# hamaadshah/gan_deeplearning4j

Hardware: NVIDIA H100
Metric: images/sec (full G+D step) (higher is better)
Workload: dtype bf16

## Files before the change

gan_deeplearning4j_b200/__init__.py:

```python
from ._lib import B200GanError, LIB_PATH, PROTOTYPES, load
from .engine import BF16, FP32, EPI_ACTBWD, EPI_BNBWD, EPI_PLAIN, EPI_STATS, Context, Gan, Net, comm_unique_id, test_bn, test_conv, test_conv_ex, test_dropout, test_ew
from . import data, models, parallel, serializer
```

gan_deeplearning4j_b200/_lib.py:

```python
from __future__ import annotations

import ctypes as C
import os

_HERE = os.path.dirname(os.path.abspath(__file__))
LIB_PATH = os.path.join(_HERE, "lib", "libb200gan.so")
NAME_LEN = 64


class B200GanError(RuntimeError):
    def __init__(self, code, msg):
        super().__init__(f"libb200gan error {code}: {msg}")
        self.code = code


class LayerDesc(C.Structure):
    _fields_ = [("type", C.c_int32), ("name", C.c_char * NAME_LEN), ("n_in", C.c_int32), ("n_out", C.c_int32),
                ("k_h", C.c_int32), ("k_w", C.c_int32), ("s_h", C.c_int32), ("s_w", C.c_int32), ("p_h", C.c_int32), ("p_w", C.c_int32),
                ("has_bias", C.c_int32), ("act", C.c_int32), ("act_alpha", C.c_float), ("updater", C.c_int32),
                ("lr", C.c_float), ("beta1", C.c_float), ("beta2", C.c_float), ("eps", C.c_float), ("l2", C.c_float),
                ("bn_decay", C.c_float), ("bn_eps", C.c_float), ("pre_h", C.c_int32), ("pre_w", C.c_int32), ("pre_c", C.c_int32),
                ("loss", C.c_int32), ("frozen", C.c_int32)]


class NetConfig(C.Structure):
    _fields_ = [("in_h", C.c_int32), ("in_w", C.c_int32), ("in_c", C.c_int32), ("max_batch", C.c_int32), ("precision", C.c_int32),
                ("grad_clip", C.c_float), ("xent_clip_eps", C.c_float), ("bn_groups", C.c_int32), ("seed", C.c_uint64)]


class GanConfig(C.Structure):
    _fields_ = [("fake_bn_train", C.c_int32), ("use_cuda_graph", C.c_int32)]


class LrSchedule(C.Structure):
    _fields_ = [("kind", C.c_int32), ("type", C.c_int32), ("initial", C.c_double), ("gamma", C.c_double), ("power", C.c_double),
                ("step", C.c_double), ("decay_rate", C.c_double), ("n_map", C.c_int32), ("map_keys", C.POINTER(C.c_int32)),
                ("map_values", C.POINTER(C.c_double))]


class ConvGeom(C.Structure):
    _fields_ = [(k, C.c_int32) for k in ("n", "h", "w", "c", "oh", "ow", "o", "kh", "kw", "sh", "sw", "ph", "pw")]


class TestConvOpts(C.Structure):
    _fields_ = [("epi", C.c_int32), ("act", C.c_int32), ("alpha", C.c_float), ("bias", C.POINTER(C.c_float)), ("scale", C.POINTER(C.c_float)),
                ("groups", C.c_int32), ("aux", C.POINTER(C.c_float)), ("aux2", C.POINTER(C.c_float)), ("stats", C.POINTER(C.c_double)), ("kernel", C.c_char * 64),
                ("bn", C.c_int32), ("max_ctas", C.c_int32), ("poison", C.c_int32), ("w_mn", C.c_int32), ("per_tap", C.c_int32), ("slab", C.c_int32),
                ("defer", C.c_int32), ("db", C.POINTER(C.c_float)), ("param_offset", C.c_int32), ("splits", C.c_int32)]


class EwReduceJob(C.Structure):
    _fields_ = [("n", C.c_int64), ("stride", C.c_int64), ("src_off", C.c_int64), ("dst_off", C.c_int64), ("splits", C.c_int32), ("wide", C.c_int32)]


class TestEwOpts(C.Structure):
    _fields_ = [("op", C.c_int32), ("n", C.c_int64), ("rows", C.c_int32), ("cols", C.c_int32), ("groups", C.c_int32), ("splits", C.c_int32),
                ("stride", C.c_int64)] + [(k, C.c_int32) for k in ("N", "H", "W", "C", "KH", "KW", "SH", "SW", "act")] + [
                ("alpha", C.c_float), ("clip_eps", C.c_float), ("offset", C.c_int32), ("in_place", C.c_int32), ("accumulate", C.c_int32),
                ("poison", C.c_int32), ("n_jobs", C.c_int32), ("jobs", C.POINTER(EwReduceJob)), ("n_seg", C.c_int32),
                ("seg_off", C.POINTER(C.c_int64)), ("seg_len", C.POINTER(C.c_int64)), ("seg_coef", C.POINTER(C.c_float)), ("sumsq", C.c_double),
                ("kernel", C.c_char * 64), ("loss", C.c_int32)]


_vp, _i32, _i64, _fp = C.c_void_p, C.c_int32, C.c_int64, C.POINTER(C.c_float)
_pvp = C.POINTER(C.c_void_p)

PROTOTYPES = {
    "b2g_version": (_i32, []),
    "b2g_ctx_create": (_i32, [_i32, _pvp]),
    "b2g_ctx_destroy": (_i32, [_vp]),
    "b2g_last_error": (C.c_char_p, []),
    "b2g_sync": (_i32, [_vp]),
    "b2g_launch_count": (_i32, [_vp, C.POINTER(C.c_uint64)]),
    "b2g_timer_start": (_i32, [_vp]),
    "b2g_timer_stop_ms": (_i32, [_vp, _fp]),
    "b2g_flush_l2": (_i32, [_vp]),
    "b2g_device_info": (_i32, [_vp, C.POINTER(_i32), C.POINTER(_i32), C.POINTER(_i32), C.POINTER(C.c_uint64)]),
    "b2g_net_create": (_i32, [_vp, C.POINTER(NetConfig), C.POINTER(LayerDesc), _i32, _pvp]),
    "b2g_net_destroy": (_i32, [_vp]),
    "b2g_net_num_params": (_i32, [_vp, C.POINTER(_i64)]),
    "b2g_net_output_size": (_i32, [_vp, C.POINTER(_i64)]),
    "b2g_net_layer_output_size": (_i32, [_vp, _i32, C.POINTER(_i64)]),
    "b2g_net_set_param": (_i32, [_vp, C.c_char_p, C.c_char_p, _fp, _i64]),
    "b2g_net_get_param": (_i32, [_vp, C.c_char_p, C.c_char_p, _fp, _i64]),
    "b2g_net_get_params": (_i32, [_vp, _fp, _i64]),
    "b2g_net_set_params": (_i32, [_vp, _fp, _i64]),
    "b2g_net_get_gradients": (_i32, [_vp, _fp, _i64]),
    "b2g_net_updater_state_size": (_i32, [_vp, C.POINTER(_i64)]),
    "b2g_net_get_updater_state": (_i32, [_vp, _fp, _i64]),
    "b2g_net_set_updater_state": (_i32, [_vp, _fp, _i64]),
    "b2g_net_output": (_i32, [_vp, _fp, _i32, _i32, _fp]),
    "b2g_net_get_activation": (_i32, [_vp, _i32, _i32, _fp]),
    "b2g_net_compute_gradient_and_score": (_i32, [_vp, _fp, _fp, _i32, _fp]),
    "b2g_net_get_input_gradient": (_i32, [_vp, _i32, _fp]),
    "b2g_net_fit": (_i32, [_vp, _fp, _fp, _i32, _fp]),
    "b2g_net_get_iteration": (_i32, [_vp, C.POINTER(_i64)]),
    "b2g_net_set_iteration": (_i32, [_vp, _i64]),
    "b2g_net_get_dropout_pass": (_i32, [_vp, C.POINTER(_i64)]),
    "b2g_net_set_dropout_pass": (_i32, [_vp, _i64]),
    "b2g_net_set_gradient_normalization": (_i32, [_vp, _i32, C.c_float]),
    "b2g_net_set_lr_schedule": (_i32, [_vp, C.c_char_p, C.POINTER(LrSchedule)]),
    "b2g_net_get_learning_rate": (_i32, [_vp, C.c_char_p, _fp]),
    "b2g_net_get_epoch": (_i32, [_vp, C.POINTER(_i64)]),
    "b2g_net_set_epoch": (_i32, [_vp, _i64]),
    "b2g_net_simt_gemm_calls": (_i32, [_vp, C.POINTER(C.c_uint64)]),
    "b2g_gan_create": (_i32, [_vp, _vp, C.POINTER(GanConfig), _pvp]),
    "b2g_gan_destroy": (_i32, [_vp]),
    "b2g_gan_step": (_i32, [_vp, _fp, _fp, _fp, _fp, _fp, _fp, _i32, _fp]),
    "b2g_gan_upload": (_i32, [_vp, _fp, _fp, _fp, _fp, _fp, _fp, _i32]),
    "b2g_gan_step_resident": (_i32, [_vp, _i32]),
    "b2g_gan_read_losses": (_i32, [_vp, _fp]),
    "b2g_gan_last_step_ms": (_i32, [_vp, _fp]),
    "b2g_comm_unique_id": (_i32, [_vp]),
    "b2g_ctx_comm_init": (_i32, [_vp, _i32, _i32, _vp]),
    "b2g_ctx_comm_destroy": (_i32, [_vp]),
    "b2g_net_set_grad_allreduce": (_i32, [_vp, _i32]),
    "b2g_net_average_parameters": (_i32, [_vp]),
    "b2g_net_set_sync_bn": (_i32, [_vp, _i32]),
    "b2g_net_set_grad_payload_bf16": (_i32, [_vp, _i32]),
    "b2g_net_enable_p2p_allreduce": (_i32, [_vp, C.POINTER(C.c_int32)]),
    "b2g_ctx_allreduce_test": (_i32, [_vp, _fp, _i64]),
    "b2g_test_conv": (_i32, [_vp, _i32, _i32, _i32, C.POINTER(ConvGeom), _fp, _fp, _fp, _i32, _fp]),
    "b2g_test_hbm_kernels": (_i32, [_vp, _i32, _i32, _i32, _fp]),
    "b2g_test_conv_ex": (_i32, [_vp, _i32, _i32, _i32, C.POINTER(ConvGeom), _fp, _fp, _fp, _i32, _fp, C.POINTER(TestConvOpts)]),
    "b2g_test_bn": (_i32, [_vp, _i32, _i32, _i32, _i32, _i32, _fp, _fp, _fp, _fp, _fp, _fp, _i32, C.c_float, C.c_float, C.c_float,
                           _i32, _fp, _fp, _fp, _fp, _fp, _fp, _fp, _fp]),
    "b2g_test_net_shadow": (_i32, [_vp, _i32, _i32, _fp, _i64]),
    "b2g_test_dropout": (_i32, [_vp, _i32, C.c_uint64, _i32, _i32, _i64, _i32, _i32, _i32, _i32, C.c_float, _fp, _fp, _fp, _fp]),
    "b2g_test_ew": (_i32, [_vp, _i32, C.POINTER(TestEwOpts), _fp, _fp, _fp, _fp, _fp]),
}

_lib = None


def load():
    global _lib
    if _lib is not None:
        return _lib
    if not os.path.exists(LIB_PATH):
        raise B200GanError(-7, f"{LIB_PATH} is missing: build it with `make` (nvcc, sm_90a). There is no CPU fallback.")
    lib = C.CDLL(LIB_PATH, mode=C.RTLD_GLOBAL)
    for name, (res, args) in PROTOTYPES.items():
        fn = getattr(lib, name)
        fn.restype, fn.argtypes = res, args
    _lib = lib
    return lib


def check(code):
    if code != 0:
        raise B200GanError(code, load().b2g_last_error().decode(errors="replace"))
```

gan_deeplearning4j_b200/csrc/common.cuh:

```cuda
#pragma once
#include <cuda_runtime.h>
#include <cuda_bf16.h>
#include <math.h>
#include <stdlib.h>
#include <stdint.h>
#include "kernels.h"

namespace b2g {

#define LAUNCHED() do { ++::b2g::g_launch_count; } while (0)

__device__ __forceinline__ void pdl_wait() { asm volatile("griddepcontrol.wait;" ::: "memory"); }
__device__ __forceinline__ void pdl_trigger() { asm volatile("griddepcontrol.launch_dependents;" ::: "memory"); }
__device__ __forceinline__ void pdl_enter() { pdl_trigger(); pdl_wait(); }
template <typename... KArgs, typename... Args>
inline cudaError_t launch_pdl(void (*kernel)(KArgs...), dim3 grid, dim3 block, size_t smem, cudaStream_t stream, Args&&... args) {
  cudaLaunchConfig_t cfg{}; cfg.gridDim = grid; cfg.blockDim = block; cfg.dynamicSmemBytes = smem; cfg.stream = stream;
  cudaLaunchAttribute at[1]; at[0].id = cudaLaunchAttributeProgrammaticStreamSerialization; at[0].val.programmaticStreamSerializationAllowed = 1;
  cfg.attrs = at; cfg.numAttrs = 1;
  return cudaLaunchKernelEx(&cfg, kernel, static_cast<KArgs>(args)...);
}

__device__ __forceinline__ void sacc_add(unsigned long long* hi_lo, size_t stride, size_t idx, double d) {
  const long long hi = __double2ll_rn(d * 1024.0);
  const double r = d - (double)hi * (1.0 / 1024.0);
  const long long lo = __double2ll_rn(r * 1152921504606846976.0);
  atomicAdd(hi_lo + idx, (unsigned long long)hi);
  atomicAdd(hi_lo + stride + idx, (unsigned long long)lo);
}
__device__ __forceinline__ double sacc_read(const unsigned long long* hi_lo, size_t stride, size_t idx) {
  return (double)(long long)hi_lo[idx] * (1.0 / 1024.0) + (double)(long long)hi_lo[stride + idx] * (1.0 / 1152921504606846976.0);
}

__device__ __forceinline__ double block_sum(double v, double* red) {
#pragma unroll
  for (int o = 16; o > 0; o >>= 1) v += __shfl_xor_sync(0xffffffffu, v, o);
  if ((threadIdx.x & 31) == 0) red[threadIdx.x >> 5] = v;
  __syncthreads();
  double t = 0.0;
  if (threadIdx.x == 0) for (int w = 0; w < (int)(blockDim.x >> 5); ++w) t += red[w];
  return t;
}

struct Philox4 { uint32_t x[4]; };
__device__ __forceinline__ Philox4 philox4x32_10(uint32_t c0, uint32_t c1, uint32_t c2, uint32_t c3, uint32_t k0, uint32_t k1) {
#pragma unroll
  for (int r = 0; r < 10; ++r) {
    if (r) { k0 += 0x9E3779B9u; k1 += 0xBB67AE85u; }
    const uint32_t lo0 = 0xD2511F53u * c0, hi0 = __umulhi(0xD2511F53u, c0);
    const uint32_t lo1 = 0xCD9E8D57u * c2, hi1 = __umulhi(0xCD9E8D57u, c2);
    c0 = hi1 ^ c1 ^ k0; c1 = lo1; c2 = hi0 ^ c3 ^ k1; c3 = lo0;
  }
  return Philox4{{c0, c1, c2, c3}};
}

#define DISPATCH_PREC(prec, T, ...)                                   \
  do {                                                                \
    if ((prec) == ::b2g::PREC_F32) { using T = float; __VA_ARGS__; }  \
    else { using T = __nv_bfloat16; __VA_ARGS__; }                    \
  } while (0)

__device__ __forceinline__ float ldf(const float* p, size_t i) { return p[i]; }
__device__ __forceinline__ float ldf(const __nv_bfloat16* p, size_t i) { return __bfloat162float(p[i]); }
__device__ __forceinline__ void stf(float* p, size_t i, float v) { p[i] = v; }
__device__ __forceinline__ void stf(__nv_bfloat16* p, size_t i, float v) { p[i] = __float2bfloat16_rn(v); }

__device__ __forceinline__ float act_fwd(int act, float z, float alpha) {
  switch (act) {
    case ACT_TANH: return tanhf(z);
    case ACT_SIGMOID: return 1.0f / (1.0f + expf(-z));
    case ACT_RELU: return fmaxf(z, 0.f);
    case ACT_LRELU: return z > 0.f ? z : alpha * z;
    default: return z;
  }
}
__device__ __forceinline__ float act_grad_from_pre(int act, float z, float alpha) {
  switch (act) {
    case ACT_TANH: { float t = tanhf(z); return 1.0f - t * t; }
    case ACT_SIGMOID: { float s = 1.0f / (1.0f + expf(-z)); return s * (1.0f - s); }
    case ACT_RELU: return z > 0.f ? 1.0f : 0.f;
    case ACT_LRELU: return z > 0.f ? 1.0f : alpha;
    default: return 1.0f;
  }
}
__device__ __forceinline__ float act_grad_from_out(int act, float a, float alpha) {
  switch (act) {
    case ACT_TANH: return 1.0f - a * a;
    case ACT_SIGMOID: return a * (1.0f - a);
    case ACT_RELU: return a > 0.f ? 1.0f : 0.f;
    case ACT_LRELU: return a > 0.f ? 1.0f : alpha;
    default: return 1.0f;
  }
}

}
```

gan_deeplearning4j_b200/csrc/engine.cu:

```cuda
#include <cuda_runtime.h>
#include <dlfcn.h>
#include <math.h>
#include <stdarg.h>
#include <stdio.h>
#include <stdlib.h>
#include <string.h>

#include <algorithm>
#include <string>
#include <vector>

#include "../../include/b200gan.h"
#include "kernels.h"

using namespace b2g;

static thread_local char g_err[1024] = "";
static int32_t fail(int32_t code, const char* fmt, ...) {
  va_list ap; va_start(ap, fmt); vsnprintf(g_err, sizeof(g_err), fmt, ap); va_end(ap); return code;
}
#define CU(call) do { cudaError_t e_ = (call); if (e_ != cudaSuccess) return fail(B2G_ERR_CUDA, "%s:%d %s -> %s", __FILE__, __LINE__, #call, cudaGetErrorString(e_)); } while (0)
#define B2(call) do { int32_t r_ = (call); if (r_ != 0) return r_; } while (0)
#define CHECK_KERNELS() CU(cudaGetLastError())

// ... 1065 lines not shown
      g->graph_launches = g_launch_count - before; g_launch_count = before;
      g->graph_simt_g = g->G->simt_gemm_calls - sg0; g->graph_simt_d = g->D->simt_gemm_calls - sd0; g->G->simt_gemm_calls = sg0; g->D->simt_gemm_calls = sd0;
      if (r) return r; if (e != cudaSuccess) return fail(B2G_ERR_CUDA, "graph capture: %s", cudaGetErrorString(e));
      CU(cudaGraphInstantiate(&g->exec1, g->graph1, 0)); CU(cudaGraphInstantiate(&g->exec, g->graph, 0)); g->graph_batch = batch;
      g->graph_settings_g = g->G->settings_gen; g->graph_settings_d = g->D->settings_gen;
    }
    CU(cudaGraphLaunch(g->exec1, s));
    CU(cudaStreamWaitEvent(s, g->ev_x, 0));
    CU(cudaGraphLaunch(g->exec, s)); g_launch_count += g->graph_launches; g->G->simt_gemm_calls += g->graph_simt_g; g->D->simt_gemm_calls += g->graph_simt_d;
  }
  CU(cudaEventRecord(g->ev1, s)); g->ev1_valid = true;
  return 0;
}
extern "C" int32_t b2g_gan_read_losses(b2g_gan* g, float* losses) {
  if (!g || !losses) return fail(B2G_ERR_ARG, "null"); cudaStream_t s = g->G->ctx->stream; CU(cudaSetDevice(g->G->ctx->device));
  float h[4]; CU(cudaMemcpyAsync(h, g->loss_dev, sizeof(h), cudaMemcpyDeviceToHost, s)); CU(cudaStreamSynchronize(s));
  int N = g->last_batch;
  losses[0] = h[0] / N; losses[1] = h[1] / N; losses[2] = h[2] / N; return 0;
}
extern "C" int32_t b2g_gan_last_step_ms(b2g_gan* g, float* ms) {
  if (!g || !ms) return fail(B2G_ERR_ARG, "null"); CU(cudaEventSynchronize(g->ev1)); CU(cudaEventElapsedTime(ms, g->ev0, g->ev1)); return 0;
}
extern "C" int32_t b2g_gan_step(b2g_gan* g, const float* x_real, const float* z_d, const float* z_g, const float* y_real, const float* y_fake, const float* y_gen, int32_t batch, float* losses) {
  B2(b2g_gan_upload(g, x_real, z_d, z_g, y_real, y_fake, y_gen, batch));
  B2(b2g_gan_step_resident(g, batch));
  if (losses) return b2g_gan_read_losses(g, losses);
  return 0;
}

extern "C" int32_t b2g_net_get_iteration(b2g_net* n, int64_t* out) {
  if (!n || !out) return fail(B2G_ERR_ARG, "null"); CU(cudaSetDevice(n->ctx->device));
  int v = 0; CU(cudaMemcpyAsync(&v, n->step_dev, sizeof(int), cudaMemcpyDeviceToHost, n->ctx->stream)); CU(cudaStreamSynchronize(n->ctx->stream)); *out = v; return 0;
}
extern "C" int32_t b2g_net_set_iteration(b2g_net* n, int64_t it) {
  if (!n || it < 0 || it > 0x7fffffff) return fail(B2G_ERR_ARG, "bad iteration"); CU(cudaSetDevice(n->ctx->device));
  int v = (int)it; CU(cudaMemcpyAsync(n->step_dev, &v, sizeof(int), cudaMemcpyHostToDevice, n->ctx->stream)); CU(cudaStreamSynchronize(n->ctx->stream)); return 0;
}
extern "C" int32_t b2g_net_get_dropout_pass(b2g_net* n, int64_t* out) {
  if (!n || !out) return fail(B2G_ERR_ARG, "null"); CU(cudaSetDevice(n->ctx->device));
  unsigned long long v = 0; CU(cudaMemcpyAsync(&v, n->drop_pass, sizeof(v), cudaMemcpyDeviceToHost, n->ctx->stream)); CU(cudaStreamSynchronize(n->ctx->stream)); *out = (int64_t)v; return 0;
}
extern "C" int32_t b2g_net_set_dropout_pass(b2g_net* n, int64_t pass) {
  if (!n || pass < 0) return fail(B2G_ERR_ARG, "bad dropout pass"); CU(cudaSetDevice(n->ctx->device));
  unsigned long long v = (unsigned long long)pass; CU(cudaMemcpyAsync(n->drop_pass, &v, sizeof(v), cudaMemcpyHostToDevice, n->ctx->stream)); CU(cudaStreamSynchronize(n->ctx->stream)); return 0;
}
extern "C" int32_t b2g_net_set_gradient_normalization(b2g_net* n, int32_t mode, float threshold) {
  if (!n) return fail(B2G_ERR_ARG, "null");
  if (mode == B2G_GN_CLIP_ELEMENTWISE) return fail(B2G_ERR_ARG, "ClipElementWiseAbsoluteValue is b2g_net_config.grad_clip, set when the net is created");
  if (mode != B2G_GN_NONE && mode != B2G_GN_RENORM_L2_LAYER && mode != B2G_GN_RENORM_L2_PARAM && mode != B2G_GN_CLIP_L2_LAYER && mode != B2G_GN_CLIP_L2_PARAM)
    return fail(B2G_ERR_ARG, "unknown gradient normalization %d", mode);
  if (mode != B2G_GN_NONE && n->cfg.grad_clip > 0.f)
    return fail(B2G_ERR_ARG, "the net was created with grad_clip %g (ClipElementWiseAbsoluteValue): one gradient normalization per layer", (double)n->cfg.grad_clip);
  const bool clip = mode == B2G_GN_CLIP_L2_LAYER || mode == B2G_GN_CLIP_L2_PARAM;
  if (clip && !(threshold > 0.f && isfinite(threshold))) return fail(B2G_ERR_ARG, "gradient normalization threshold %g: the clip modes need a finite threshold > 0", (double)threshold);
  if (!clip) threshold = 1.0f;
  if (mode != n->gn_mode || threshold != n->gn_threshold) { n->gn_mode = mode; n->gn_threshold = threshold; ++n->settings_gen; }
  return 0;
}

static int lr_segment(const b2g_net* n, int li) {
  for (size_t i = 0; i < n->segs.size(); ++i) if (n->seg_layer[i] == li && n->segs[i].kind != 3 && n->segs[i].kind != 9) return (int)i;
  return -1;
}
static bool layer_has_lr(const b2g_net* n, int li) { return lr_segment(n, li) >= 0; }
static int32_t find_lr_layer(const b2g_net* n, const char* layer, int* li) {
  for (size_t i = 0; i < n->L.size(); ++i) if (!strncmp(n->L[i].d.name, layer, B2G_NAME_LEN)) {
    if (!layer_has_lr(n, (int)i)) return fail(B2G_ERR_ARG, "layer %s has no learning rate (frozen, no parameters, NoOp or AdaDelta)", layer);
    *li = (int)i; return 0;
  }
  return fail(B2G_ERR_ARG, "no layer named %s", layer);
}
static int32_t net_upload_schedules(b2g_net* n) {
  cudaStream_t s = n->ctx->stream;
  size_t nv = 0; for (auto& ls : n->layer_sched) nv += ls.vals.size();
  const size_t bytes = nv * (sizeof(double) + sizeof(int32_t));
  CU(cudaStreamSynchronize(s));
  if (bytes > n->sched_map_bytes) {
    if (n->sched_map) { cudaFree(n->sched_map); n->sched_map = nullptr; n->sched_map_bytes = 0; }
    cudaError_t e = cudaMalloc(&n->sched_map, bytes);
    if (e != cudaSuccess) { n->sched_map = nullptr; return fail(B2G_ERR_OOM, "cudaMalloc(%zu) failed: %s", bytes, cudaGetErrorString(e)); }
    n->sched_map_bytes = bytes;
  }
  std::vector<char> host(bytes); double* dv = (double*)n->sched_map; int32_t* dk = (int32_t*)((char*)n->sched_map + nv * sizeof(double));
  std::vector<UpdSched> per_layer(n->L.size()); size_t at = 0;
  for (size_t li = 0; li < n->L.size(); ++li) {
    const auto& ls = n->layer_sched[li]; per_layer[li] = ls.sc;
    if (ls.sc.kind == B2G_SCHED_MAP) {
      memcpy(host.data() + at * sizeof(double), ls.vals.data(), ls.vals.size() * sizeof(double));
      memcpy(host.data() + nv * sizeof(double) + at * sizeof(int32_t), ls.keys.data(), ls.keys.size() * sizeof(int32_t));
      per_layer[li].vals = dv + at; per_layer[li].keys = dk + at; at += ls.vals.size();
    }
  }
  std::vector<UpdSched> seg(n->segs.size()); bool on = false;
  for (size_t i = 0; i < n->segs.size(); ++i) { seg[i] = per_layer[n->seg_layer[i]]; on = on || seg[i].kind != B2G_SCHED_NONE; }
  if (bytes) CU(cudaMemcpyAsync(n->sched_map, host.data(), bytes, cudaMemcpyHostToDevice, s));
  if (!seg.empty()) CU(cudaMemcpyAsync(n->sched_dev, seg.data(), sizeof(UpdSched) * seg.size(), cudaMemcpyHostToDevice, s));
  CU(cudaStreamSynchronize(s));
  n->sched_on = on; ++n->settings_gen;
  return 0;
}
extern "C" int32_t b2g_net_set_lr_schedule(b2g_net* n, const char* layer, const b2g_lr_schedule* s) {
  if (!n) return fail(B2G_ERR_ARG, "null"); CU(cudaSetDevice(n->ctx->device));
  b2g_net::LayerSched ls;
  if (s && s->kind != B2G_SCHED_NONE) {
    if (s->kind < B2G_SCHED_EXPONENTIAL || s->kind > B2G_SCHED_MAP) return fail(B2G_ERR_ARG, "unknown schedule kind %d (PolySchedule is not supported)", s->kind);
    if (s->type != B2G_SCHED_ITERATION && s->type != B2G_SCHED_EPOCH) return fail(B2G_ERR_ARG, "unknown schedule type %d", s->type);
    if (!std::isfinite(s->initial) || !std::isfinite(s->gamma) || !std::isfinite(s->power) || !std::isfinite(s->step) || !std::isfinite(s->decay_rate))
      return fail(B2G_ERR_ARG, "schedule parameters must be finite");
    if (s->kind == B2G_SCHED_STEP && !(s->step > 0.0)) return fail(B2G_ERR_ARG, "StepSchedule step %g: must be > 0", s->step);
    if (s->kind == B2G_SCHED_INVERSE && s->gamma < 0.0) return fail(B2G_ERR_ARG, "InverseSchedule gamma %g: must be >= 0", s->gamma);
    UpdSched& sc = ls.sc; sc.kind = s->kind; sc.type = s->type;
    sc.initial = s->initial; sc.gamma = s->gamma; sc.power = s->power; sc.step = s->step; sc.decay = s->decay_rate;
    if (s->kind == B2G_SCHED_MAP) {
      if (s->n_map < 1 || !s->map_keys || !s->map_values) return fail(B2G_ERR_ARG, "MapSchedule needs at least one entry");
      bool has0 = false;
      for (int j = 0; j < s->n_map; ++j) {
        if (j > 0 && s->map_keys[j] <= s->map_keys[j - 1]) return fail(B2G_ERR_ARG, "MapSchedule keys must strictly increase");
        if (!std::isfinite(s->map_values[j])) return fail(B2G_ERR_ARG, "MapSchedule values must be finite");
        has0 = has0 || s->map_keys[j] == 0;
      }
      if (!has0) return fail(B2G_ERR_ARG, "MapSchedule has no value for key 0");
      ls.keys.assign(s->map_keys, s->map_keys + s->n_map); ls.vals.assign(s->map_values, s->map_values + s->n_map); sc.n_map = s->n_map;
    }
  }
  if (layer) { int li = 0; B2(find_lr_layer(n, layer, &li)); n->layer_sched[li] = ls; }
  else for (size_t li = 0; li < n->L.size(); ++li) if (layer_has_lr(n, (int)li)) n->layer_sched[li] = ls;
  return net_upload_schedules(n);
}
extern "C" int32_t b2g_net_get_learning_rate(b2g_net* n, const char* layer, float* out) {
  if (!n || !layer || !out) return fail(B2G_ERR_ARG, "null"); CU(cudaSetDevice(n->ctx->device));
  int li = 0; B2(find_lr_layer(n, layer, &li));
  const int seg = lr_segment(n, li);
  k_sched_lr(n->segs_dev, n->sched_dev, seg, n->step_dev, n->epoch_dev, n->lr_out, n->ctx->stream); CHECK_KERNELS();
  CU(cudaMemcpyAsync(out, n->lr_out, sizeof(float), cudaMemcpyDeviceToHost, n->ctx->stream)); CU(cudaStreamSynchronize(n->ctx->stream));
  return 0;
}
extern "C" int32_t b2g_net_get_epoch(b2g_net* n, int64_t* out) {
  if (!n || !out) return fail(B2G_ERR_ARG, "null"); CU(cudaSetDevice(n->ctx->device));
  int64_t v = 0; CU(cudaMemcpyAsync(&v, n->epoch_dev, sizeof(v), cudaMemcpyDeviceToHost, n->ctx->stream)); CU(cudaStreamSynchronize(n->ctx->stream)); *out = v; return 0;
}
extern "C" int32_t b2g_net_set_epoch(b2g_net* n, int64_t epoch) {
  if (!n || epoch < 0) return fail(B2G_ERR_ARG, "bad epoch"); CU(cudaSetDevice(n->ctx->device));
  CU(cudaMemcpyAsync(n->epoch_dev, &epoch, sizeof(epoch), cudaMemcpyHostToDevice, n->ctx->stream)); CU(cudaStreamSynchronize(n->ctx->stream)); return 0;
}
extern "C" int32_t b2g_net_simt_gemm_calls(b2g_net* n, uint64_t* out) { if (!n || !out) return fail(B2G_ERR_ARG, "null"); *out = n->simt_gemm_calls; return 0; }

extern "C" int32_t b2g_comm_unique_id(void* id128) { if (!id128) return fail(B2G_ERR_ARG, "null"); B2(nccl_load()); NcclId id; NC(g_nccl.uid(&id)); memcpy(id128, &id, sizeof(id)); return 0; }
extern "C" int32_t b2g_ctx_comm_init(b2g_ctx* c, int32_t world, int32_t rank, const void* id128) {
  if (!c || !id128 || world < 1 || rank < 0 || rank >= world) return fail(B2G_ERR_ARG, "bad communicator arguments");
  B2(nccl_load()); CU(cudaSetDevice(c->device));
  NcclId id; memcpy(&id, id128, sizeof(id));
  NC(g_nccl.init(&c->comm, world, id, rank)); c->world = world; c->rank = rank; return 0;
}
extern "C" int32_t b2g_ctx_comm_destroy(b2g_ctx* c) { if (c && c->comm) { g_nccl.destroy(c->comm); c->comm = nullptr; c->world = 1; c->rank = 0; } return 0; }
extern "C" int32_t b2g_net_set_grad_allreduce(b2g_net* n, int32_t enabled) { if (!n) return fail(B2G_ERR_ARG, "null"); n->grad_allreduce = enabled != 0; return 0; }
extern "C" int32_t b2g_net_set_sync_bn(b2g_net* n, int32_t enabled) { if (!n) return fail(B2G_ERR_ARG, "null"); if (enabled && n->prec != PREC_BF16) return fail(B2G_ERR_UNSUPPORTED, "sync_bn rides on the fused BatchNorm path (BF16 nets)"); n->sync_bn = enabled != 0; return 0; }
extern "C" int32_t b2g_net_set_grad_payload_bf16(b2g_net* n, int32_t enabled) {
  if (!n) return fail(B2G_ERR_ARG, "null"); CU(cudaSetDevice(n->ctx->device));
  if (enabled && !n->ar_buf) B2(dalloc(n, &n->ar_buf, sizeof(__nv_bfloat16) * (size_t)n->n_params));
  n->ar_bf16 = enabled != 0; return 0;
}
extern "C" int32_t b2g_net_enable_p2p_allreduce(b2g_net* n, int32_t* enabled) {
  if (!n) return fail(B2G_ERR_ARG, "null"); b2g_ctx* c = n->ctx; CU(cudaSetDevice(c->device)); if (enabled) *enabled = 0;
  if (!c->comm || c->world < 2) return 0;
  if (c->world > 8 || !g_nccl.ag) return 0;
  cudaStream_t s = c->stream;
  if (!c->p2p_flags) { CU(cudaMalloc(&c->p2p_flags, 16 * sizeof(unsigned))); CU(cudaMalloc(&c->p2p_state, 2 * sizeof(unsigned)));
                       CU(cudaMemsetAsync(c->p2p_flags, 0, 16 * sizeof(unsigned), s)); CU(cudaMemsetAsync(c->p2p_state, 0, 2 * sizeof(unsigned), s)); CU(cudaStreamSynchronize(s)); }
  struct Pair { cudaIpcMemHandle_t flags, grads; };
  Pair mine; memset(&mine, 0, sizeof(mine)); float ok = 1.f;
  if (cudaIpcGetMemHandle(&mine.flags, c->p2p_flags) != cudaSuccess || cudaIpcGetMemHandle(&mine.grads, n->grads) != cudaSuccess) { cudaGetLastError(); ok = 0.f; }
  std::vector<Pair> all(c->world);
  char *d_send = nullptr, *d_recv = nullptr; float* d_ok = nullptr;
  CU(cudaMalloc(&d_send, sizeof(Pair))); CU(cudaMalloc(&d_recv, sizeof(Pair) * c->world)); CU(cudaMalloc(&d_ok, sizeof(float)));
  CU(cudaMemcpyAsync(d_send, &mine, sizeof(Pair), cudaMemcpyHostToDevice, s));
  NC(g_nccl.ag(d_send, d_recv, sizeof(Pair),  0, c->comm, s));
  CU(cudaMemcpyAsync(all.data(), d_recv, sizeof(Pair) * c->world, cudaMemcpyDeviceToHost, s)); CU(cudaStreamSynchronize(s));
  float* pg[8] = {}; unsigned* pf[8] = {};
  for (int r = 0; r < c->world && ok > 0.f; ++r) {
    if (r == c->rank) { pg[r] = n->grads; pf[r] = c->p2p_flags; continue; }
    void* q = nullptr;
    if (cudaIpcOpenMemHandle(&q, all[r].grads, cudaIpcMemLazyEnablePeerAccess) != cudaSuccess) { cudaGetLastError(); ok = 0.f; break; }
    pg[r] = (float*)q;
    if (c->p2p_flags_mapped) pf[r] = c->p2p_peer_flags[r];
    else { if (cudaIpcOpenMemHandle(&q, all[r].flags, cudaIpcMemLazyEnablePeerAccess) != cudaSuccess) { cudaGetLastError(); ok = 0.f; break; } pf[r] = (unsigned*)q; }
  }
  CU(cudaMemcpyAsync(d_ok, &ok, sizeof(float), cudaMemcpyHostToDevice, s)); NC(g_nccl.ar(d_ok, d_ok, 1, 7, 0, c->comm, s));
  float sum = 0.f; CU(cudaMemcpyAsync(&sum, d_ok, sizeof(float), cudaMemcpyDeviceToHost, s)); CU(cudaStreamSynchronize(s));
  cudaFree(d_send); cudaFree(d_recv); cudaFree(d_ok);
  if (sum < (float)c->world - 0.5f) {
    for (int r = 0; r < c->world; ++r) { if (r == c->rank) continue; if (pg[r]) cudaIpcCloseMemHandle(pg[r]); if (!c->p2p_flags_mapped && pf[r]) cudaIpcCloseMemHandle(pf[r]); }
    return 0;
  }
  for (int r = 0; r < c->world; ++r) { n->p2p_peer_grads[r] = pg[r]; c->p2p_peer_flags[r] = pf[r]; }
  c->p2p_flags_mapped = true; n->p2p = true; if (enabled) *enabled = 1;
  return 0;
}
extern "C" int32_t b2g_net_average_parameters(b2g_net* n) {
  if (!n) return fail(B2G_ERR_ARG, "null"); b2g_ctx* c = n->ctx; CU(cudaSetDevice(c->device));
  if (!c->comm || c->world == 1) return 0;
  const float inv = 1.0f / (float)c->world; cudaStream_t s = c->stream;
  float* bufs[4] = {n->params, n->st0, n->st1, n->st2};
  for (float* b : bufs) { if (!b) continue; NC(g_nccl.ar(b, b, (size_t)n->n_params, 7, 0, c->comm, s)); k_scale_f32(b, inv, (size_t)n->n_params, s); }
  net_refresh_shadow(n);
  CU(cudaStreamSynchronize(s)); return 0;
}
extern "C" int32_t b2g_ctx_allreduce_test(b2g_ctx* c, float* host, int64_t n) {
  if (!c || !host || n < 1) return fail(B2G_ERR_ARG, "null"); if (!c->comm) return fail(B2G_ERR_NCCL, "no communicator"); CU(cudaSetDevice(c->device));
  float* d = nullptr; CU(cudaMalloc(&d, sizeof(float) * n));
  CU(cudaMemcpyAsync(d, host, sizeof(float) * n, cudaMemcpyHostToDevice, c->stream));
  NC(g_nccl.ar(d, d, (size_t)n, 7, 0, c->comm, c->stream));
  CU(cudaMemcpyAsync(host, d, sizeof(float) * n, cudaMemcpyDeviceToHost, c->stream)); CU(cudaStreamSynchronize(c->stream)); cudaFree(d); return 0;
}

struct TcTestSchedule {
  TcTestSchedule(int bn, int max_ctas, int per_tap) { g_tc_test_bn = bn; g_tc_test_max_ctas = max_ctas; g_tc_test_per_tap = per_tap; }
  ~TcTestSchedule() { reset(); }
  void reset() { g_tc_test_bn = 0; g_tc_test_max_ctas = 0; g_tc_test_per_tap = 0; }
};
extern "C" int32_t b2g_test_conv_ex(b2g_ctx* c, int32_t kind, int32_t impl, int32_t precision, const b2g_conv_geom* gg, const float* a_host, const float* b_host, float* out, int32_t iters, float* ms_per_iter,
                                    b2g_test_conv_opts* opt) {
  if (!c || !gg || !a_host || !b_host || !out) return fail(B2G_ERR_ARG, "null"); CU(cudaSetDevice(c->device));
  cudaStream_t s = c->stream; int prec = precision == B2G_PREC_BF16 ? PREC_BF16 : PREC_F32; size_t ts = prec_size(prec);
  ConvGeom g{gg->n, gg->h, gg->w, gg->c, gg->oh, gg->ow, gg->o, gg->kh, gg->kw, gg->sh, gg->sw, gg->ph, gg->pw};
  size_t nx = (size_t)g.N * g.H * g.W * g.C, ny = (size_t)g.N * g.OH * g.OW * g.O, nw = (size_t)g.O * g.KH * g.KW * g.C;
  size_t na = kind == 1 ? ny : nx, nb = kind == 2 ? ny : nw, no = kind == 0 ? ny : kind == 1 ? nx : nw;
  const int oc = kind == 0 ? g.O : g.C;
  if (impl == 1) {
    if (prec != PREC_BF16 || !c->tc_ok) return fail(B2G_ERR_UNSUPPORTED, "tensor-core kernels need BF16 precision and a working tensor-map encoder");
    bool ok = kind == 0 ? tc_fprop_supported(g) : kind == 1 ? tc_dgrad_supported(g) : tc_wgrad_supported(g);
    if (!ok) return fail(B2G_ERR_UNSUPPORTED, "no tensor-core kernel for this shape");
  }
  const bool tc_conv = impl == 1 && kind != 2, ps = impl == 3 && kind == 1;
  const bool gemm = impl == 0 || impl == 2 || impl == 4;
  const bool gemm_epi = gemm && kind != 2 && !(impl == 4 && kind == 1 && !dense_small_k_supported(g));
  if (opt && gemm) {
    if (opt->epi || (!gemm_epi && (opt->bias || opt->scale || opt->act)))
      return fail(B2G_ERR_UNSUPPORTED, "impl %d kind %d: no epilogue (bias / activation: impl 0 / 2 kind 0 / 1, impl 4 kind 0 and the short-reduction kind 1; no fused BatchNorm epilogue)", impl, kind);
    if (opt->scale && impl != 0) return fail(B2G_ERR_UNSUPPORTED, "scale applies to the SIMT fprop / dgrad (impl 0) and the tensor-core kernels");
  }
  else if (opt && !tc_conv && !ps && (opt->epi || opt->bias || opt->scale || opt->act))
    return fail(B2G_ERR_UNSUPPORTED, "epilogue options apply to the tensor-core fprop / dgrad kernels (impl 1, kind 0 / 1), the pixel-shuffle deconv (impl 3, kind 1) and the SIMT / skinny-layer / dense kernels (impl 0 / 2 / 4)");
  const int poff = opt ? opt->param_offset : 0;
  if (poff < 0 || (poff && !gemm)) return fail(B2G_ERR_UNSUPPORTED, "param_offset %d: applies to the SIMT / skinny-layer / dense kernels (impl 0 / 2 / 4)", poff);
  if (opt && ps && (opt->scale || (opt->epi != EPI_PLAIN && opt->epi != EPI_ACTBWD)))
    return fail(B2G_ERR_UNSUPPORTED, "the pixel-shuffle deconv has bias, activation and the activation-backward epilogue only");
  const int force_bn = opt ? opt->bn : 0, max_ctas = opt ? opt->max_ctas : 0;
  const bool poison = opt && opt->poison, w_mn = opt && opt->w_mn, per_tap = opt && opt->per_tap;
  if (per_tap && !tc_conv) return fail(B2G_ERR_UNSUPPORTED, "per_tap applies to the tensor-core fprop / dgrad kernels (impl 1, kind 0 / 1)");
  if (force_bn && (!tc_conv || (force_bn != 64 && force_bn != 128) || oc % force_bn))
    return fail(B2G_ERR_UNSUPPORTED, "bn %d: the tensor-core fprop / dgrad tile is 64 or 128 columns and must divide the %d output channels", force_bn, oc);
  if (max_ctas < 0 || (max_ctas && !tc_conv && !ps)) return fail(B2G_ERR_UNSUPPORTED, "max_ctas %d: a grid cap applies to tc_conv_kernel launches only", max_ctas);
  if (poison && kind == 2 && !gemm) return fail(B2G_ERR_UNSUPPORTED, "poison applies to the outputs of kinds 0 / 1, and to the weight gradients of impl 0 / 2 / 4");
  if (w_mn && (impl != 1 || kind != 0 || g.KH != 1 || g.KW != 1)) return fail(B2G_ERR_UNSUPPORTED, "w_mn: the [C][O] weight operand exists for the 1x1 tensor-core fprop only");
  const bool defer = opt && opt->defer; float* db_host = opt ? opt->db : nullptr;
  if (defer && !(kind == 2 && (impl == 1 || impl == 3))) return fail(B2G_ERR_UNSUPPORTED, "defer applies to the tensor-core weight gradients (kind 2, impl 1 / 3)");
  if (db_host && !(kind == 2 && impl == 3)) return fail(B2G_ERR_UNSUPPORTED, "db is the edge tensor-core weight gradient's bias column (kind 2, impl 3)");
  if (impl == 2 || impl == 3) {
    bool ok = kind == 0 ? edge_conv_small_cin_supported(g) : kind == 1 ? edge_deconv_small_c_supported(g) : edge_wgrad_small_cin_supported(g);
    if (impl == 3) ok = ok && prec == PREC_BF16 && c->tc_ok && (kind == 0 ? tc_edge_conv_supported(g) : kind == 1 ? tc_deconv_ps_supported(g) : tc_edge_wgrad_supported(g));
    if (ps) ok = prec == PREC_BF16 && c->tc_ok && tc_deconv_ps_supported(g);
    if (!ok) return fail(B2G_ERR_UNSUPPORTED, "no skinny-layer kernel (impl %d) for this shape", impl);
  }
  if (impl == 4 && !(dense_small_o_supported(g) || (dense_small_k_supported(g) && kind != 0))) return fail(B2G_ERR_UNSUPPORTED, "no dense kernel for this shape");
  float *fa = nullptr, *fb = nullptr, *fo = nullptr, *scratch = nullptr; void *ta = nullptr, *tb = nullptr, *to = nullptr; __nv_bfloat16* wps = nullptr;
  float *d_bias = nullptr, *d_scale = nullptr, *d_coef = nullptr, *d_auxf = nullptr; __nv_bfloat16 *d_aux = nullptr, *d_aux2 = nullptr; unsigned long long* d_acc = nullptr;
  size_t sc = std::max(std::max(std::max(k_simt_wgrad_scratch_floats(g), k_tc_wgrad_scratch_floats(g)), std::max(k_edge_wgrad_scratch_floats(g), k_tc_edge_wgrad_scratch_floats(g))), k_dense_small_o_wgrad_scratch_floats(g)) + 16;
  const size_t woff = (prec == PREC_F32 && kind != 2) ? (size_t)poff : 0, dwoff = kind == 2 ? (size_t)poff : 0;
  CU(cudaMalloc(&fa, 4 * na)); CU(cudaMalloc(&fb, 4 * nb)); CU(cudaMalloc(&fo, 4 * (no + dwoff))); CU(cudaMalloc(&scratch, 4 * sc));
  CU(cudaMalloc(&ta, ts * na)); CU(cudaMalloc(&tb, ts * nb + 4 * woff)); CU(cudaMalloc(&to, ts * no));
  float* const fres = fo + dwoff;
  void* const tbase = tb; tb = (float*)tb + woff;
  CU(cudaMemcpyAsync(fa, a_host, 4 * na, cudaMemcpyHostToDevice, s)); CU(cudaMemcpyAsync(fb, b_host, 4 * nb, cudaMemcpyHostToDevice, s));
  if (prec == PREC_BF16) { k_cast_f32_to_bf16(fa, (__nv_bfloat16*)ta, na, s); k_cast_f32_to_bf16(fb, (__nv_bfloat16*)tb, nb, s); }
  else { CU(cudaMemcpyAsync(ta, fa, 4 * na, cudaMemcpyDeviceToDevice, s)); CU(cudaMemcpyAsync(tb, fb, 4 * nb, cudaMemcpyDeviceToDevice, s)); }
  if (impl == 3 && kind == 1) { CU(cudaMalloc(&wps, 2 * k_tc_deconv_ps_weight_elems(g))); k_pack_deconv_ps(fb, wps, g.O, g.C, s); }
  float* d_db = nullptr; int db_written = 0;
  if (db_host) CU(cudaMalloc(&d_db, 4 * (size_t)g.O));
  ReduceList rl{}; ReduceList* prl = defer ? &rl : nullptr;
  TcEpi epi{}; const TcEpi* pe = nullptr; const float* bias = nullptr; int act = 0; float alpha = 0.f; int groups = 1;
  if (opt && (tc_conv || ps)) {
    groups = opt->groups > 0 ? opt->groups : 1; act = opt->act; alpha = opt->alpha;
    if (opt->bias) { CU(cudaMalloc(&d_bias, 4 * oc)); CU(cudaMemcpyAsync(d_bias, opt->bias, 4 * oc, cudaMemcpyHostToDevice, s)); bias = d_bias; }
    if (opt->scale) { CU(cudaMalloc(&d_scale, 4 * oc)); CU(cudaMemcpyAsync(d_scale, opt->scale, 4 * oc, cudaMemcpyHostToDevice, s)); }
    epi.mode = opt->epi; epi.scale = d_scale; epi.imgs_per_group = g.N / groups; epi.act = opt->act; epi.alpha = opt->alpha;
    if (opt->epi == EPI_STATS || opt->epi == EPI_BNBWD) { CU(cudaMalloc(&d_acc, 8 * k_bn_acc_elems(oc, groups))); epi.acc = d_acc; }
    if (opt->epi == EPI_BNBWD || opt->epi == EPI_ACTBWD) {
      if (!opt->aux) return fail(B2G_ERR_ARG, "epilogue %d needs aux", opt->epi);
      CU(cudaMalloc(&d_auxf, 4 * no)); CU(cudaMalloc(&d_aux, 2 * no)); CU(cudaMemcpyAsync(d_auxf, opt->aux, 4 * no, cudaMemcpyHostToDevice, s)); k_cast_f32_to_bf16(d_auxf, d_aux, no, s); epi.aux = d_aux;
    }
    if (opt->epi == EPI_BNBWD) {
      if (!opt->aux2) return fail(B2G_ERR_ARG, "epilogue 2 needs aux2 (the BatchNorm input z)");
      CU(cudaMalloc(&d_coef, 4 * no)); CU(cudaMalloc(&d_aux2, 2 * no)); CU(cudaMemcpyAsync(d_coef, opt->aux2, 4 * no, cudaMemcpyHostToDevice, s)); k_cast_f32_to_bf16(d_coef, d_aux2, no, s); epi.aux2 = d_aux2;
    }
    if (opt->epi || opt->scale) pe = &epi;
  }
  if (opt && gemm_epi) {
    act = opt->act; alpha = opt->alpha;
    if (opt->bias) { CU(cudaMalloc(&d_bias, 4 * oc)); CU(cudaMemcpyAsync(d_bias, opt->bias, 4 * oc, cudaMemcpyHostToDevice, s)); bias = d_bias; }
    if (opt->scale) { CU(cudaMalloc(&d_scale, 4 * oc)); CU(cudaMemcpyAsync(d_scale, opt->scale, 4 * oc, cudaMemcpyHostToDevice, s)); }
  }
  cudaEvent_t e0, e1; CU(cudaEventCreate(&e0)); CU(cudaEventCreate(&e1));
  int reps = iters < 1 ? 1 : iters; int rc = 0;
  g_tc_last_kernel = ""; g_tc_last_slab = false; g_gemm_last_kernel = ""; g_gemm_last_splits = 0;
  TcTestSchedule schedule(force_bn, max_ctas, per_tap);
  for (int it = -1; it < reps; ++it) {
    if (it == 0) CU(cudaEventRecord(e0, s));
    if (d_acc) CU(cudaMemsetAsync(d_acc, 0, 8 * k_bn_acc_elems(oc, groups), s));
    if (poison) CU(cudaMemsetAsync(to, 0xFF, ts * no, s));
    if (poison && kind == 2) { CU(cudaMemsetAsync(fres, 0xFF, 4 * no, s)); CU(cudaMemsetAsync(scratch, 0xFF, 4 * sc, s)); }
    if (impl == 4) {
      const bool so = dense_small_o_supported(g);
      if (kind == 0) k_dense_small_o_fwd(prec, prec, g, ta, tb, bias, to, act, alpha, s);
      else if (kind == 1) { if (so && !bias && !act) k_dense_small_o_dgrad(prec, prec, g, ta, tb, to, s); else k_dense_small_k_dgrad(prec, prec, g, ta, tb, bias, to, act, alpha, s); }
      else { if (so) k_dense_small_o_wgrad(prec, g, ta, tb, fres, scratch, 0, s); else k_dense_small_k_wgrad(prec, g, ta, tb, fres, s); }
    }
    else if (impl >= 2) {
      if (kind == 0) { if (impl == 3) rc = k_tc_edge_conv(g, (const __nv_bfloat16*)ta, (const __nv_bfloat16*)tb, nullptr, (__nv_bfloat16*)to, 0, 0.f, s); else k_edge_conv_small_cin(prec, prec, g, ta, tb, bias, to, act, alpha, s); }
      else if (kind == 1) { if (impl == 3) rc = k_tc_deconv_ps(g, (const __nv_bfloat16*)ta, wps, bias, (__nv_bfloat16*)to, act, alpha, s, pe); else k_edge_deconv_small_c(prec, prec, g, ta, tb, bias, to, act, alpha, s); }
      else {
        if (impl == 3) { rc = k_tc_edge_wgrad(g, (const __nv_bfloat16*)ta, (const __nv_bfloat16*)tb, fres, d_db, scratch, sc, 0, s, prl); if (rc >= 0) { db_written = rc; rc = 0; } }
        else k_edge_wgrad_small_cin(prec, g, ta, tb, fres, scratch, 0, s);
      }
    }
    else if (kind == 0) { if (impl) rc = k_tc_fprop(g, (const __nv_bfloat16*)ta, (const __nv_bfloat16*)tb, bias, (__nv_bfloat16*)to, act, alpha, s, pe, w_mn ? 1 : 0); else k_simt_fprop(prec, prec, g, ta, tb, bias, to, act, alpha, s, d_scale); }
    else if (kind == 1) { if (impl) rc = k_tc_dgrad(g, (const __nv_bfloat16*)ta, (const __nv_bfloat16*)tb, bias, (__nv_bfloat16*)to, act, alpha, s, pe); else k_simt_dgrad(prec, prec, g, ta, tb, bias, to, act, alpha, s, d_scale); }
    else { if (impl) rc = k_tc_wgrad(g, (const __nv_bfloat16*)ta, (const __nv_bfloat16*)tb, fres, scratch, sc, 0, s, prl); else k_simt_wgrad(prec, g, ta, tb, fres, scratch, sc, 0, s); }
    if (rc) break;
    if (defer) {
      if (!rl.count) { rc = -4; break; }
      k_reduce_multi(rl, s); rl.count = 0;
    }
  }
  schedule.reset();
  CU(cudaEventRecord(e1, s));
  if (rc == -4) return fail(B2G_ERR_CUDA, "defer: the weight gradient queued no reduction");
  if (rc) return fail(B2G_ERR_CUDA, "tensor-core kernel launch failed (%d)", rc);
  if (opt) {
    strncpy(opt->kernel, gemm ? g_gemm_last_kernel : g_tc_last_kernel, sizeof(opt->kernel) - 1); opt->kernel[sizeof(opt->kernel) - 1] = 0; opt->slab = g_tc_last_slab;
    opt->splits = gemm ? g_gemm_last_splits : 0;
  }
  if (d_db) {
    if (!db_written) { cudaFree(d_db); return fail(B2G_ERR_UNSUPPORTED, "the edge weight gradient produces no bias column for C = %d", g.C); }
    CU(cudaMemcpyAsync(db_host, d_db, 4 * (size_t)g.O, cudaMemcpyDeviceToHost, s));
  }
  if (kind != 2) { if (prec == PREC_BF16) {  k_nhwc_to_nchw_f32(prec, to, fo, 1, 1, (int)no, s); } else CU(cudaMemcpyAsync(fo, to, 4 * no, cudaMemcpyDeviceToDevice, s)); }
  CU(cudaMemcpyAsync(out, fres, 4 * no, cudaMemcpyDeviceToHost, s));
  CU(cudaStreamSynchronize(s)); CHECK_KERNELS();
  if (d_acc && opt && opt->stats) {
    std::vector<long long> h(k_bn_acc_elems(oc, groups)); CU(cudaMemcpy(h.data(), d_acc, 8 * h.size(), cudaMemcpyDeviceToHost));
    for (int gi = 0; gi < groups; ++gi) for (int st = 0; st < 2; ++st) for (int ch = 0; ch < oc; ++ch)
      opt->stats[((size_t)gi * 2 + st) * oc + ch] = (double)h[((size_t)(gi * 2 + st) * 2 + 0) * oc + ch] / 1024.0 + (double)h[((size_t)(gi * 2 + st) * 2 + 1) * oc + ch] / 1152921504606846976.0;
  }
  float ms = 0.f; CU(cudaEventElapsedTime(&ms, e0, e1)); if (ms_per_iter) *ms_per_iter = ms / reps;
  cudaEventDestroy(e0); cudaEventDestroy(e1);
  cudaFree(fa); cudaFree(fb); cudaFree(fo); cudaFree(scratch); cudaFree(ta); cudaFree(tbase); cudaFree(to); if (wps) cudaFree(wps); if (d_db) cudaFree(d_db);
  if (d_bias) cudaFree(d_bias); if (d_scale) cudaFree(d_scale); if (d_coef) cudaFree(d_coef); if (d_auxf) cudaFree(d_auxf); if (d_aux) cudaFree(d_aux); if (d_aux2) cudaFree(d_aux2); if (d_acc) cudaFree(d_acc);
  return 0;
}
extern "C" int32_t b2g_test_conv(b2g_ctx* c, int32_t kind, int32_t impl, int32_t precision, const b2g_conv_geom* gg, const float* a_host, const float* b_host, float* out, int32_t iters, float* ms_per_iter) {
  return b2g_test_conv_ex(c, kind, impl, precision, gg, a_host, b_host, out, iters, ms_per_iter, nullptr);
}

extern "C" int32_t b2g_test_bn(b2g_ctx* c, int32_t precision, int32_t path, int32_t groups, int32_t rows, int32_t C, const float* x, const float* eps_out,
                               const float* gamma, const float* beta, const float* run_mean, const float* run_var, int32_t act, float alpha, float eps, float decay,
                               int32_t want_param_grads, float* y, float* eps_in, float* g_gamma, float* g_beta, float* g_mean, float* g_var, float* mean, float* invstd) {
  if (!c || !x || !eps_out || !gamma || !beta || !run_mean || !run_var || !y || !eps_in || !g_gamma || !g_beta || !g_mean || !g_var || !mean || !invstd) return fail(B2G_ERR_ARG, "null");
  if (groups < 1 || rows < 1 || C < 1 || path < 0 || path > 2) return fail(B2G_ERR_ARG, "bad BatchNorm test arguments");
  const int prec = precision == B2G_PREC_BF16 ? PREC_BF16 : PREC_F32;
  if (path != 0 && !k_bn_vec_ok(prec, C)) return fail(B2G_ERR_UNSUPPORTED, "the accumulator BatchNorm kernels need bf16 and C %% 8 == 0 with 256 %% (C/8) == 0 (C = %d)", C);
  CU(cudaSetDevice(c->device)); cudaStream_t s = c->stream;
  const size_t n = (size_t)groups * rows * C, gc = (size_t)groups * C, ts = prec_size(prec);
  std::vector<void*> mem;
  auto alloc = [&](void** p, size_t bytes) -> int32_t { *p = nullptr; CU(cudaMalloc(p, bytes)); mem.push_back(*p); return 0; };
  auto release = [&]() { for (void* p : mem) cudaFree(p); mem.clear(); };
  float *fx, *fe, *fo, *d_par, *d_grad, *d_stat, *scratch, *coef, *unit; void *tx, *te, *ty, *tei; unsigned long long* acc;
  int32_t r = 0;
  if ((r = alloc((void**)&fx, 4 * n)) || (r = alloc((void**)&fe, 4 * n)) || (r = alloc((void**)&fo, 4 * n)) || (r = alloc(&tx, ts * n)) || (r = alloc(&te, ts * n)) ||
      (r = alloc(&ty, ts * n)) || (r = alloc(&tei, ts * n)) || (r = alloc((void**)&d_par, 4 * 4 * (size_t)C)) || (r = alloc((void**)&d_grad, 4 * 4 * (size_t)C)) ||
      (r = alloc((void**)&d_stat, 4 * 2 * gc)) || (r = alloc((void**)&scratch, 4 * k_bn_scratch_floats(C, groups))) || (r = alloc((void**)&coef, 4 * 4 * gc)) ||
      (r = alloc((void**)&unit, 4 * 4 * gc)) || (r = alloc((void**)&acc, 8 * 2 * k_bn_acc_elems(C, groups)))) { release(); return r; }
  float *d_gamma = d_par, *d_beta = d_par + C, *d_rm = d_par + 2 * C, *d_rv = d_par + 3 * C;
  float *d_gg = d_grad, *d_gb = d_grad + C, *d_gm = d_grad + 2 * C, *d_gv = d_grad + 3 * C, *d_mean = d_stat, *d_is = d_stat + gc;
  unsigned long long *acc_f = acc, *acc_b = acc + k_bn_acc_elems(C, groups);
  auto up = [&](float* d, const float* h, size_t k) { return cudaMemcpyAsync(d, h, 4 * k, cudaMemcpyHostToDevice, s); };
  if (up(fx, x, n) || up(fe, eps_out, n) || up(d_gamma, gamma, C) || up(d_beta, beta, C) || up(d_rm, run_mean, C) || up(d_rv, run_var, C) ||
      up(d_gg, g_gamma, C) || up(d_gb, g_beta, C) || cudaMemsetAsync(acc, 0, 8 * 2 * k_bn_acc_elems(C, groups), s)) { release(); return fail(B2G_ERR_CUDA, "BatchNorm test upload failed"); }
  if (prec == PREC_BF16) { k_cast_f32_to_bf16(fx, (__nv_bfloat16*)tx, n, s); k_cast_f32_to_bf16(fe, (__nv_bfloat16*)te, n, s); }
  else { cudaMemcpyAsync(tx, fx, 4 * n, cudaMemcpyDeviceToDevice, s); cudaMemcpyAsync(te, fe, 4 * n, cudaMemcpyDeviceToDevice, s); }
  const int want = want_param_grads ? 1 : 0;
  if (path == 0) {
    k_bn_stats(prec, tx, rows, C, groups, scratch, d_mean, d_is, eps, d_rm, d_rv, d_gm, d_gv, decay, s);
    k_bn_apply(prec, tx, ty, rows, C, groups, d_mean, d_is, d_gamma, d_beta, act, alpha, s);
    k_bn_bwd(prec, tx, te, tei, rows, C, groups, d_mean, d_is, d_gamma, d_beta, act, alpha, scratch, d_gg, d_gb, want, s);
  } else {
    k_bn_stats_acc(tx, rows, C, groups, acc_f, s);
    k_bn_apply_acc(tx, ty, rows, C, groups, acc_f, d_gamma, d_beta, act, alpha, eps, coef, d_rm, d_rv, d_gm, d_gv, decay, s, 1);
    if (path == 1) k_bn_bwd_stats_acc(tx, te, rows, C, groups, coef, act, alpha, acc_b, s);
    else {
      for (int g = 0; g < groups; ++g) for (int k = 0; k < 4; ++k) k_fill_f32(unit + (size_t)(g * 4 + k) * C, (k == 0 || k == 3) ? 1.f : 0.f, C, s);
      k_bn_bwd_stats_acc(tx, te, rows, C, groups, unit, ACT_IDENTITY, 0.f, acc_b, s);
    }
    k_bn_bwd_apply_acc(tx, te, tei, rows, C, groups, coef, act, alpha, path == 2 ? 1 : 0, acc_b, d_gg, d_gb, want, s, 1);
    for (int g = 0; g < groups; ++g) {
      cudaMemcpyAsync(d_mean + (size_t)g * C, coef + (size_t)(g * 4 + 2) * C, 4 * C, cudaMemcpyDeviceToDevice, s);
      cudaMemcpyAsync(d_is + (size_t)g * C, coef + (size_t)(g * 4 + 3) * C, 4 * C, cudaMemcpyDeviceToDevice, s);
    }
  }
  auto down = [&](float* h, const void* t) -> int32_t {
    k_nhwc_to_nchw_f32(prec, t, fo, 1, 1, (int)n, s); CU(cudaMemcpyAsync(h, fo, 4 * n, cudaMemcpyDeviceToHost, s)); CU(cudaStreamSynchronize(s)); return 0;
  };
  if ((r = down(y, ty)) || (r = down(eps_in, tei))) { release(); return r; }
  cudaError_t e = cudaSuccess;
  float* hs[6] = {g_gamma, g_beta, g_mean, g_var, mean, invstd}; const float* ds[6] = {d_gg, d_gb, d_gm, d_gv, d_mean, d_is}; const size_t ks[6] = {(size_t)C, (size_t)C, (size_t)C, (size_t)C, gc, gc};
  for (int k = 0; k < 6 && e == cudaSuccess; ++k) e = cudaMemcpyAsync(hs[k], ds[k], 4 * ks[k], cudaMemcpyDeviceToHost, s);
  if (e == cudaSuccess) e = cudaStreamSynchronize(s);
  if (e == cudaSuccess) e = cudaGetLastError();
  release();
  if (e != cudaSuccess) return fail(B2G_ERR_CUDA, "BatchNorm test: %s", cudaGetErrorString(e));
  return 0;
}

extern "C" int32_t b2g_test_dropout(b2g_ctx* c, int32_t precision, uint64_t seed, int32_t layer, int32_t rank, int64_t pass, int32_t rows, int32_t h, int32_t w, int32_t ch,
                                    float p, const float* x, const float* dy, float* y, float* dx) {
  if (!c || !x || !dy || !y || !dx) return fail(B2G_ERR_ARG, "null");
  if (!(p > 0.f && p <= 1.f)) return fail(B2G_ERR_ARG, "dropout retain probability %g outside (0, 1]", (double)p);
  if (rows < 1 || h < 1 || w < 1 || ch < 1 || layer < 0 || layer > 0xffff || rank < 0 || rank > 0xffff || pass < 0) return fail(B2G_ERR_ARG, "bad dropout test arguments");
  const size_t n = (size_t)rows * h * w * ch;
  if (n > 0x7fffffff) return fail(B2G_ERR_UNSUPPORTED, "the dropout test hook takes at most 2^31 - 1 elements (%zu)", n);
  const int prec = precision == B2G_PREC_BF16 ? PREC_BF16 : PREC_F32; const size_t ts = prec_size(prec);
  CU(cudaSetDevice(c->device)); cudaStream_t s = c->stream;
  std::vector<void*> mem;
  auto alloc = [&](void** q, size_t bytes) -> int32_t { *q = nullptr; CU(cudaMalloc(q, bytes)); mem.push_back(*q); return 0; };
  auto release = [&]() { for (void* q : mem) cudaFree(q); mem.clear(); };
  float *fx, *fe; void *tx, *te, *ty; uint32_t* mask; unsigned long long* dpass; unsigned* ticket; int32_t r = 0;
  if ((r = alloc((void**)&fx, 4 * n)) || (r = alloc((void**)&fe, 4 * n)) || (r = alloc(&tx, ts * n)) || (r = alloc(&te, ts * n)) || (r = alloc(&ty, ts * n)) ||
      (r = alloc((void**)&mask, 4 * ((n + 31) / 32))) || (r = alloc((void**)&dpass, sizeof(unsigned long long))) || (r = alloc((void**)&ticket, sizeof(unsigned)))) { release(); return r; }
  const unsigned long long p0 = (unsigned long long)pass;
  cudaError_t e = cudaMemcpyAsync(fx, x, 4 * n, cudaMemcpyHostToDevice, s);
  if (e == cudaSuccess) e = cudaMemcpyAsync(fe, dy, 4 * n, cudaMemcpyHostToDevice, s);
  if (e == cudaSuccess) e = cudaMemcpyAsync(dpass, &p0, sizeof(p0), cudaMemcpyHostToDevice, s);
  if (e == cudaSuccess) e = cudaMemsetAsync(ticket, 0, sizeof(unsigned), s);
  if (e != cudaSuccess) { release(); return fail(B2G_ERR_CUDA, "dropout test upload: %s", cudaGetErrorString(e)); }
  if (prec == PREC_BF16) { k_cast_f32_to_bf16(fx, (__nv_bfloat16*)tx, n, s); k_cast_f32_to_bf16(fe, (__nv_bfloat16*)te, n, s); }
  else { cudaMemcpyAsync(tx, fx, 4 * n, cudaMemcpyDeviceToDevice, s); cudaMemcpyAsync(te, fe, 4 * n, cudaMemcpyDeviceToDevice, s); }
  const DropoutArgs a = make_dropout_args(seed, layer, rank, p);
  k_dropout_fwd(prec, tx, ty, mask, n, a, dpass, ticket, 1, s);
  k_dropout_bwd(prec, te, te, mask, n, a.scale, s);
  unsigned long long p1 = 0;
  k_nhwc_to_nchw_f32(prec, ty, fx, 1, 1, (int)n, s);
  k_nhwc_to_nchw_f32(prec, te, fe, 1, 1, (int)n, s);
  e = cudaMemcpyAsync(y, fx, 4 * n, cudaMemcpyDeviceToHost, s);
  if (e == cudaSuccess) e = cudaMemcpyAsync(dx, fe, 4 * n, cudaMemcpyDeviceToHost, s);
  if (e == cudaSuccess) e = cudaMemcpyAsync(&p1, dpass, sizeof(p1), cudaMemcpyDeviceToHost, s);
  if (e == cudaSuccess) e = cudaStreamSynchronize(s);
  if (e == cudaSuccess) e = cudaGetLastError();
  release();
  if (e != cudaSuccess) return fail(B2G_ERR_CUDA, "dropout test: %s", cudaGetErrorString(e));
  if (p1 != p0 + 1) return fail(B2G_ERR_CUDA, "dropout test: the forward left the pass counter at %llu, expected %llu", p1, p0 + 1);
  return 0;
}

namespace {
struct EwMem {
  std::vector<void*> v;
  ~EwMem() { for (void* p : v) cudaFree(p); }
};
}
extern "C" int32_t b2g_test_ew(b2g_ctx* c, int32_t precision, b2g_test_ew_opts* o, const float* in0, const float* in1, float* out0, float* out1, float* out2) {
  if (!c || !o) return fail(B2G_ERR_ARG, "null");
  const int prec = precision == B2G_PREC_BF16 ? PREC_BF16 : PREC_F32; const size_t ts = prec_size(prec);
  const int off = o->offset;
  if (off < 0 || off > 64) return fail(B2G_ERR_ARG, "offset %d outside [0, 64]", off);
  if (o->poison && o->accumulate) return fail(B2G_ERR_ARG, "poison would overwrite the initial destination accumulate adds to");
  CU(cudaSetDevice(c->device)); cudaStream_t s = c->stream;
  EwMem mem;
  auto dev = [&](size_t count, size_t es, void** p) -> int32_t { void* b = nullptr; CU(cudaMalloc(&b, es * (count + off) + 16)); mem.v.push_back(b); *p = (char*)b + es * off; return 0; };
  auto upF = [&](const float* h, size_t count, float** p) -> int32_t {
    B2(dev(count, 4, (void**)p)); if (h) CU(cudaMemcpyAsync(*p, h, 4 * count, cudaMemcpyHostToDevice, s)); return 0; };
  auto upT = [&](const float* h, size_t count, void** p) -> int32_t {
    B2(dev(count, ts, p)); if (!h) return 0;
    if (prec == PREC_F32) { CU(cudaMemcpyAsync(*p, h, 4 * count, cudaMemcpyHostToDevice, s)); return 0; }
    float* f = nullptr; CU(cudaMalloc(&f, 4 * count)); mem.v.push_back(f);
    CU(cudaMemcpyAsync(f, h, 4 * count, cudaMemcpyHostToDevice, s)); k_cast_f32_to_bf16(f, (__nv_bfloat16*)*p, count, s); return 0; };
  auto downF = [&](float* h, const float* d, size_t count) -> int32_t { if (h) CU(cudaMemcpyAsync(h, d, 4 * count, cudaMemcpyDeviceToHost, s)); return 0; };
  auto downT = [&](float* h, const void* d, size_t count) -> int32_t {
    if (!h) return 0;
    float* f = nullptr; CU(cudaMalloc(&f, 4 * count)); mem.v.push_back(f);
    k_nhwc_to_nchw_f32(prec, d, f, 1, 1, (int)count, s); CU(cudaMemcpyAsync(h, f, 4 * count, cudaMemcpyDeviceToHost, s)); return 0; };
  auto poison = [&](void* d, size_t bytes) -> int32_t { if (o->poison) CU(cudaMemsetAsync(d, 0xFF, bytes, s)); return 0; };
  std::string names;
  auto ran = [&]() { if (!names.empty()) names += ","; names += g_ew_last_kernel; g_ew_last_kernel = ""; };
  const int64_t lim = 0x7fffffff;
  g_ew_last_kernel = "";
  switch (o->op) {
    case B2G_EW_REDUCE_SPLITS: {
      if (!in0 || o->n < 1 || o->n > lim || o->splits < 1 || o->stride < o->n || (o->accumulate && !in1)) return fail(B2G_ERR_ARG, "bad REDUCE_SPLITS arguments");
      float *src = nullptr, *dst = nullptr; B2(upF(in0, (size_t)o->splits * o->stride, &src)); B2(upF(in1, (size_t)o->n, &dst)); B2(poison(dst, 4 * o->n));
      k_reduce_splits(src, dst, (size_t)o->n, o->splits, (size_t)o->stride, o->accumulate ? 1 : 0, s); ran();
      B2(downF(out0, dst, (size_t)o->n));
      break;
    }
    case B2G_EW_REDUCE_MULTI: {
      if (!in0 || o->n < 1 || o->n > lim || o->n_jobs < 1 || o->n_jobs > ReduceList::MAX_JOBS || !o->jobs) return fail(B2G_ERR_ARG, "bad REDUCE_MULTI arguments");
      const b2g_ew_reduce_job* J = o->jobs;
      auto src_end = [&](int i) { return J[i].src_off + (int64_t)(J[i].splits - 1) * J[i].stride + J[i].n; };
      for (int i = 0; i < o->n_jobs; ++i) {
        if (J[i].n < 1 || J[i].splits < 1 || J[i].stride < J[i].n || J[i].src_off < 0 || J[i].dst_off < 0 || src_end(i) > o->n || J[i].dst_off + J[i].n > o->n)
          return fail(B2G_ERR_ARG, "reduce job %d outside the buffer", i);
        for (int k = 0; k < o->n_jobs; ++k) {
          const bool src_hit = J[i].dst_off < src_end(k) && J[k].src_off < J[i].dst_off + J[i].n;
          const bool dst_hit = k != i && J[i].dst_off < J[k].dst_off + J[k].n && J[k].dst_off < J[i].dst_off + J[i].n;
          if (src_hit || dst_hit) return fail(B2G_ERR_ARG, "reduce job %d's destination overlaps job %d", i, k);
        }
      }
      float* buf = nullptr; B2(upF(in0, (size_t)o->n, &buf));
      ReduceList rl{};
      for (int i = 0; i < o->n_jobs; ++i) {
        reduce_list_push(&rl, buf + J[i].src_off, buf + J[i].dst_off, J[i].n, J[i].splits, J[i].stride);
        o->jobs[i].wide = rl.jobs[i].blocks < 0 ? 1 : 0;
        B2(poison(buf + J[i].dst_off, 4 * (size_t)J[i].n));
      }
      if (rl.count != o->n_jobs) return fail(B2G_ERR_ARG, "the reduce list took %d of %d jobs", rl.count, o->n_jobs);
      k_reduce_multi(rl, s); ran();
      B2(downF(out0, buf, (size_t)o->n));
      break;
    }
    case B2G_EW_COLSUM: {
      if (!in0 || o->rows < 1 || o->cols < 1 || (int64_t)o->rows * o->cols > lim || (o->accumulate && !in1)) return fail(B2G_ERR_ARG, "bad COLSUM arguments");
      void* x = nullptr; float *out = nullptr, *scratch = nullptr; B2(upT(in0, (size_t)o->rows * o->cols, &x)); B2(upF(in1, (size_t)o->cols, &out)); B2(poison(out, 4 * (size_t)o->cols));
      CU(cudaMalloc(&scratch, 4 * k_colsum_scratch_floats(o->cols))); mem.v.push_back(scratch);
      k_colsum(prec, x, o->rows, o->cols, scratch, out, o->accumulate ? 1 : 0, s); ran();
      B2(downF(out0, out, (size_t)o->cols));
      break;
    }
    case B2G_EW_XENT: {
      const size_t n = (size_t)o->rows * o->groups;
      if (!in0 || !in1 || o->rows < 1 || o->groups < 1 || (int64_t)n > lim) return fail(B2G_ERR_ARG, "bad XENT arguments");
      void *z = nullptr, *dz = nullptr; float *y = nullptr, *loss = nullptr; B2(upT(in0, n, &z)); B2(upF(in1, n, &y)); B2(dev(n, ts, &dz)); B2(upF(nullptr, (size_t)o->groups, &loss));
      B2(poison(dz, ts * n)); B2(poison(loss, 4 * (size_t)o->groups));
      k_xent(prec, z, y, dz, loss, o->rows, o->groups, o->clip_eps, s); ran();
      B2(downT(out0, dz, n)); B2(downF(out1, loss, (size_t)o->groups));
      break;
    }
    case B2G_EW_SOFTMAX_XENT: {
      const size_t n = (size_t)o->rows * o->cols;
      if (!in0 || o->rows < 1 || o->cols < 1 || (int64_t)n > lim) return fail(B2G_ERR_ARG, "bad SOFTMAX_XENT arguments");
      void *z = nullptr, *dz = nullptr, *p = nullptr; float *y = nullptr, *loss = nullptr; B2(upT(in0, n, &z)); if (in1) B2(upF(in1, n, &y));
      B2(dev(n, ts, &dz)); B2(dev(n, ts, &p)); B2(upF(nullptr, 1, &loss));
      B2(poison(dz, ts * n)); B2(poison(p, ts * n)); B2(poison(loss, 4));
      k_softmax_xent(prec, z, y, y ? dz : nullptr, p, y ? loss : nullptr, o->rows, o->cols, s); ran();
      B2(downT(out0, dz, n)); B2(downF(out1, loss, 1)); B2(downT(out2, p, n));
      break;
    }
    case B2G_EW_LOSS: {
      const size_t per = (size_t)o->rows * o->cols, n = per * o->groups;
      if (!in0 || !in1 || o->rows < 1 || o->cols < 1 || o->groups < 1 || (int64_t)n > lim || o->loss < B2G_LOSS_MSE || o->loss > B2G_LOSS_WASSERSTEIN ||
          o->act < B2G_ACT_IDENTITY || o->act > B2G_ACT_LRELU) return fail(B2G_ERR_ARG, "bad LOSS arguments");
      void *z = nullptr, *dz = nullptr; float *y = nullptr, *loss = nullptr; double* partial = nullptr; unsigned* ticket = nullptr;
      B2(upT(in0, n, &z)); B2(upF(in1, n, &y)); B2(dev(n, ts, &dz)); B2(upF(nullptr, (size_t)o->groups, &loss));
      B2(dev((size_t)o->groups * k_loss_blocks(per, o->groups), 8, (void**)&partial)); B2(dev(1, 4, (void**)&ticket)); CU(cudaMemsetAsync(ticket, 0, 4, s));
      B2(poison(dz, ts * n)); B2(poison(loss, 4 * (size_t)o->groups));
      k_loss(prec, o->loss, o->act, o->alpha, z, y, dz, loss, o->rows, o->cols, o->groups, partial, ticket, s); ran();
      B2(downT(out0, dz, n)); B2(downF(out1, loss, (size_t)o->groups));
      break;
    }
    case B2G_EW_ACT_FWD: case B2G_EW_ACT_BWD: {
      const size_t n = (size_t)o->n; const bool bwd = o->op == B2G_EW_ACT_BWD;
      if (!in0 || (bwd && !in1) || o->n < 1 || o->n > lim || o->act < B2G_ACT_IDENTITY || o->act > B2G_ACT_LRELU) return fail(B2G_ERR_ARG, "bad activation arguments");
      void *a = nullptr, *e = nullptr, *r = nullptr; B2(upT(in0, n, &a));
      if (bwd) B2(upT(in1, n, &e));
      if (bwd && o->in_place) r = e;
      else { B2(dev(n, ts, &r)); B2(poison(r, ts * n)); }
      if (bwd) k_act_bwd_from_output(prec, a, e, r, n, o->act, o->alpha, s);
      else k_act_fwd(prec, a, r, n, o->act, o->alpha, s);
      ran();
      B2(downT(out0, r, n));
      break;
    }
    case B2G_EW_MAXPOOL: {
      if (!in0 || !in1 || o->N < 1 || o->C < 1 || o->KH < 1 || o->KW < 1 || o->SH < 1 || o->SW < 1 || o->H < o->KH || o->W < o->KW || o->KH * o->KW > 255)
        return fail(B2G_ERR_ARG, "bad MAXPOOL arguments");
      const int OH = (o->H - o->KH) / o->SH + 1, OW = (o->W - o->KW) / o->SW + 1;
      const size_t ni = (size_t)o->N * o->H * o->W * o->C, no = (size_t)o->N * OH * OW * o->C;
      if (ni > (size_t)lim) return fail(B2G_ERR_ARG, "MAXPOOL input too large");
      void *x = nullptr, *eo = nullptr, *y = nullptr, *ei = nullptr; uint8_t* arg = nullptr;
      B2(upT(in0, ni, &x)); B2(upT(in1, no, &eo)); B2(dev(no, ts, &y)); B2(dev(ni, ts, &ei)); B2(dev(no, 1, (void**)&arg));
      B2(poison(y, ts * no)); B2(poison(ei, ts * ni)); B2(poison(arg, no));
      k_maxpool_fwd(prec, x, y, arg, o->N, o->H, o->W, o->C, OH, OW, o->KH, o->KW, o->SH, o->SW, s); ran();
      k_maxpool_bwd(prec, eo, arg, ei, o->N, o->H, o->W, o->C, OH, OW, o->KH, o->KW, o->SH, o->SW, s); ran();
      B2(downT(out0, y, no)); B2(downT(out1, ei, ni));
      if (out2) {
        std::vector<uint8_t> h(no); CU(cudaMemcpyAsync(h.data(), arg, no, cudaMemcpyDeviceToHost, s)); CU(cudaStreamSynchronize(s));
        for (size_t i = 0; i < no; ++i) out2[i] = (float)h[i];
      }
      break;
    }
    case B2G_EW_UPSAMPLE: {
      const int f = o->KH;
      if (!in0 || !in1 || o->N < 1 || o->H < 1 || o->W < 1 || o->C < 1 || f < 1) return fail(B2G_ERR_ARG, "bad UPSAMPLE arguments");
      const size_t ni = (size_t)o->N * o->H * o->W * o->C, no = ni * f * f;
      if (no > (size_t)lim) return fail(B2G_ERR_ARG, "UPSAMPLE output too large");
      void *x = nullptr, *eo = nullptr, *y = nullptr, *ei = nullptr;
      B2(upT(in0, ni, &x)); B2(upT(in1, no, &eo)); B2(dev(no, ts, &y)); B2(dev(ni, ts, &ei)); B2(poison(y, ts * no)); B2(poison(ei, ts * ni));
      k_upsample_fwd(prec, x, y, o->N, o->H, o->W, o->C, f, s); ran();
      k_upsample_bwd(prec, eo, ei, o->N, o->H, o->W, o->C, f, s); ran();
      B2(downT(out0, y, no)); B2(downT(out1, ei, ni));
      break;
    }
    case B2G_EW_SUMSQ: {
      if (!in0 || o->n < 1 || o->n_seg < 1 || !o->seg_off || !o->seg_len || !o->seg_coef) return fail(B2G_ERR_ARG, "bad SUMSQ arguments");
      for (int i = 0; i < o->n_seg; ++i)
        if (o->seg_off[i] < 0 || o->seg_len[i] < 0 || o->seg_off[i] + o->seg_len[i] > o->n) return fail(B2G_ERR_ARG, "segment %d outside the tensor", i);
      float *p = nullptr, *coef = nullptr; int64_t *so = nullptr, *sl = nullptr; double* res = nullptr;
      B2(upF(in0, (size_t)o->n, &p)); B2(upF(o->seg_coef, (size_t)o->n_seg, &coef)); B2(dev((size_t)o->n_seg, 8, (void**)&so)); B2(dev((size_t)o->n_seg, 8, (void**)&sl)); B2(dev(1, 8, (void**)&res));
      CU(cudaMemcpyAsync(so, o->seg_off, 8 * (size_t)o->n_seg, cudaMemcpyHostToDevice, s)); CU(cudaMemcpyAsync(sl, o->seg_len, 8 * (size_t)o->n_seg, cudaMemcpyHostToDevice, s));
      B2(poison(res, 8));
      k_sumsq_segments(p, so, sl, coef, o->n_seg, res, s); ran();
      CU(cudaMemcpyAsync(&o->sumsq, res, 8, cudaMemcpyDeviceToHost, s));
      break;
    }
    default: return fail(B2G_ERR_ARG, "unknown op %d", o->op);
  }
  CU(cudaStreamSynchronize(s)); CHECK_KERNELS();
  strncpy(o->kernel, names.c_str(), sizeof(o->kernel) - 1); o->kernel[sizeof(o->kernel) - 1] = 0;
  return 0;
}

extern "C" int32_t b2g_test_net_shadow(b2g_net* n, int32_t layer, int32_t which, float* out, int64_t count) {
  if (!n || !out) return fail(B2G_ERR_ARG, "null");
  if (layer < 0 || layer >= (int)n->L.size()) return fail(B2G_ERR_ARG, "layer %d out of range", layer);
  if (n->prec != PREC_BF16) return fail(B2G_ERR_UNSUPPORTED, "FP32 nets keep no bf16 weight copies");
  const LayerRT& l = n->L[layer];
  int64_t off = -1, len = 0;
  if (which == 0) { off = l.off_W_bf; len = l.n_W; }
  else if (which == 1) { off = l.off_Wps_bf; len = (int64_t)k_tc_deconv_ps_weight_elems(l.geom); }
  else return fail(B2G_ERR_ARG, "which = %d (0 straight copy, 1 pixel-shuffle operand)", which);
  if (off < 0) return fail(B2G_ERR_UNSUPPORTED, "layer %d has no %s", layer, which ? "pixel-shuffle operand" : "bf16 weight copy");
  if (count != len) return fail(B2G_ERR_SHAPE, "layer %d operand has %lld elements, %lld requested", layer, (long long)len, (long long)count);
  CU(cudaSetDevice(n->ctx->device)); cudaStream_t s = n->ctx->stream;
  if ((size_t)len > n->stage_floats) return fail(B2G_ERR_SHAPE, "operand larger than the staging buffer");
  k_nhwc_to_nchw_f32(PREC_BF16, n->shadow + off, n->stage_f32, 1, 1, (int)len, s);
  CU(cudaMemcpyAsync(out, n->stage_f32, sizeof(float) * len, cudaMemcpyDeviceToHost, s)); CU(cudaStreamSynchronize(s)); CHECK_KERNELS();
  return 0;
}

extern "C" int32_t b2g_test_hbm_kernels(b2g_net* n, int32_t rows, int32_t channels, int32_t iters, float* ms3) {
  if (!n || !ms3 || rows < 8 || iters < 1) return fail(B2G_ERR_ARG, "bad arguments"); b2g_ctx* c = n->ctx; CU(cudaSetDevice(c->device)); cudaStream_t s = c->stream;
  if (!k_bn_vec_ok(PREC_BF16, channels)) return fail(B2G_ERR_UNSUPPORTED, "channels %d not supported by the vector BatchNorm kernels", channels);
  const size_t ne = (size_t)rows * channels; __nv_bfloat16 *x = nullptr, *e = nullptr, *y = nullptr; float *coef = nullptr, *gb = nullptr; unsigned long long* acc = nullptr;
  CU(cudaMalloc(&x, 2 * ne)); CU(cudaMalloc(&e, 2 * ne)); CU(cudaMalloc(&y, 2 * ne)); CU(cudaMalloc(&coef, 4 * 4 * channels)); CU(cudaMalloc(&gb, 4 * 4 * channels)); CU(cudaMalloc(&acc, 8 * k_bn_acc_elems(channels, 1)));
  CU(cudaMemsetAsync(x, 0x3c, 2 * ne, s)); CU(cudaMemsetAsync(e, 0x3c, 2 * ne, s)); CU(cudaMemsetAsync(acc, 0, 8 * k_bn_acc_elems(channels, 1), s)); k_fill_f32(coef, 1.0f, 4 * channels, s); k_fill_f32(gb, 1.0f, 4 * channels, s);
  cudaEvent_t e0, e1; CU(cudaEventCreate(&e0)); CU(cudaEventCreate(&e1));
  ms3[0] = ms3[1] = ms3[2] = 0.f;
  for (int which = 0; which < 3; ++which) for (int it = -1; it < iters; ++it) {
    B2(b2g_flush_l2(c));
    CU(cudaEventRecord(e0, s));
    if (which == 0) k_updater(n->params, n->grads, n->st0, n->st1, n->st2, n->segs_dev, n->chunk_seg_dev, n->chunk_off_dev, n->nchunks, 1.0f, 1.0f, n->step_dev, n->upd_ticket,
                              n->shadow, nullptr, nullptr, nullptr, n->upd_ext, s);
    else if (which == 1) k_bn_apply_acc(x, y, rows, channels, 1, acc, gb, gb + channels, ACT_LRELU, 0.2f, 1e-5f, coef, gb + 2 * channels, gb + 3 * channels, nullptr, nullptr, 0.9f, s);
    else k_bn_bwd_apply_acc(x, e, y, rows, channels, 1, coef, ACT_LRELU, 0.2f, 1, acc, gb, gb + channels, 0, s);
    CU(cudaEventRecord(e1, s)); CU(cudaEventSynchronize(e1));
    float ms = 0.f; CU(cudaEventElapsedTime(&ms, e0, e1)); if (it >= 0) ms3[which] += ms / iters;
  }
  CHECK_KERNELS();
// ... 4 lines not shown
```

gan_deeplearning4j_b200/csrc/kernels.h:

```cpp
#pragma once
#include <cuda_runtime.h>
#include <cuda_bf16.h>
#include <stdint.h>

namespace b2g {

enum Prec { PREC_F32 = 0, PREC_BF16 = 1 };
enum Act { ACT_IDENTITY = 0, ACT_TANH = 1, ACT_SIGMOID = 2, ACT_RELU = 3, ACT_LRELU = 4 };
enum Loss { LOSS_MSE = 2, LOSS_L1 = 3, LOSS_L2 = 4, LOSS_MAE = 5, LOSS_HINGE = 6, LOSS_SQUARED_HINGE = 7, LOSS_WASSERSTEIN = 8 };

inline size_t prec_size(int prec) { return prec == PREC_F32 ? 4 : 2; }

struct ConvGeom {
  int N, H, W, C;
  int OH, OW, O;
  int KH, KW, SH, SW, PH, PW;
};

extern uint64_t g_launch_count;
extern const char* g_ew_last_kernel;
int device_sm_count();

void k_nchw_f32_to_nhwc(int prec, const float* src, void* dst, int N, int C, int HW, cudaStream_t s);
void k_nhwc_to_nchw_f32(int prec, const void* src, float* dst, int N, int C, int HW, cudaStream_t s);
void k_permute(int prec, const void* src, void* dst, int N, int C, int HW, int to_nhwc, cudaStream_t s);
void k_cast_f32_to_bf16(const float* src, __nv_bfloat16* dst, size_t n, cudaStream_t s);

void k_bn_stats(int prec, const void* x, int rows_per_group, int C, int groups, float* scratch,
                float* mean, float* invstd, float eps,
                const float* run_mean, const float* run_var, float* g_mean, float* g_var, float decay, cudaStream_t s);
size_t k_bn_scratch_floats(int C, int groups);
void k_bn_fold(const float* run_mean, const float* run_var, const float* gamma, const float* beta, const float* conv_bias, int C, float eps, float* scale, float* shift, cudaStream_t s);
void k_bn_prep_infer(const float* run_mean, const float* run_var, int C, int groups, float eps, float* mean, float* invstd, cudaStream_t s);
void k_bn_apply(int prec, const void* x, void* y, int rows_per_group, int C, int groups, const float* mean, const float* invstd,
                const float* gamma, const float* beta, int act, float alpha, cudaStream_t s);
void k_bn_bwd(int prec, const void* x, const void* eps_out, void* eps_in, int rows_per_group, int C, int groups,
              const float* mean, const float* invstd, const float* gamma, const float* beta, int act, float alpha,
              float* scratch, float* g_gamma, float* g_beta, int want_param_grads, cudaStream_t s);

bool k_bn_vec_ok(int prec, int C);
size_t k_bn_acc_elems(int C, int groups);
void k_bn_stats_acc(const void* x, int rows_per_group, int C, int groups, unsigned long long* acc, cudaStream_t s);
void k_bn_apply_acc(const void* x, void* y, int rows_per_group, int C, int groups, const unsigned long long* acc, const float* gamma, const float* beta,
                    int act, float alpha, float eps, float* coef, const float* run_mean, const float* run_var, float* g_mean, float* g_var, float decay, cudaStream_t s, int replicas = 1);
void k_bn_bwd_stats_acc(const void* x, const void* eps_out, int rows_per_group, int C, int groups, const float* coef, int act, float alpha, unsigned long long* acc, cudaStream_t s);
void k_bn_bwd_apply_acc(const void* x, const void* eps_out, void* eps_in, int rows_per_group, int C, int groups, const float* coef, int act, float alpha, int premul,
                        const unsigned long long* acc, float* g_gamma, float* g_beta, int want_param_grads, cudaStream_t s, int replicas = 1);

void k_act_fwd(int prec, const void* x, void* y, size_t n, int act, float alpha, cudaStream_t s);
void k_act_bwd_from_output(int prec, const void* a, const void* eps_out, void* eps_in, size_t n, int act, float alpha, cudaStream_t s);
void k_maxpool_fwd(int prec, const void* x, void* y, uint8_t* argmax, int N, int H, int W, int C, int OH, int OW, int KH, int KW, int SH, int SW, cudaStream_t s);
void k_maxpool_bwd(int prec, const void* eps_out, const uint8_t* argmax, void* eps_in, int N, int H, int W, int C, int OH, int OW, int KH, int KW, int SH, int SW, cudaStream_t s);
void k_upsample_fwd(int prec, const void* x, void* y, int N, int H, int W, int C, int f, cudaStream_t s);
void k_upsample_bwd(int prec, const void* eps_out, void* eps_in, int N, int H, int W, int C, int f, cudaStream_t s);

struct DropoutArgs { uint64_t seed; uint32_t tag; uint32_t threshold; float scale; int keep_all; };
void k_dropout_fwd(int prec, const void* x, void* y, uint32_t* mask, size_t n, const DropoutArgs& a, unsigned long long* pass, unsigned* ticket, int bump_pass, cudaStream_t s);
void k_dropout_bwd(int prec, const void* eps_out, void* eps_in, const uint32_t* mask, size_t n, float scale, cudaStream_t s);

void k_xent(int prec, const void* z, const float* y, void* dz, float* loss_sums, int rows_per_group, int groups, float clip_eps, cudaStream_t s);
void k_sigmoid_out(int prec, const void* z, void* p, size_t n, cudaStream_t s);
void k_softmax_xent(int prec, const void* z, const float* y, void* dz, void* p_out, float* loss_sums, int rows, int K, cudaStream_t s);
int k_loss_blocks(size_t n_per_group, int groups);
void k_loss(int prec, int loss, int act, float alpha, const void* z, const float* y, void* dz, float* loss_sums, int rows_per_group, int n_out, int groups,
            double* partial, unsigned* ticket, cudaStream_t s);

void k_colsum(int prec, const void* x, int rows, int C, float* scratch, float* out, int accumulate, cudaStream_t s);
size_t k_colsum_scratch_floats(int C);
void k_sumsq_segments(const float* p, const int64_t* seg_off, const int64_t* seg_len, const float* seg_coef, int nseg, double* out, cudaStream_t s);
void k_reduce_splits(const float* src, float* dst, size_t n, int splits, size_t stride, int accumulate, cudaStream_t s);
struct ReduceJob { const float* src; float* dst; int64_t n, stride; int splits, blocks; };
struct ReduceList { static const int MAX_JOBS = 24; ReduceJob jobs[MAX_JOBS]; int count; };
void reduce_list_push(ReduceList* rl, const float* src, float* dst, int64_t n, int splits, int64_t stride);
void k_reduce_multi(const ReduceList& rl, cudaStream_t s);

struct UpdSeg {
  int64_t off, len;
  int kind;
  float lr, b1, b2, eps;
  float l2;
  float clip;
  int div_mb;
  int64_t off_bf, off_ps;
  int ps_O, ps_C;
};
struct UpdSched {
  int kind, type;
  int n_map;
  double initial, gamma, power, step, decay;
  const int32_t* keys; const double* vals;
};
void k_updater(float* params, const float* grads, float* st0, float* st1, float* st2, const UpdSeg* segs_dev, const int32_t* chunk_seg_dev,
               const int64_t* chunk_off_dev, int nchunks, float inv_mb, float inv_world, int* step_dev , unsigned* ticket,
               __nv_bfloat16* shadow, const float* gn_mult, const UpdSched* sched, const int64_t* epoch_dev, bool ext, cudaStream_t s);
void k_sched_lr(const UpdSeg* segs_dev, const UpdSched* sched, int seg, const int* step_dev, const int64_t* epoch_dev, float* out, cudaStream_t s);
static const int UPD_CHUNK = 4096;

struct GnGroup { int32_t chunk_begin, chunk_end, seg_begin, seg_end; };
void k_gradnorm(const float* grads, const UpdSeg* segs_dev, const int32_t* chunk_seg_dev, const int64_t* chunk_off_dev, int nchunks,
                const GnGroup* groups_dev, int ngroups, int clip, float threshold, float inv_mb, float inv_world, double* partial, unsigned* ticket,
                float* mult, cudaStream_t s);
void k_fill_f32(float* p, float v, size_t n, cudaStream_t s);
void k_scale_f32(float* p, float v, size_t n, cudaStream_t s);
struct P2pArgs { float* grads[8]; unsigned* flags[8]; int rank, world; size_t n; unsigned* state; };
void k_p2p_allreduce(const P2pArgs& a, cudaStream_t s);

void k_simt_fprop(int prec, int wprec, const ConvGeom& g, const void* x, const void* w, const float* bias, void* out, int act, float alpha, cudaStream_t s, const float* scale = nullptr);
void k_simt_dgrad(int prec, int wprec, const ConvGeom& g, const void* dy, const void* w, const float* bias, void* dx, int act, float alpha, cudaStream_t s, const float* scale = nullptr);
void k_simt_wgrad(int prec, const ConvGeom& g, const void* x, const void* dy, float* dw, float* scratch, size_t scratch_floats, int accumulate, cudaStream_t s);
size_t k_simt_wgrad_scratch_floats(const ConvGeom& g);
extern const char* g_gemm_last_kernel;
extern int g_gemm_last_splits;

bool edge_deconv_small_c_supported(const ConvGeom& g);
bool edge_conv_small_cin_supported(const ConvGeom& g);
bool edge_wgrad_small_cin_supported(const ConvGeom& g);
bool dense_small_o_supported(const ConvGeom& g);
void k_edge_deconv_small_c(int prec, int wprec, const ConvGeom& g, const void* dy, const void* w, const float* bias, void* dx, int act, float alpha, cudaStream_t s);
void k_edge_conv_small_cin(int prec, int wprec, const ConvGeom& g, const void* x, const void* w, const float* bias, void* out, int act, float alpha, cudaStream_t s);
void k_edge_wgrad_small_cin(int prec, const ConvGeom& g, const void* x, const void* dy, float* dw, float* scratch, int accumulate, cudaStream_t s);
size_t k_edge_wgrad_scratch_floats(const ConvGeom& g);
void k_dense_small_o_fwd(int prec, int wprec, const ConvGeom& g, const void* x, const void* w, const float* bias, void* out, int act, float alpha, cudaStream_t s);
void k_dense_small_o_dgrad(int prec, int wprec, const ConvGeom& g, const void* dy, const void* w, void* dx, cudaStream_t s);
void k_dense_small_o_wgrad(int prec, const ConvGeom& g, const void* x, const void* dy, float* dw, float* scratch, int accumulate, cudaStream_t s);
size_t k_dense_small_o_wgrad_scratch_floats(const ConvGeom& g);
bool dense_small_k_supported(const ConvGeom& g);
void k_dense_small_k_dgrad(int prec, int wprec, const ConvGeom& g, const void* dy, const void* w, const float* bias, void* dx, int act, float alpha, cudaStream_t s);
void k_dense_small_k_wgrad(int prec, const ConvGeom& g, const void* x, const void* dy, float* dw, cudaStream_t s);

bool tc_fprop_supported(const ConvGeom& g);
bool tc_dgrad_supported(const ConvGeom& g);
bool tc_wgrad_supported(const ConvGeom& g);
int  tc_init();
extern const char* g_tc_last_kernel;
extern int g_tc_test_bn, g_tc_test_max_ctas;
extern int g_tc_test_per_tap;
extern bool g_tc_last_slab;
enum { EPI_PLAIN = 0, EPI_STATS = 1, EPI_BNBWD = 2, EPI_ACTBWD = 3 };
struct TcEpi {
  int mode;
  const float* scale;
  unsigned long long* acc;
  int imgs_per_group;
  const __nv_bfloat16* aux;
  const __nv_bfloat16* aux2;
  int act; float alpha;
};
int k_tc_fprop(const ConvGeom& g, const __nv_bfloat16* x, const __nv_bfloat16* w, const float* bias, __nv_bfloat16* out, int act, float alpha, cudaStream_t s, const TcEpi* epi = nullptr, int w_mn = 0);
int k_tc_dgrad(const ConvGeom& g, const __nv_bfloat16* dy, const __nv_bfloat16* w, const float* bias, __nv_bfloat16* dx, int act, float alpha, cudaStream_t s, const TcEpi* epi = nullptr);
int k_tc_wgrad(const ConvGeom& g, const __nv_bfloat16* x, const __nv_bfloat16* dy, float* dw, float* scratch, size_t scratch_floats, int accumulate, cudaStream_t s, ReduceList* defer = nullptr);
size_t k_tc_wgrad_scratch_floats(const ConvGeom& g);
bool tc_deconv_ps_shape(const ConvGeom& g);
bool tc_deconv_ps_supported(const ConvGeom& g);
size_t k_tc_deconv_ps_weight_elems(const ConvGeom& g);
void k_pack_deconv_ps(const float* w, __nv_bfloat16* wps, int O, int C, cudaStream_t s);
bool tc_edge_conv_supported(const ConvGeom& g);
bool tc_edge_wgrad_supported(const ConvGeom& g);
size_t k_tc_edge_wgrad_scratch_floats(const ConvGeom& g);
int k_tc_edge_conv(const ConvGeom& g, const __nv_bfloat16* x, const __nv_bfloat16* w, const float* bias, __nv_bfloat16* out, int act, float alpha, cudaStream_t s);
int k_tc_edge_wgrad(const ConvGeom& g, const __nv_bfloat16* x, const __nv_bfloat16* dy, float* dw, float* db, float* scratch, size_t scratch_floats, int accumulate, cudaStream_t s, ReduceList* defer = nullptr);
int k_tc_deconv_ps(const ConvGeom& g, const __nv_bfloat16* dy, const __nv_bfloat16* wps, const float* bias, __nv_bfloat16* dx, int act, float alpha, cudaStream_t s, const TcEpi* epi = nullptr);

}
```

gan_deeplearning4j_b200/csrc/kernels_tc.cu:

```cuda
#include <cuda.h>
#include <stdio.h>
#include <stdlib.h>
#include <algorithm>

#include "common.cuh"
#include "kernels.h"

namespace b2g {

typedef CUresult (*PFN_encodeTiled)(CUtensorMap*, CUtensorMapDataType, cuuint32_t, void*, const cuuint64_t*, const cuuint64_t*, const cuuint32_t*,
                                    const cuuint32_t*, CUtensorMapInterleave, CUtensorMapSwizzle, CUtensorMapL2promotion, CUtensorMapFloatOOBfill);
static PFN_encodeTiled g_encode = nullptr;

int tc_init() {
  if (g_encode) return 0;
  void* fn = nullptr; cudaDriverEntryPointQueryResult q;
  if (cudaGetDriverEntryPoint("cuTensorMapEncodeTiled", &fn, cudaEnableDefault, &q) != cudaSuccess || !fn || q != cudaDriverEntryPointSuccess) return -1;
  g_encode = (PFN_encodeTiled)fn; return 0;
}

static int make_map_bf16(CUtensorMap* m, const void* base, int rank, const cuuint64_t* dims, const cuuint64_t* strides_bytes, const cuuint32_t* box, const cuuint32_t* estr) {
  if (!g_encode) return -1;
  CUresult r = g_encode(m, CU_TENSOR_MAP_DATA_TYPE_BFLOAT16, (cuuint32_t)rank, const_cast<void*>(base), dims, strides_bytes, box, estr, CU_TENSOR_MAP_INTERLEAVE_NONE,
                        CU_TENSOR_MAP_SWIZZLE_128B, CU_TENSOR_MAP_L2_PROMOTION_L2_256B, CU_TENSOR_MAP_FLOAT_OOB_FILL_NONE);
  if (r != CUDA_SUCCESS) { fprintf(stderr, "[b200gan] cuTensorMapEncodeTiled failed: %d (rank %d)\n", (int)r, rank); return -1; }
  return 0;
}

__device__ __forceinline__ uint32_t smem_u32(const void* p) { return (uint32_t)__cvta_generic_to_shared(p); }
__device__ __forceinline__ void mbar_init(uint32_t bar, uint32_t count) { asm volatile("mbarrier.init.shared::cta.b64 [%0], %1;" ::"r"(bar), "r"(count)); }
__device__ __forceinline__ void fence_mbar_init() { asm volatile("fence.mbarrier_init.release.cluster;" ::: "memory"); }
__device__ __forceinline__ void mbar_expect_tx(uint32_t bar, uint32_t bytes) { asm volatile("mbarrier.arrive.expect_tx.shared::cta.b64 _, [%0], %1;" ::"r"(bar), "r"(bytes) : "memory"); }
__device__ __forceinline__ void mbar_arrive(uint32_t bar) { asm volatile("mbarrier.arrive.shared::cta.b64 _, [%0];" ::"r"(bar) : "memory"); }
__device__ int g_tc_timeout_flag = 0;
__device__ __forceinline__ void mbar_wait(uint32_t bar, uint32_t parity) {
  uint32_t done = 0;
  for (uint32_t it = 0; it < (1u << 26); ++it) {
    asm volatile("{\n\t.reg .pred p;\n\tmbarrier.try_wait.parity.shared::cta.b64 p, [%1], %2;\n\tselp.u32 %0, 1, 0, p;\n\t}" : "=r"(done) : "r"(bar), "r"(parity) : "memory");
    if (done) return;
  }
  g_tc_timeout_flag = 1; __trap();
}
__device__ __forceinline__ void tma_load_4d(uint32_t dst, const CUtensorMap* map, uint32_t bar, int c0, int c1, int c2, int c3) {
  asm volatile("cp.async.bulk.tensor.4d.shared::cluster.global.tile.mbarrier::complete_tx::bytes [%0], [%1, {%3, %4, %5, %6}], [%2];"
               ::"r"(dst), "l"(map), "r"(bar), "r"(c0), "r"(c1), "r"(c2), "r"(c3) : "memory");
}
__device__ __forceinline__ void tma_load_3d(uint32_t dst, const CUtensorMap* map, uint32_t bar, int c0, int c1, int c2) {
  asm volatile("cp.async.bulk.tensor.3d.shared::cluster.global.tile.mbarrier::complete_tx::bytes [%0], [%1, {%3, %4, %5}], [%2];"
               ::"r"(dst), "l"(map), "r"(bar), "r"(c0), "r"(c1), "r"(c2) : "memory");
}
__device__ __forceinline__ void tma_load_2d(uint32_t dst, const CUtensorMap* map, uint32_t bar, int c0, int c1) {
  asm volatile("cp.async.bulk.tensor.2d.shared::cluster.global.tile.mbarrier::complete_tx::bytes [%0], [%1, {%3, %4}], [%2];"
               ::"r"(dst), "l"(map), "r"(bar), "r"(c0), "r"(c1) : "memory");
}
__device__ __forceinline__ bool elect_one_sync() {
  uint32_t pred = 0;
  asm volatile("{\n\t.reg .pred P1;\n\t.reg .b32 rx;\n\telect.sync rx|P1, %1;\n\t@P1 mov.s32 %0, 1;\n\t}" : "+r"(pred) : "r"(0xffffffffu));
  return pred != 0;
}
__device__ __forceinline__ void prefetch_map(const CUtensorMap* map) { asm volatile("prefetch.tensormap [%0];" ::"l"(map) : "memory"); }
__device__ __forceinline__ void fence_proxy_async_smem() { asm volatile("fence.proxy.async.shared::cta;" ::: "memory"); }

__device__ __forceinline__ uint64_t gmma_desc(uint32_t saddr, uint32_t lbo_bytes) {
  return (uint64_t)((saddr & 0x3FFFFu) >> 4) | ((uint64_t)((lbo_bytes >> 4) & 0x3FFF) << 16) | ((uint64_t)(1024 >> 4) << 32) | (1ull << 62);
}
__device__ __forceinline__ uint64_t desc_kmajor_sw128(uint32_t saddr) { return gmma_desc(saddr, 16); }
__device__ __forceinline__ uint64_t desc_mnmajor_sw128(uint32_t saddr, uint32_t lbo_bytes) { return gmma_desc(saddr, lbo_bytes); }

__device__ __forceinline__ void wg_fence() { asm volatile("wgmma.fence.sync.aligned;" ::: "memory"); }
__device__ __forceinline__ void wg_commit() { asm volatile("wgmma.commit_group.sync.aligned;" ::: "memory"); }
template <int N>
__device__ __forceinline__ void wg_wait() { asm volatile("wgmma.wait_group.sync.aligned %0;" ::"n"(N) : "memory"); }

template <int TA, int TB>
__device__ __forceinline__ void wgmma_n64(float (&d)[32], uint64_t da, uint64_t db) {
  asm volatile(
      "wgmma.mma_async.sync.aligned.m64n64k16.f32.bf16.bf16 "
      "{%0, %1, %2, %3, %4, %5, %6, %7, %8, %9, %10, %11, %12, %13, %14, %15, %16, %17, %18, %19, %20, %21, %22, %23, %24, %25, %26, %27, %28, %29, %30, %31}, "
      "%32, %33, 1, 1, 1, %34, %35;"
      : "+f"(d[0]), "+f"(d[1]), "+f"(d[2]), "+f"(d[3]), "+f"(d[4]), "+f"(d[5]), "+f"(d[6]), "+f"(d[7]), "+f"(d[8]), "+f"(d[9]), "+f"(d[10]),
        "+f"(d[11]), "+f"(d[12]), "+f"(d[13]), "+f"(d[14]), "+f"(d[15]), "+f"(d[16]), "+f"(d[17]), "+f"(d[18]), "+f"(d[19]), "+f"(d[20]),
        "+f"(d[21]), "+f"(d[22]), "+f"(d[23]), "+f"(d[24]), "+f"(d[25]), "+f"(d[26]), "+f"(d[27]), "+f"(d[28]), "+f"(d[29]), "+f"(d[30]), "+f"(d[31])
      : "l"(da), "l"(db), "n"(TA), "n"(TB));
}
template <int TA, int TB>
__device__ __forceinline__ void wgmma_n128(float (&d0)[32], float (&d1)[32], uint64_t da, uint64_t db) {
  asm volatile(
      "wgmma.mma_async.sync.aligned.m64n128k16.f32.bf16.bf16 "
      "{%0, %1, %2, %3, %4, %5, %6, %7, %8, %9, %10, %11, %12, %13, %14, %15, %16, %17, %18, %19, %20, %21, %22, %23, %24, %25, %26, %27, %28, %29, %30, %31, %32, %33, %34, %35, %36, %37, %38, %39, %40, %41, %42, %43, %44, %45, %46, %47, %48, %49, %50, %51, %52, %53, %54, %55, %56, %57, %58, %59, %60, %61, %62, %63}, "
      "%64, %65, 1, 1, 1, %66, %67;"
      : "+f"(d0[0]), "+f"(d0[1]), "+f"(d0[2]), "+f"(d0[3]), "+f"(d0[4]), "+f"(d0[5]), "+f"(d0[6]), "+f"(d0[7]), "+f"(d0[8]), "+f"(d0[9]), "+f"(d0[10]), "+f"(d0[11]), "+f"(d0[12]), "+f"(d0[13]), "+f"(d0[14]), "+f"(d0[15]), "+f"(d0[16]), "+f"(d0[17]), "+f"(d0[18]), "+f"(d0[19]), "+f"(d0[20]), "+f"(d0[21]), "+f"(d0[22]), "+f"(d0[23]), "+f"(d0[24]), "+f"(d0[25]), "+f"(d0[26]), "+f"(d0[27]), "+f"(d0[28]), "+f"(d0[29]), "+f"(d0[30]), "+f"(d0[31]),
        "+f"(d1[0]), "+f"(d1[1]), "+f"(d1[2]), "+f"(d1[3]), "+f"(d1[4]), "+f"(d1[5]), "+f"(d1[6]), "+f"(d1[7]), "+f"(d1[8]), "+f"(d1[9]), "+f"(d1[10]), "+f"(d1[11]), "+f"(d1[12]), "+f"(d1[13]), "+f"(d1[14]), "+f"(d1[15]), "+f"(d1[16]), "+f"(d1[17]), "+f"(d1[18]), "+f"(d1[19]), "+f"(d1[20]), "+f"(d1[21]), "+f"(d1[22]), "+f"(d1[23]), "+f"(d1[24]), "+f"(d1[25]), "+f"(d1[26]), "+f"(d1[27]), "+f"(d1[28]), "+f"(d1[29]), "+f"(d1[30]), "+f"(d1[31])
      : "l"(da), "l"(db), "n"(TA), "n"(TB));
}
__device__ __forceinline__ void wgmma_n16(float (&d)[8], uint64_t da, uint64_t db) {
  asm volatile(
      "wgmma.mma_async.sync.aligned.m64n16k16.f32.bf16.bf16 {%0, %1, %2, %3, %4, %5, %6, %7}, %8, %9, 1, 1, 1, 0, 0;"
      : "+f"(d[0]), "+f"(d[1]), "+f"(d[2]), "+f"(d[3]), "+f"(d[4]), "+f"(d[5]), "+f"(d[6]), "+f"(d[7])
      : "l"(da), "l"(db));
}



struct TcConvParams {
  int mode;
  int Nt, Ht, Wt;
  int GH, GW;
  int tiles_y;
  int taps_h, taps_w;
  int slab_bytes;
  int a_wg_bytes;
  int a_tap_bytes;
  int chunks;
  int KW, SH, SW, PH, PW;
  int OC;
  int outH, outW;
  int b_mn;
  const float* bias; const float* scale; int act; float alpha;
  __nv_bfloat16* out;
  int epi;
  unsigned long long* acc;
  int imgs_per_group;
  const __nv_bfloat16* aux;
  const __nv_bfloat16* aux2;
  int tiles_m, tiles_n, phases;
};

static constexpr int TC_THREADS = 384;
static constexpr int TC_CONV_THREADS = 640;
static constexpr int SLAB_ROWS = 144;
template <int BN, int STAGES, int EPI = EPI_PLAIN, bool SLAB = false>
struct TcSmem {
  static constexpr int A_BYTES = (SLAB ? SLAB_ROWS : 128) * 128;
  static constexpr int B_BYTES = (SLAB ? 2 : 1) * BN * 128;
  static constexpr int STAGE_BYTES = A_BYTES + B_BYTES;
  static constexpr int RING_BYTES = STAGES * STAGE_BYTES;
  static constexpr int ACC_PITCH = BN + 4;
  static constexpr int PARK_BYTES = 128 * ACC_PITCH * 4;
  static constexpr int PARKS = BN >= 128 ? 1 : 2;
  static constexpr int PARK_OFF = RING_BYTES;
  static constexpr int BAR_OFF = PARK_OFF + PARKS * PARK_BYTES;
  static constexpr int STAT_OFF = BAR_OFF + 256;
  static constexpr int STG_OFF = STAT_OFF + ((EPI == EPI_STATS || EPI == EPI_BNBWD) ? 4 * 2 * BN * 4 : 0);
  static constexpr int TOTAL = STG_OFF + (BN >= 32 ? 8 * 2048 : 0) + 1024;
  static_assert(TOTAL <= 227 * 1024, "one CTA per SM must fit the shared memory of an sm_90 SM");
};

__device__ __forceinline__ void epi_bar_sync() { asm volatile("bar.sync 1, 256;" ::: "memory"); }
template <int N> __device__ __forceinline__ void setmaxnreg_inc() { asm volatile("setmaxnreg.inc.sync.aligned.u32 %0;" ::"n"(N)); }
template <int N> __device__ __forceinline__ void setmaxnreg_dec() { asm volatile("setmaxnreg.dec.sync.aligned.u32 %0;" ::"n"(N)); }

template <int OFF>
__device__ __forceinline__ void warp_colsum_level(float (&a)[32], int lane) {
  const bool up = (lane & OFF) != 0;
#pragma unroll
  for (int j = 0; j < OFF; ++j) {
    const float lo = a[j], hi = a[j + OFF];
    const float send = up ? lo : hi, keep = up ? hi : lo;
    a[j] = keep + __shfl_xor_sync(0xffffffffu, send, OFF);
  }
  if constexpr (OFF > 1) warp_colsum_level<OFF / 2>(a, lane);
}
__device__ __forceinline__ void warp_colsum32(float (&a)[32], int lane) { warp_colsum_level<16>(a, lane); }

template <int BN, int EPI, bool AFFINE>
__device__ __forceinline__ void epi_tile(const TcConvParams& p, const float* srow, size_t roff, int nb0, int group, float* sst, uint4* stg, int q, int lane, int ep_tid,
                                         int c_beg, int c_end) {
  constexpr bool stats = EPI == EPI_STATS || EPI == EPI_BNBWD;
  const bool has_bias = p.bias != nullptr;
  const int sub = lane >> 2, cq = lane & 3, sx = (lane >> 1) & 3;
  size_t roff_i[4];
#pragma unroll
  for (int i = 0; i < 4; ++i) roff_i[i] = __shfl_sync(0xffffffffu, (unsigned long long)roff, i * 8 + sub) + cq * 8;
#pragma unroll 1
  for (int c0 = c_beg; c0 < c_end; c0 += 32) {
    uint32_t v[32];
    uint4 gy[4], gz[4], ax[4], az[4];
    if constexpr (EPI >= EPI_BNBWD) {
#pragma unroll
      for (int i = 0; i < 4; ++i) gy[i] = *reinterpret_cast<const uint4*>(p.aux + roff_i[i] + c0);
    }
    if constexpr (EPI == EPI_BNBWD) {
#pragma unroll
      for (int i = 0; i < 4; ++i) gz[i] = *reinterpret_cast<const uint4*>(p.aux2 + roff_i[i] + c0);
    }
    if constexpr (EPI >= EPI_BNBWD) {
#pragma unroll
      for (int i = 0; i < 4; ++i) { const int r = i * 8 + sub; stg[r * 4 + (cq ^ ((r >> 1) & 3))] = gy[i]; }
      __syncwarp();
#pragma unroll
      for (int j = 0; j < 4; ++j) ax[j] = stg[lane * 4 + (j ^ sx)];
      __syncwarp();
    }
    if constexpr (EPI == EPI_BNBWD) {
#pragma unroll
      for (int i = 0; i < 4; ++i) { const int r = i * 8 + sub; stg[r * 4 + (cq ^ ((r >> 1) & 3))] = gz[i]; }
      __syncwarp();
#pragma unroll
      for (int j = 0; j < 4; ++j) az[j] = stg[lane * 4 + (j ^ sx)];
      __syncwarp();
    }
#pragma unroll
    for (int j = 0; j < 8; ++j) { const uint4 t = reinterpret_cast<const uint4*>(srow + c0)[j]; v[4 * j] = t.x; v[4 * j + 1] = t.y; v[4 * j + 2] = t.z; v[4 * j + 3] = t.w; }
    float o[32], s2[32];
    if constexpr (EPI == EPI_BNBWD) {
      const __nv_bfloat162* yb = reinterpret_cast<const __nv_bfloat162*>(ax);
      const __nv_bfloat162* zb = reinterpret_cast<const __nv_bfloat162*>(az);
#define B2G_BNBWD_LOOP(ACTC)                                                                                                   \
  _Pragma("unroll") for (int j = 0; j < 16; ++j) {                                                                             \
    const float2 y2 = __bfloat1622float2(yb[j]), z2 = __bfloat1622float2(zb[j]);                                               \
    o[2 * j] = __uint_as_float(v[2 * j]) * act_grad_from_out(ACTC, y2.x, p.alpha);                                             \
    o[2 * j + 1] = __uint_as_float(v[2 * j + 1]) * act_grad_from_out(ACTC, y2.y, p.alpha);                                     \
    s2[2 * j] = z2.x; s2[2 * j + 1] = z2.y;                                                                                    \
  }
      if (p.act == ACT_LRELU) { B2G_BNBWD_LOOP(ACT_LRELU) }
      else if (p.act == ACT_RELU) { B2G_BNBWD_LOOP(ACT_RELU) }
      else { B2G_BNBWD_LOOP(p.act) }
#undef B2G_BNBWD_LOOP
    } else if constexpr (EPI == EPI_ACTBWD) {
      const __nv_bfloat162* ab = reinterpret_cast<const __nv_bfloat162*>(ax);
#define B2G_ACTBWD_LOOP(ACTC)                                                                                                  \
  _Pragma("unroll") for (int j = 0; j < 16; ++j) {                                                                             \
    const float2 a2 = __bfloat1622float2(ab[j]);                                                                               \
    o[2 * j] = __uint_as_float(v[2 * j]) * act_grad_from_out(ACTC, a2.x, p.alpha);                                             \
    o[2 * j + 1] = __uint_as_float(v[2 * j + 1]) * act_grad_from_out(ACTC, a2.y, p.alpha);                                     \
  }
      if (p.act == ACT_LRELU) { B2G_ACTBWD_LOOP(ACT_LRELU) }
      else if (p.act == ACT_TANH) { B2G_ACTBWD_LOOP(ACT_TANH) }
      else { B2G_ACTBWD_LOOP(p.act) }
#undef B2G_ACTBWD_LOOP
    } else {
#define B2G_EPI_LOOP(ACTC)                                                                                                     \
  _Pragma("unroll") for (int j = 0; j < 32; ++j) {                                                                             \
    float a = __uint_as_float(v[j]);                                                                                           \
    if (AFFINE) a = fmaf(a, p.scale[nb0 + c0 + j], p.bias[nb0 + c0 + j]);                                                      \
    else if (has_bias) a += p.bias[nb0 + c0 + j];                                                                              \
    o[j] = act_fwd(ACTC, a, p.alpha);                                                                                          \
  }
      if (p.act == ACT_IDENTITY) { B2G_EPI_LOOP(ACT_IDENTITY) }
      else if (p.act == ACT_LRELU) { B2G_EPI_LOOP(ACT_LRELU) }
      else if (p.act == ACT_RELU) { B2G_EPI_LOOP(ACT_RELU) }
      else { B2G_EPI_LOOP(p.act) }
#undef B2G_EPI_LOOP
    }
    uint32_t packed[16];
#pragma unroll
    for (int j = 0; j < 16; ++j) {
      __nv_bfloat162 h = __floats2bfloat162_rn(o[2 * j], o[2 * j + 1]);
      packed[j] = *reinterpret_cast<uint32_t*>(&h);
      if constexpr (stats) { const float2 r = __bfloat1622float2(h); o[2 * j] = r.x; o[2 * j + 1] = r.y; }
    }
#pragma unroll
    for (int j = 0; j < 4; ++j) stg[lane * 4 + (j ^ sx)] = make_uint4(packed[4 * j], packed[4 * j + 1], packed[4 * j + 2], packed[4 * j + 3]);
    __syncwarp();
#pragma unroll
    for (int i = 0; i < 4; ++i) { const int r = i * 8 + sub; *reinterpret_cast<uint4*>(p.out + roff_i[i] + c0) = stg[r * 4 + (cq ^ ((r >> 1) & 3))]; }
    __syncwarp();
    if constexpr (stats) {
      if constexpr (EPI == EPI_STATS) {
#pragma unroll
        for (int j = 0; j < 32; ++j) s2[j] = o[j] * o[j];
      } else {
#pragma unroll
        for (int j = 0; j < 32; ++j) s2[j] = o[j] * s2[j];
      }
      warp_colsum32(o, lane); warp_colsum32(s2, lane);
      sst[(q * 2 + 0) * BN + c0 + lane] = o[0];
      sst[(q * 2 + 1) * BN + c0 + lane] = s2[0];
    }
  }
  if constexpr (stats) {
    epi_bar_sync();
    for (int col = ep_tid; col < BN; col += 256) {
#pragma unroll
      for (int st = 0; st < 2; ++st) {
        const float s = ((sst[(0 * 2 + st) * BN + col] + sst[(1 * 2 + st) * BN + col]) + sst[(2 * 2 + st) * BN + col]) + sst[(3 * 2 + st) * BN + col];
        sacc_add(p.acc + (size_t)(group * 2 + st) * 2 * p.OC, (size_t)p.OC, (size_t)(nb0 + col), s);
      }
    }
  }
}

template <int BN>
__device__ __forceinline__ void load_b_tile(const TcConvParams& p, const CUtensorMap* tmB, uint32_t dst, uint32_t bar, int ch, int wtap, int nb0) {
  if (!p.b_mn) tma_load_3d(dst, tmB, bar, ch * 64, wtap, nb0);
  else {
#pragma unroll
    for (int j = 0; j < (BN >= 64 ? BN / 64 : 1); ++j) tma_load_3d(dst + j * 8192, tmB, bar, nb0 + j * 64, wtap, ch * 64);
  }
}
template <int BN, int NB, int NACC>
__device__ __forceinline__ void mma_kblock(float (&acc)[NB][NACC], uint32_t a_smem, uint32_t b_smem, int b_mn) {
  const uint64_t adesc = desc_kmajor_sw128(a_smem);
  if constexpr (BN < 64) {
    const uint64_t bdesc = desc_kmajor_sw128(b_smem);
#pragma unroll
    for (int k = 0; k < 4; ++k) wgmma_n16(acc[0], adesc + 2 * k, bdesc + 2 * k);
  } else if constexpr (NB == 2) {
    if (!b_mn) {
#pragma unroll
      for (int k = 0; k < 4; ++k) wgmma_n128<0, 0>(acc[0], acc[1], adesc + 2 * k, desc_kmajor_sw128(b_smem) + 2 * k);
    } else {
#pragma unroll
      for (int k = 0; k < 4; ++k) wgmma_n128<0, 1>(acc[0], acc[1], adesc + 2 * k, desc_mnmajor_sw128(b_smem + k * 2048, 8192));
    }
  } else if (!b_mn) {
#pragma unroll
    for (int k = 0; k < 4; ++k) wgmma_n64<0, 0>(acc[0], adesc + 2 * k, desc_kmajor_sw128(b_smem) + 2 * k);
  } else {
#pragma unroll
    for (int k = 0; k < 4; ++k) wgmma_n64<0, 1>(acc[0], adesc + 2 * k, desc_mnmajor_sw128(b_smem + k * 2048, 8192));
  }
}
__device__ __forceinline__ void tap_coords(const TcConvParams& p, int ta, int tb, int py, int px, int& ax, int& dy_, int& wtap) {
  if (p.mode == 0) { dy_ = -p.PH + ta; ax = -p.PW + tb; wtap = ta * p.KW + tb; }
  else {
    const int r = py == 0 ? (ta == 0 ? 1 : 3) : (ta == 0 ? 0 : 2), dyr = py == 0 ? (ta == 0 ? 0 : -1) : (ta == 0 ? 1 : 0);
    const int sx = px == 0 ? (tb == 0 ? 1 : 3) : (tb == 0 ? 0 : 2), dxc = px == 0 ? (tb == 0 ? 0 : -1) : (tb == 0 ? 1 : 0);
    dy_ = dyr; ax = dxc; wtap = r * 4 + sx;
  }
}
__device__ __forceinline__ void slab_coords(const TcConvParams& p, int ta, int tb, int py, int px, int& ax, int& dy_, int& wlo, int& whi) {
  int ax2, dy2;
  tap_coords(p, p.mode == 0 ? ta : 1, tb, py, px, ax, dy_, wlo);
  tap_coords(p, p.mode == 0 ? ta + 2 : 0, tb, py, px, ax2, dy2, whi);
}

template <int BN>
struct TcConvRegs {
  static constexpr int LAUNCH = 96, PRODUCER = 24, MMA = BN >= 128 ? 96 : 64, EPI = BN >= 128 ? 128 : 160;
  static_assert(PRODUCER + 2 * MMA + 2 * EPI <= 5 * LAUNCH, "setmaxnreg budget exceeds the launch allocation");
};
template <int BN, int STAGES, int EPI, bool AFFINE, bool PS = false, bool SLAB = false>
__global__ void __launch_bounds__(TC_CONV_THREADS, 1) tc_conv_kernel(const __grid_constant__ CUtensorMap tmA, const __grid_constant__ CUtensorMap tmB, const TcConvParams p) {
  using S = TcSmem<BN, STAGES, EPI, SLAB>;
  using R = TcConvRegs<BN>;
  constexpr int NB = BN >= 64 ? BN / 64 : 1, NACC = BN >= 64 ? 32 : BN / 2;
  extern __shared__ uint8_t smem_raw[];
  const uint32_t smem_base = (smem_u32(smem_raw) + 1023u) & ~1023u;
  uint8_t* smem_gen = smem_raw + (smem_base - smem_u32(smem_raw));
  const uint32_t bar_full = smem_base + S::BAR_OFF;
  const uint32_t bar_empty = bar_full + 8 * STAGES;
  const uint32_t park_full = bar_empty + 8 * STAGES;
  const uint32_t park_empty = park_full + 8 * S::PARKS;
  float* sst = reinterpret_cast<float*>(smem_gen + S::STAT_OFF);
  const int warp = threadIdx.x >> 5, lane = threadIdx.x & 31;
  const int num_kb = p.taps_h * p.taps_w * p.chunks;
  const int tiles = p.tiles_m * p.tiles_n * p.phases;
  auto tile_coords = [&](int t, int& nb0, int& phase, int& n0, int& y0) {
    const int mt = t % p.tiles_m, r = t / p.tiles_m;
    nb0 = (r % p.tiles_n) * BN; phase = r / p.tiles_n;
    if (p.Nt > 1) { n0 = mt * p.Nt; y0 = 0; } else { n0 = mt / p.tiles_y; y0 = (mt % p.tiles_y) * p.Ht; }
  };

  if (threadIdx.x == 0) {
    prefetch_map(&tmA); prefetch_map(&tmB);
    for (int s = 0; s < STAGES; ++s) { mbar_init(bar_full + 8 * s, 1); mbar_init(bar_empty + 8 * s, 8); }
    for (int k = 0; k < S::PARKS; ++k) { mbar_init(park_full + 8 * k, 256); mbar_init(park_empty + 8 * k, 256); }
    fence_mbar_init();
  }
  __syncthreads();
  pdl_wait();

  if (warp >= 16) {
    setmaxnreg_dec<R::PRODUCER>();
    if (warp == 16) {
      int s = 0; uint32_t ph = 0;
      for (int t = blockIdx.x; t < tiles; t += gridDim.x) {
        int nb0, phase, n0, y0; tile_coords(t, nb0, phase, n0, y0);
        const int py = phase >> 1, px = phase & 1;
        const int ybase = p.mode == 0 ? y0 * p.SH : y0;
        int ch = 0, ta = 0, tb = 0;
        int ax, dy_, wtap, wtap2 = 0;
        auto coords = [&]() { if constexpr (SLAB) slab_coords(p, ta, tb, py, px, ax, dy_, wtap, wtap2); else tap_coords(p, ta, tb, py, px, ax, dy_, wtap); };
        coords();
        for (int kb = 0; kb < num_kb; ++kb) {
          mbar_wait(bar_empty + 8 * s, ph ^ 1);
          if (elect_one_sync()) {
            const uint32_t st = smem_base + s * S::STAGE_BYTES;
            mbar_expect_tx(bar_full + 8 * s, SLAB ? p.slab_bytes + S::B_BYTES : S::STAGE_BYTES);
            tma_load_4d(st, &tmA, bar_full + 8 * s, ch * 64, ax, ybase + dy_, n0);
            load_b_tile<BN>(p, &tmB, st + S::A_BYTES, bar_full + 8 * s, ch, wtap, nb0);
            if constexpr (SLAB) load_b_tile<BN>(p, &tmB, st + S::A_BYTES + BN * 128, bar_full + 8 * s, ch, wtap2, nb0);
          }
          __syncwarp();
          if (++s == STAGES) { s = 0; ph ^= 1; }
          if (++ch == p.chunks) { ch = 0; if (++tb == p.taps_w) { tb = 0; ++ta; } coords(); }
        }
      }
    }
  } else if (warp < 8) {
    if constexpr (R::MMA < R::LAUNCH) setmaxnreg_dec<R::MMA>();
    const int wg = warp >> 2;
    const int r0 = wg * 64 + (warp & 3) * 16 + (lane >> 2);
    int s = 0, k = 0; uint32_t ph = 0, kph = 0;
    for (int t = blockIdx.x; t < tiles; t += gridDim.x) {
      float acc[NB][NACC];
#pragma unroll
      for (int nb = 0; nb < NB; ++nb)
#pragma unroll
        for (int j = 0; j < NACC; ++j) acc[nb][j] = 0.f;
      int prev = -1;
      for (int kb = 0; kb < num_kb; ++kb) {
        mbar_wait(bar_full + 8 * s, ph);
        wg_fence();
        const uint32_t st = smem_base + s * S::STAGE_BYTES;
        if constexpr (SLAB) {
          const uint32_t a = st + wg * p.a_wg_bytes;
          mma_kblock<BN, NB, NACC>(acc, a, st + S::A_BYTES, p.b_mn);
          mma_kblock<BN, NB, NACC>(acc, a + p.a_tap_bytes, st + S::A_BYTES + BN * 128, p.b_mn);
        } else {
          mma_kblock<BN, NB, NACC>(acc, st + wg * 8192, st + S::A_BYTES, PS ? 0 : p.b_mn);
        }
        wg_commit();
        wg_wait<1>();
        if (prev >= 0 && lane == 0) mbar_arrive(bar_empty + 8 * prev);
        prev = s;
        if (++s == STAGES) { s = 0; ph ^= 1; }
      }
      wg_wait<0>();
      if (lane == 0) mbar_arrive(bar_empty + 8 * prev);
      mbar_wait(park_empty + 8 * k, kph ^ 1);
      float* park = reinterpret_cast<float*>(smem_gen + S::PARK_OFF + k * S::PARK_BYTES);
#pragma unroll
      for (int nb = 0; nb < NB; ++nb)
#pragma unroll
        for (int j = 0; j < NACC / 4; ++j) {
          const int col = nb * 64 + j * 8 + 2 * (lane & 3);
          *reinterpret_cast<float2*>(park + r0 * S::ACC_PITCH + col) = make_float2(acc[nb][4 * j], acc[nb][4 * j + 1]);
          *reinterpret_cast<float2*>(park + (r0 + 8) * S::ACC_PITCH + col) = make_float2(acc[nb][4 * j + 2], acc[nb][4 * j + 3]);
        }
      mbar_arrive(park_full + 8 * k);
      if (++k == S::PARKS) { k = 0; kph ^= 1; }
    }
  } else {
    setmaxnreg_inc<R::EPI>();
    const int ew = warp - 8, q = ew & 3, half = ew >> 2;
    const int row = q * 32 + lane;
    const int img = row / (p.Ht * p.Wt), rem = row % (p.Ht * p.Wt), yy = rem / p.Wt, xx = rem % p.Wt;
    int k = 0; uint32_t kph = 0;
    for (int t = blockIdx.x; t < tiles; t += gridDim.x) {
      int nb0, phase, n0, y0; tile_coords(t, nb0, phase, n0, y0);
      const int py = phase >> 1, px = phase & 1;
      const int n = n0 + img, gy = y0 + yy, gx = xx;
      mbar_wait(park_full + 8 * k, kph);
      const float* srow = reinterpret_cast<const float*>(smem_gen + S::PARK_OFF + k * S::PARK_BYTES) + row * S::ACC_PITCH;
      if constexpr (PS) {
        if (half == 0) {
          const int C = p.OC;
#pragma unroll
          for (int ppy = 0; ppy < 2; ++ppy) {
            const size_t doff = (((size_t)n * p.outH + 2 * gy + ppy) * p.outW + 2 * gx) * C;
            __nv_bfloat16* dst = p.out + doff;
            float o[8];
#pragma unroll
            for (int ppx = 0; ppx < 2; ++ppx)
#pragma unroll
              for (int c = 0; c < 4; ++c) {
                float a = srow[(ppy * 2 + ppx) * 4 + c];
                if constexpr (EPI == EPI_ACTBWD) { if (c < C) a *= act_grad_from_out(p.act, __bfloat162float(p.aux[doff + ppx * C + c]), p.alpha); }
                else { if (p.bias && c < C) a += p.bias[c]; a = act_fwd(p.act, a, p.alpha); }
                o[ppx * 4 + c] = a;
              }
            if (C == 3) {
              __nv_bfloat162 h0 = __floats2bfloat162_rn(o[0], o[1]), h1 = __floats2bfloat162_rn(o[2], o[4]), h2 = __floats2bfloat162_rn(o[5], o[6]);
              uint32_t* d32 = reinterpret_cast<uint32_t*>(dst);
              d32[0] = *reinterpret_cast<uint32_t*>(&h0); d32[1] = *reinterpret_cast<uint32_t*>(&h1); d32[2] = *reinterpret_cast<uint32_t*>(&h2);
            } else {
#pragma unroll
              for (int ppx = 0; ppx < 2; ++ppx)
#pragma unroll
                for (int c = 0; c < 4; ++c) if (c < C) dst[ppx * C + c] = __float2bfloat16(o[ppx * 4 + c]);
            }
          }
        }
      } else {
        size_t pix;
        if (p.mode == 0) pix = ((size_t)n * p.outH + gy) * p.outW + gx;
        else pix = ((size_t)n * p.outH + 2 * gy + py) * p.outW + 2 * gx + px;
        const int group = p.imgs_per_group > 0 ? n0 / p.imgs_per_group : 0;
        epi_tile<BN, EPI, AFFINE>(p, srow, pix * p.OC + nb0, nb0, group, sst, reinterpret_cast<uint4*>(smem_gen + S::STG_OFF) + ew * 128, q, lane,
                                  (int)threadIdx.x - 256, half * (BN / 2), (half + 1) * (BN / 2));
        if constexpr (EPI == EPI_STATS || EPI == EPI_BNBWD) epi_bar_sync();
      }
      mbar_arrive(park_empty + 8 * k);
      if (++k == S::PARKS) { k = 0; kph ^= 1; }
    }
  }
}

const char* g_tc_last_kernel = "";
bool g_tc_last_slab = false;
int g_tc_test_bn = 0, g_tc_test_max_ctas = 0, g_tc_test_per_tap = 0;
static int tc_device() { int dev = 0; cudaGetDevice(&dev); return dev < 0 || dev >= 64 ? 0 : dev; }
#define TC_SET_SMEM_ONCE(kernel, bytes)                                                                                            \
  do { static bool set_[64] = {}; const int d_ = tc_device();                                                                       \
       if (!set_[d_]) { if (cudaFuncSetAttribute(kernel, cudaFuncAttributeMaxDynamicSharedMemorySize, (int)(bytes)) != cudaSuccess) return -2; set_[d_] = true; } } while (0)

static bool pick_row_tile(int N, int GH, int GW, int rows, int* Nt, int* Ht, int* Wt) {
  const int P = GH * GW;
  if (GW > rows || rows % GW) return false;
  if (P >= rows) { if (P % rows) return false; *Nt = 1; *Ht = rows / GW; *Wt = GW; return GH % *Ht == 0; }
  if (rows % P || N % (rows / P)) return false;
  *Nt = rows / P; *Ht = GH; *Wt = GW; return true;
}
static int pick_bn(int OC) { return OC % 128 == 0 ? 128 : OC % 64 == 0 ? 64 : 0; }
static int pick_bn_fill(int OC, long m_tiles_x_phases) {
  if (g_tc_test_bn) return g_tc_test_bn;
  const int target = device_sm_count();
  int bn = pick_bn(OC);
  while (bn > 64 && m_tiles_x_phases * (OC / bn) < target) bn /= 2;
  return bn;
}

bool tc_fprop_supported(const ConvGeom& g) {
  int a, b, c;
  return g.C % 64 == 0 && pick_bn(g.O) != 0 && g.SH >= 1 && g.SH <= 2 && g.SW == g.SH && g.KH * g.KW * (g.C / 64) >= 1 &&
         pick_row_tile(g.N, g.OH, g.OW, 128, &a, &b, &c) && c * g.SW <= 256 && b * g.SH <= 256 && g.N >= 1;
}
bool tc_dgrad_supported(const ConvGeom& g) {
  int a, b, c;
  return g.KH == 4 && g.KW == 4 && g.SH == 2 && g.SW == 2 && g.PH == 1 && g.PW == 1 && g.O % 64 == 0 && pick_bn(g.C) != 0 && g.H == 2 * g.OH && g.W == 2 * g.OW &&
         pick_row_tile(g.N, g.OH, g.OW, 128, &a, &b, &c);
}
static bool tc_epi_ok(const TcEpi* e, int Nt) { return !e || e->mode == EPI_PLAIN || e->mode == EPI_ACTBWD || (e->imgs_per_group > 0 && e->imgs_per_group % Nt == 0 && e->acc); }

template <int BN, int STAGES, int EPI, bool AFFINE, bool PS = false, bool SLAB = false>
static int launch_conv_e(const CUtensorMap& tmA, const CUtensorMap& tmB, const TcConvParams& p, cudaStream_t s) {
  using S = TcSmem<BN, STAGES, EPI, SLAB>;
  TC_SET_SMEM_ONCE((tc_conv_kernel<BN, STAGES, EPI, AFFINE, PS, SLAB>), S::TOTAL);
  const long tiles = (long)p.tiles_m * p.tiles_n * p.phases;
  const unsigned grid = (unsigned)std::min<long>(tiles, g_tc_test_max_ctas > 0 ? g_tc_test_max_ctas : device_sm_count());
  launch_pdl(tc_conv_kernel<BN, STAGES, EPI, AFFINE, PS, SLAB>, dim3(grid), dim3(TC_CONV_THREADS), (size_t)(S::TOTAL), s, tmA, tmB, p);
  LAUNCHED();
  return cudaPeekAtLastError() == cudaSuccess ? 0 : -3;
}
template <int BN, int STAGES, bool SLAB>
static int launch_conv(const CUtensorMap& tmA, const CUtensorMap& tmB, const TcConvParams& p, cudaStream_t s, const char* name) {
  g_tc_last_kernel = name; g_tc_last_slab = SLAB;
  switch (p.epi) {
    case EPI_STATS: return launch_conv_e<BN, STAGES, EPI_STATS, false, false, SLAB>(tmA, tmB, p, s);
    case EPI_BNBWD: return launch_conv_e<BN, STAGES, EPI_BNBWD, false, false, SLAB>(tmA, tmB, p, s);
    case EPI_ACTBWD: return launch_conv_e<BN, STAGES, EPI_ACTBWD, false, false, SLAB>(tmA, tmB, p, s);
  }
  return (p.scale && p.bias) ? launch_conv_e<BN, STAGES, EPI_PLAIN, true, false, SLAB>(tmA, tmB, p, s) : launch_conv_e<BN, STAGES, EPI_PLAIN, false, false, SLAB>(tmA, tmB, p, s);
}
static int dispatch_conv(int BN, bool slab, const CUtensorMap& tmA, const CUtensorMap& tmB, const TcConvParams& p, cudaStream_t s) {
  switch (BN * 2 + slab) {
    case 128: return launch_conv<64, 4, false>(tmA, tmB, p, s, "tc_conv_kernel<64,4>");
    case 256: return launch_conv<128, 4, false>(tmA, tmB, p, s, "tc_conv_kernel<128,4>");
    case 129: return launch_conv<64, 4, true>(tmA, tmB, p, s, "tc_conv_kernel<64,4>");
  }
  return -4;
}
static bool slab_tile(const TcConvParams& p, int BN) {
  if (g_tc_test_per_tap || BN != 64 || p.Wt % 8) return false;
  if (!((p.Nt == 1 && p.Ht >= 2) || (p.Nt == 2 && p.Ht * p.Wt == 64))) return false;
  return p.Nt * (p.Ht + 1) * p.Wt <= SLAB_ROWS;
}
static bool is_k4s2p1_geom(const ConvGeom& g) { return g.KH == 4 && g.KW == 4 && g.SH == 2 && g.SW == 2 && g.PH == 1 && g.PW == 1 && g.H == 2 * g.OH && g.W == 2 * g.OW; }
static void set_slab(TcConvParams& p) {
  p.taps_h = p.mode == 0 ? 2 : 1;
  p.slab_bytes = p.Nt * (p.Ht + 1) * p.Wt * 128;
  p.a_wg_bytes = p.Nt == 1 ? 64 * 128 : (p.Ht + 1) * p.Wt * 128;
  p.a_tap_bytes = p.Wt * 128;
}

static int weight_map(CUtensorMap* m, const __nv_bfloat16* w, int rows, int taps, int inner, int box_rows) {
  cuuint64_t dims[3] = {(cuuint64_t)inner, (cuuint64_t)taps, (cuuint64_t)rows};
  cuuint64_t strides[2] = {(cuuint64_t)inner * 2, (cuuint64_t)taps * inner * 2};
  cuuint32_t box[3] = {64, 1, (cuuint32_t)box_rows}; cuuint32_t es[3] = {1, 1, 1};
  return make_map_bf16(m, w, 3, dims, strides, box, es);
}
static void fill_epi(TcConvParams& p, const float* bias, int act, float alpha, const TcEpi* e) {
  p.bias = bias; p.act = act; p.alpha = alpha; p.epi = EPI_PLAIN;
  if (!e) return;
  p.scale = e->scale; p.epi = e->mode; p.acc = e->acc; p.imgs_per_group = e->mode == EPI_STATS || e->mode == EPI_BNBWD ? e->imgs_per_group : 0;
  p.aux = e->aux; p.aux2 = e->aux2;
  if (e->mode == EPI_BNBWD || e->mode == EPI_ACTBWD) { p.act = e->act; p.alpha = e->alpha; p.bias = nullptr; p.scale = nullptr; }
}

int k_tc_fprop(const ConvGeom& g, const __nv_bfloat16* x, const __nv_bfloat16* w, const float* bias, __nv_bfloat16* out, int act, float alpha, cudaStream_t s, const TcEpi* epi, int w_mn) {
  TcConvParams p{}; p.mode = 0;
  if (!pick_row_tile(g.N, g.OH, g.OW, 128, &p.Nt, &p.Ht, &p.Wt) || !tc_epi_ok(epi, p.Nt)) return -1;
  if (w_mn && (g.KH != 1 || g.KW != 1)) return -1;
  const int BN = pick_bn_fill(g.O, (long)g.N * g.OH * g.OW / 128);
  p.GH = g.OH; p.GW = g.OW; p.tiles_y = g.OH / p.Ht; p.taps_h = g.KH; p.taps_w = g.KW; p.chunks = g.C / 64; p.KW = g.KW;
  p.SH = g.SH; p.SW = g.SW; p.PH = g.PH; p.PW = g.PW; p.OC = g.O; p.outH = g.OH; p.outW = g.OW; p.out = out; p.b_mn = w_mn;
  fill_epi(p, bias, act, alpha, epi);
  const bool slab = is_k4s2p1_geom(g) && !w_mn && slab_tile(p, BN);
  if (slab) set_slab(p);
  CUtensorMap tmA, tmB;
  cuuint64_t dims[4] = {(cuuint64_t)g.C, (cuuint64_t)g.W, (cuuint64_t)g.H, (cuuint64_t)g.N};
  cuuint64_t strides[3] = {(cuuint64_t)g.C * 2, (cuuint64_t)g.W * g.C * 2, (cuuint64_t)g.H * g.W * g.C * 2};
  cuuint32_t box[4] = {64, (cuuint32_t)(p.Wt * g.SW), (cuuint32_t)((p.Ht + slab) * g.SH), (cuuint32_t)p.Nt};
  cuuint32_t es[4] = {1, (cuuint32_t)g.SW, (cuuint32_t)g.SH, 1};
  if (make_map_bf16(&tmA, x, 4, dims, strides, box, es)) return -1;
  p.tiles_m = g.N * g.OH * g.OW / 128; p.tiles_n = g.O / BN; p.phases = 1;
  if (w_mn ? weight_map(&tmB, w, g.C, 1, g.O, 64) : weight_map(&tmB, w, g.O, g.KH * g.KW, g.C, BN)) return -1;
  return dispatch_conv(BN, slab, tmA, tmB, p, s);
}

int k_tc_dgrad(const ConvGeom& g, const __nv_bfloat16* dy, const __nv_bfloat16* w, const float* bias, __nv_bfloat16* dx, int act, float alpha, cudaStream_t s, const TcEpi* epi) {
  TcConvParams p{}; p.mode = 1;
  if (!pick_row_tile(g.N, g.OH, g.OW, 128, &p.Nt, &p.Ht, &p.Wt) || !tc_epi_ok(epi, p.Nt)) return -1;
  const int BN = pick_bn_fill(g.C, (long)g.N * g.OH * g.OW / 128 * 4);
  p.GH = g.OH; p.GW = g.OW; p.tiles_y = g.OH / p.Ht; p.taps_h = 2; p.taps_w = 2; p.chunks = g.O / 64; p.KW = 4;
  p.SH = 1; p.SW = 1; p.PH = 0; p.PW = 0; p.OC = g.C; p.outH = g.H; p.outW = g.W; p.out = dx; p.b_mn = 1;
  fill_epi(p, bias, act, alpha, epi);
  const bool slab = slab_tile(p, BN);
  if (slab) set_slab(p);
  CUtensorMap tmA, tmB;
  cuuint64_t dims[4] = {(cuuint64_t)g.O, (cuuint64_t)g.OW, (cuuint64_t)g.OH, (cuuint64_t)g.N};
  cuuint64_t strides[3] = {(cuuint64_t)g.O * 2, (cuuint64_t)g.OW * g.O * 2, (cuuint64_t)g.OH * g.OW * g.O * 2};
  cuuint32_t box[4] = {64, (cuuint32_t)p.Wt, (cuuint32_t)(p.Ht + slab), (cuuint32_t)p.Nt};
  cuuint32_t es[4] = {1, 1, 1, 1};
  if (weight_map(&tmB, w, g.O, 16, g.C, 64)) return -1;
  if (make_map_bf16(&tmA, dy, 4, dims, strides, box, es)) return -1;
  p.tiles_m = g.N * g.OH * g.OW / 128; p.tiles_n = g.C / BN; p.phases = 4;
  return dispatch_conv(BN, slab, tmA, tmB, p, s);
}

bool tc_deconv_ps_shape(const ConvGeom& g) { return is_k4s2p1_geom(g) && g.C >= 1 && g.C <= 4 && g.O % 64 == 0; }
bool tc_deconv_ps_supported(const ConvGeom& g) { int a, b, c; return tc_deconv_ps_shape(g) && pick_row_tile(g.N, g.OH, g.OW, 128, &a, &b, &c); }
size_t k_tc_deconv_ps_weight_elems(const ConvGeom& g) { return tc_deconv_ps_shape(g) ? (size_t)16 * 9 * g.O : 0; }
__global__ void pack_deconv_ps_kernel(const float* __restrict__ w, __nv_bfloat16* __restrict__ wps, int O, int C) { pdl_wait();
  const int idx = blockIdx.x * blockDim.x + threadIdx.x; if (idx >= 16 * 9 * O) return;
  const int o = idx % O, t = (idx / O) % 9, n = idx / (9 * O);
  const int py = n >> 3, px = (n >> 2) & 1, c = n & 3, dyr = t / 3 - 1, dxc = t % 3 - 1;
  const int r = dyr == -1 ? (py == 0 ? 3 : -1) : dyr == 0 ? (py == 0 ? 1 : 2) : (py == 1 ? 0 : -1);
  const int sx = dxc == -1 ? (px == 0 ? 3 : -1) : dxc == 0 ? (px == 0 ? 1 : 2) : (px == 1 ? 0 : -1);
  wps[idx] = __float2bfloat16((r >= 0 && sx >= 0 && c < C) ? w[((size_t)o * 16 + r * 4 + sx) * C + c] : 0.f);
}
void k_pack_deconv_ps(const float* w, __nv_bfloat16* wps, int O, int C, cudaStream_t s) {
  launch_pdl(pack_deconv_ps_kernel, dim3((16 * 9 * O + 255) / 256), dim3(256), (size_t)(0), s, w, wps, O, C); LAUNCHED();
}
int k_tc_deconv_ps(const ConvGeom& g, const __nv_bfloat16* dy, const __nv_bfloat16* wps, const float* bias, __nv_bfloat16* dx, int act, float alpha, cudaStream_t s, const TcEpi* epi) {
  TcConvParams p{}; p.mode = 0;
  if (!tc_deconv_ps_shape(g) || !pick_row_tile(g.N, g.OH, g.OW, 128, &p.Nt, &p.Ht, &p.Wt)) return -1;
  if (epi && epi->mode != EPI_PLAIN && epi->mode != EPI_ACTBWD) return -1;
  p.GH = g.OH; p.GW = g.OW; p.tiles_y = g.OH / p.Ht; p.taps_h = 3; p.taps_w = 3; p.chunks = g.O / 64; p.KW = 3;
  p.SH = 1; p.SW = 1; p.PH = 1; p.PW = 1; p.OC = g.C; p.outH = g.H; p.outW = g.W; p.out = dx;
  fill_epi(p, bias, act, alpha, epi);
  CUtensorMap tmA, tmB;
  cuuint64_t dims[4] = {(cuuint64_t)g.O, (cuuint64_t)g.OW, (cuuint64_t)g.OH, (cuuint64_t)g.N};
  cuuint64_t strides[3] = {(cuuint64_t)g.O * 2, (cuuint64_t)g.OW * g.O * 2, (cuuint64_t)g.OH * g.OW * g.O * 2};
  cuuint32_t box[4] = {64, (cuuint32_t)p.Wt, (cuuint32_t)p.Ht, (cuuint32_t)p.Nt}; cuuint32_t es[4] = {1, 1, 1, 1};
  if (make_map_bf16(&tmA, dy, 4, dims, strides, box, es)) return -1;
  if (weight_map(&tmB, wps, 16, 9, g.O, 16)) return -1;
  p.tiles_m = (int)((long)g.N * g.OH * g.OW / 128); p.tiles_n = 1; p.phases = 1;
  g_tc_last_kernel = "tc_conv_kernel<16,4,PS>";
  return p.epi == EPI_ACTBWD ? launch_conv_e<16, 4, EPI_ACTBWD, false, true>(tmA, tmB, p, s) : launch_conv_e<16, 4, EPI_PLAIN, false, true>(tmA, tmB, p, s);
}

struct TcEdgeParams {
  const __nv_bfloat16* x; const __nv_bfloat16* w; const __nv_bfloat16* dy; const float* bias; __nv_bfloat16* out; float* part; float* part_b;
  int N, H, W, C, OH, OW, O, Ht, tiles_y, tiles_total, tiles_per_cta, act; float alpha;
};
static constexpr int EDGE_SLAB_BYTES = 6144;
__device__ __forceinline__ uint32_t swz128(int row, int byte) { return (uint32_t)(row * 128 + ((((byte >> 4) ^ (row & 7)) << 4) | (byte & 15))); }

struct EdgeSlabRegs { uint4 v[3]; };
__device__ __forceinline__ void edge_fetch_slab(const TcEdgeParams& p, int n, int oy0, EdgeSlabRegs& r) {
  const int WC = p.W * p.C, cpr = WC >> 3, total = (2 * p.Ht + 2) * cpr;
#pragma unroll
  for (int q = 0; q < 3; ++q) {
    const int i = threadIdx.x + q * 128; r.v[q] = make_uint4(0u, 0u, 0u, 0u);
    if (i < total) { const int j = i / cpr, cc = i - j * cpr, iy = 2 * oy0 - 1 + j;
      if (iy >= 0 && iy < p.H) r.v[q] = __ldg(reinterpret_cast<const uint4*>(p.x + ((size_t)n * p.H + iy) * WC) + cc); }
  }
}
__device__ __forceinline__ void edge_store_slab(const TcEdgeParams& p, const EdgeSlabRegs& r, uint8_t* slab) {
  const int total = (2 * p.Ht + 2) * ((p.W * p.C) >> 3);
#pragma unroll
  for (int q = 0; q < 3; ++q) { const int i = threadIdx.x + q * 128; if (i < total) reinterpret_cast<uint4*>(slab)[i] = r.v[q]; }
}
template <int C>
__device__ __forceinline__ void edge_build_row_c(const TcEdgeParams& p, const uint8_t* slab, uint8_t* tile, int row, bool ones) {
  const int WC = p.W * C, oy_l = row / p.OW, ox = row - oy_l * p.OW;
  const int lo = ox == 0 ? C : 0, hi = ox == p.OW - 1 ? 3 * C : 4 * C;
  uint32_t out[32];
#pragma unroll
  for (int i = 0; i < 32; ++i) out[i] = 0u;
#pragma unroll
  for (int r = 0; r < 4; ++r) {
    const int b0 = ((2 * oy_l + r) * WC + (2 * ox - 1) * C) * 2;
    if (C & 1) {
      const uint32_t* wp = reinterpret_cast<const uint32_t*>(slab + b0 - 2);
      uint32_t w[2 * C + 1];
#pragma unroll
      for (int i = 0; i <= 2 * C; ++i) w[i] = wp[i];
#pragma unroll
      for (int i = 0; i < 2 * C; ++i) out[r * 2 * C + i] = __funnelshift_r(w[i], w[i + 1], 16);
    } else {
      const uint32_t* wp = reinterpret_cast<const uint32_t*>(slab + b0);
#pragma unroll
      for (int i = 0; i < 2 * C; ++i) out[r * 2 * C + i] = wp[i];
    }
#pragma unroll
    for (int i = 0; i < 2 * C; ++i) {
      const uint32_t m = ((2 * i >= lo && 2 * i < hi) ? 0xFFFFu : 0u) | ((2 * i + 1 >= lo && 2 * i + 1 < hi) ? 0xFFFF0000u : 0u);
      out[r * 2 * C + i] &= m;
    }
  }
  if (C < 4 && ones) out[8 * C] = 0x3F80u;
#pragma unroll
  for (int cc = 0; cc < 8; ++cc) *reinterpret_cast<uint4*>(tile + row * 128 + ((cc ^ (row & 7)) << 4)) = make_uint4(out[4 * cc], out[4 * cc + 1], out[4 * cc + 2], out[4 * cc + 3]);
}
__device__ __forceinline__ void edge_build_row(const TcEdgeParams& p, const uint8_t* slab, uint8_t* tile, int row, bool ones = false) {
  switch (p.C) { case 1: edge_build_row_c<1>(p, slab, tile, row, ones); break; case 2: edge_build_row_c<2>(p, slab, tile, row, ones); break;
                 case 3: edge_build_row_c<3>(p, slab, tile, row, ones); break; default: edge_build_row_c<4>(p, slab, tile, row, ones); break; }
}


__global__ void __launch_bounds__(128) tc_edge_conv_kernel(const TcEdgeParams p) { pdl_wait();
  extern __shared__ uint8_t smem_raw[];
  const uint32_t smem_base = (smem_u32(smem_raw) + 1023u) & ~1023u;
  uint8_t* sm = smem_raw + (smem_base - smem_u32(smem_raw));
  uint8_t* sA = sm; uint8_t* sB = sm + 16384; uint8_t* slab = sm + 24576;
  const int tid = threadIdx.x, warp = tid >> 5, lane = tid & 31;
  const int nb0 = blockIdx.y * 64, K = 16 * p.C;
  const int t_beg = blockIdx.x * p.tiles_per_cta, t_end = min(p.tiles_total, t_beg + p.tiles_per_cta);
  EdgeSlabRegs pre;
  if (t_beg < t_end) edge_fetch_slab(p, t_beg / p.tiles_y, (t_beg % p.tiles_y) * p.Ht, pre);
  {
    uint4 wv[4];
#pragma unroll
    for (int q = 0; q < 4; ++q) { const int i = tid + q * 128, o = i >> 3, cc = i & 7;
      wv[q] = cc < 2 * p.C ? __ldg(reinterpret_cast<const uint4*>(p.w + (size_t)(nb0 + o) * K) + cc) : make_uint4(0u, 0u, 0u, 0u); }
#pragma unroll
    for (int q = 0; q < 4; ++q) { const int i = tid + q * 128, o = i >> 3, cc = i & 7; *reinterpret_cast<uint4*>(sB + o * 128 + ((cc ^ (o & 7)) << 4)) = wv[q]; }
  }
  const bool has_bias = p.bias != nullptr;
  const int r0 = warp * 16 + (lane >> 2), cq = lane & 3;
  for (int t = t_beg; t < t_end; ++t) {
    const int n = t / p.tiles_y, oy0 = (t % p.tiles_y) * p.Ht;
    edge_store_slab(p, pre, slab);
    __syncthreads();
    if (t + 1 < t_end) edge_fetch_slab(p, (t + 1) / p.tiles_y, ((t + 1) % p.tiles_y) * p.Ht, pre);
    edge_build_row(p, slab, sA, tid);
    fence_proxy_async_smem();
    __syncthreads();
    float acc[2][32];
#pragma unroll
    for (int h = 0; h < 2; ++h)
#pragma unroll
      for (int j = 0; j < 32; ++j) acc[h][j] = 0.f;
    wg_fence();
    {
      const uint64_t bdesc = desc_kmajor_sw128(smem_base + 16384);
#pragma unroll
      for (int k = 0; k < 4; ++k)
#pragma unroll
        for (int h = 0; h < 2; ++h) wgmma_n64<0, 0>(acc[h], desc_kmajor_sw128(smem_base + h * 8192) + 2 * k, bdesc + 2 * k);
    }
    wg_commit();
    wg_wait<0>();
    __syncthreads();
#pragma unroll
    for (int h = 0; h < 2; ++h)
#pragma unroll
      for (int i = 0; i < 2; ++i) {
        const int row = h * 64 + r0 + 8 * i;
#pragma unroll
        for (int j = 0; j < 8; ++j) {
          const int col = j * 8 + 2 * cq;
          float a = acc[h][4 * j + 2 * i], b = acc[h][4 * j + 2 * i + 1];
          if (has_bias) { a += p.bias[nb0 + col]; b += p.bias[nb0 + col + 1]; }
          __nv_bfloat162 v = __floats2bfloat162_rn(act_fwd(p.act, a, p.alpha), act_fwd(p.act, b, p.alpha));
          *reinterpret_cast<__nv_bfloat162*>(sA + row * 128 + ((j ^ (row & 7)) << 4) + cq * 4) = v;
        }
      }
    __syncthreads();
    __nv_bfloat16* obase = p.out + ((size_t)n * p.OH + oy0) * p.OW * p.O + nb0;
#pragma unroll
    for (int i = 0; i < 8; ++i) {
      const int idx = tid + i * 128, r = idx >> 3, cc = idx & 7;
      *reinterpret_cast<uint4*>(obase + (size_t)r * p.O + cc * 8) = *reinterpret_cast<const uint4*>(sA + r * 128 + ((cc ^ (r & 7)) << 4));
    }
  }
}

__global__ void __launch_bounds__(128) tc_edge_wgrad_kernel(const TcEdgeParams p) { pdl_wait();
  extern __shared__ uint8_t smem_raw[];
  const uint32_t smem_base = (smem_u32(smem_raw) + 1023u) & ~1023u;
  uint8_t* sm = smem_raw + (smem_base - smem_u32(smem_raw));
  uint8_t* sDy = sm; uint8_t* sX = sm + 16384; uint8_t* slab = sm + 32768;
  const int tid = threadIdx.x, warp = tid >> 5, lane = tid & 31, K = 16 * p.C;
  const int t_beg = blockIdx.x * p.tiles_per_cta, t_end = min(p.tiles_total, t_beg + p.tiles_per_cta);
  float acc[32];
#pragma unroll
  for (int j = 0; j < 32; ++j) acc[j] = 0.f;
  EdgeSlabRegs pre; uint4 dyr[8];
  auto fetch = [&](int t) {
    const int n = t / p.tiles_y, oy0 = (t % p.tiles_y) * p.Ht;
    edge_fetch_slab(p, n, oy0, pre);
    const uint4* dyt = reinterpret_cast<const uint4*>(p.dy + (((size_t)n * p.OH + oy0) * p.OW) * 64);
#pragma unroll
    for (int i = 0; i < 8; ++i) dyr[i] = __ldg(dyt + tid + i * 128);
  };
  if (t_beg < t_end) fetch(t_beg);
  for (int t = t_beg; t < t_end; ++t) {
    edge_store_slab(p, pre, slab);
#pragma unroll
    for (int i = 0; i < 8; ++i) { const int idx = tid + i * 128, r = idx >> 3, cc = idx & 7; *reinterpret_cast<uint4*>(sDy + r * 128 + ((cc ^ (r & 7)) << 4)) = dyr[i]; }
    __syncthreads();
    if (t + 1 < t_end) fetch(t + 1);
    edge_build_row(p, slab, sX, tid, p.part_b != nullptr);
    fence_proxy_async_smem();
    __syncthreads();
    wg_fence();
#pragma unroll
    for (int k = 0; k < 8; ++k)
      wgmma_n64<1, 1>(acc, desc_mnmajor_sw128(smem_base + k * 2048, 8192), desc_mnmajor_sw128(smem_base + 16384 + k * 2048, 8192));
    wg_commit();
    wg_wait<0>();
    __syncthreads();
  }
#pragma unroll
  for (int i = 0; i < 2; ++i) {
    const int o = warp * 16 + (lane >> 2) + 8 * i;
    float* orow = p.part + ((size_t)blockIdx.x * 64 + o) * K;
#pragma unroll
    for (int j = 0; j < 8; ++j) {
      const int col = j * 8 + 2 * (lane & 3);
      if (col < K) *reinterpret_cast<float2*>(orow + col) = make_float2(acc[4 * j + 2 * i], acc[4 * j + 2 * i + 1]);
      else if (col == K && p.part_b) p.part_b[(size_t)blockIdx.x * 64 + o] = acc[4 * j + 2 * i];
    }
  }
}

static bool edge_tile(const ConvGeom& g, int* Ht) {
  if (!is_k4s2p1_geom(g) || g.C < 1 || g.C > 4 || g.OW > 128 || 128 % g.OW) return false;
  const int ht = 128 / g.OW;
  if (g.OH % ht || (g.W * g.C) % 8 || (2 * ht + 2) * g.W * g.C * 2 > EDGE_SLAB_BYTES) return false;
  *Ht = ht; return true;
}
bool tc_edge_conv_supported(const ConvGeom& g) { int ht; return edge_tile(g, &ht) && g.O % 64 == 0; }
bool tc_edge_wgrad_supported(const ConvGeom& g) { int ht; return edge_tile(g, &ht) && g.O == 64; }
static int tc_edge_wgrad_target() { return 2 * device_sm_count(); }
static int tc_edge_wgrad_ctas(const ConvGeom& g, int* tpc) {
  int ht = 1; edge_tile(g, &ht);
  const int tiles = g.N * (g.OH / ht), target = tc_edge_wgrad_target();
  const int per = (tiles + target - 1) / target; *tpc = per < 1 ? 1 : per;
  return (tiles + *tpc - 1) / *tpc;
}
size_t k_tc_edge_wgrad_scratch_floats(const ConvGeom& g) { return tc_edge_wgrad_supported(g) ? (size_t)tc_edge_wgrad_target() * (64 * 16 * g.C + 64) : 0; }
int k_tc_edge_conv(const ConvGeom& g, const __nv_bfloat16* x, const __nv_bfloat16* w, const float* bias, __nv_bfloat16* out, int act, float alpha, cudaStream_t s) {
  TcEdgeParams p{}; if (!edge_tile(g, &p.Ht) || g.O % 64) return -1;
  if ((reinterpret_cast<uintptr_t>(x) & 15) || (reinterpret_cast<uintptr_t>(w) & 15) || (reinterpret_cast<uintptr_t>(out) & 15)) return -1;
  p.x = x; p.w = w; p.bias = bias; p.out = out; p.N = g.N; p.H = g.H; p.W = g.W; p.C = g.C; p.OH = g.OH; p.OW = g.OW; p.O = g.O; p.tiles_y = g.OH / p.Ht;
  p.tiles_total = g.N * p.tiles_y; p.act = act; p.alpha = alpha;
  const size_t smem = 1024 + 24576 + EDGE_SLAB_BYTES;
  TC_SET_SMEM_ONCE(tc_edge_conv_kernel, smem);
  const int target = 8 * device_sm_count();
  p.tiles_per_cta = (p.tiles_total + target - 1) / target;
  launch_pdl(tc_edge_conv_kernel, dim3(dim3((unsigned)((p.tiles_total + p.tiles_per_cta - 1) / p.tiles_per_cta), (unsigned)(g.O / 64))), dim3(128), (size_t)(smem), s, p);
  LAUNCHED(); g_tc_last_kernel = "tc_edge_conv_kernel";
  return cudaPeekAtLastError() == cudaSuccess ? 0 : -3;
}
static void reduce_or_defer(ReduceList* defer, const float* src, float* dst, size_t n, int splits, size_t stride, int accumulate, cudaStream_t s);
int k_tc_edge_wgrad(const ConvGeom& g, const __nv_bfloat16* x, const __nv_bfloat16* dy, float* dw, float* db, float* scratch, size_t scratch_floats, int accumulate, cudaStream_t s, ReduceList* defer) {
  TcEdgeParams p{}; if (!edge_tile(g, &p.Ht) || g.O != 64) return -1;
  if ((reinterpret_cast<uintptr_t>(x) & 15) || (reinterpret_cast<uintptr_t>(dy) & 15)) return -1;
  p.x = x; p.dy = dy; p.part = scratch; p.N = g.N; p.H = g.H; p.W = g.W; p.C = g.C; p.OH = g.OH; p.OW = g.OW; p.O = g.O; p.tiles_y = g.OH / p.Ht;
  p.tiles_total = g.N * p.tiles_y;
  const int ctas = tc_edge_wgrad_ctas(g, &p.tiles_per_cta); const size_t n = (size_t)64 * 16 * g.C;
  if ((size_t)ctas * (n + 64) > scratch_floats) return -5;
  if (db && g.C < 4) p.part_b = scratch + (size_t)ctas * n;
  const size_t smem = 1024 + 32768 + EDGE_SLAB_BYTES;
  TC_SET_SMEM_ONCE(tc_edge_wgrad_kernel, smem);
  launch_pdl(tc_edge_wgrad_kernel, dim3(dim3((unsigned)ctas)), dim3(128), (size_t)(smem), s, p);
  LAUNCHED(); g_tc_last_kernel = "tc_edge_wgrad_kernel";
  if (cudaPeekAtLastError() != cudaSuccess) return -3;
  reduce_or_defer(defer, scratch, dw, n, ctas, n, accumulate, s);
  if (p.part_b) reduce_or_defer(defer, p.part_b, db, 64, ctas, 64, accumulate, s);
  return p.part_b ? 1 : 0;
}

struct TcWgradParams {
  int Nt, Ht, Wt;
  int tiles_y;
  int KW, SH, SW, PH, PW;
  int taps, C;
  int kb_total, kb_per_split;
  float* out; size_t split_stride;
};

template <int BNW, int STAGES>
struct TcWgradSmem {
  static constexpr int A_BYTES = 2 * 64 * 128;
  static constexpr int B_BYTES = (BNW / 64) * 64 * 128;
  static constexpr int STAGE_BYTES = A_BYTES + B_BYTES;
  static constexpr int BAR_OFF = STAGES * STAGE_BYTES;
  static constexpr int TOTAL = BAR_OFF + 256 + 1024;
};

template <int BNW, int STAGES>
__global__ void __launch_bounds__(TC_THREADS, 1) tc_wgrad_kernel(const __grid_constant__ CUtensorMap tmDy, const __grid_constant__ CUtensorMap tmX, const TcWgradParams p) {
  using S = TcWgradSmem<BNW, STAGES>;
  constexpr int NB = BNW / 64;
  extern __shared__ uint8_t smem_raw[];
  const uint32_t smem_base = (smem_u32(smem_raw) + 1023u) & ~1023u;
  const uint32_t bar_full = smem_base + S::BAR_OFF, bar_empty = bar_full + 8 * STAGES;
  const int warp = threadIdx.x >> 5, lane = threadIdx.x & 31;
  const int split = blockIdx.x, col0 = blockIdx.y * BNW, o0 = blockIdx.z * 128;
  const int kb_beg = split * p.kb_per_split, kb_end = min(p.kb_total, kb_beg + p.kb_per_split);
  const int num_kb = max(0, kb_end - kb_beg);

  if (threadIdx.x == 0) {
    prefetch_map(&tmDy); prefetch_map(&tmX);
    for (int s = 0; s < STAGES; ++s) { mbar_init(bar_full + 8 * s, 1); mbar_init(bar_empty + 8 * s, 8); }
    fence_mbar_init();
  }
  __syncthreads();
  pdl_trigger();
  pdl_wait();

  if (warp == 0) {
    int xc[NB], xw[NB], xh[NB];
#pragma unroll
    for (int j = 0; j < NB; ++j) { const int col = col0 + j * 64, tap = col / p.C; xc[j] = col % p.C; xw[j] = -p.PW + tap % p.KW; xh[j] = -p.PH + tap / p.KW; }
    int n0, y0;
// ... 112 lines not shown
```

gan_deeplearning4j_b200/engine.py:

```python
from __future__ import annotations

import copy
import ctypes as C
import math
from typing import Dict, List, Optional, Sequence

import numpy as np

from . import _lib
from ._lib import GanConfig, LayerDesc, LrSchedule, NetConfig, check

LAYER_TYPES = {"conv2d": 0, "deconv2d": 1, "batchnorm": 2, "dense": 3, "activation": 4, "maxpool": 5, "upsample2d": 6,
               "output": 7, "loss": 8, "ff_to_cnn": 9, "cnn_to_ff": 10, "dropout": 11}
ACTS = {"identity": 0, "tanh": 1, "sigmoid": 2, "relu": 3, "lrelu": 4}
LOSSES = {"xent": 0, "mcxent": 1, "mse": 2, "l1": 3, "l2": 4, "mae": 5, "hinge": 6, "squared_hinge": 7, "wasserstein": 8}
UPDATERS = {"sgd": 0, "rmsprop": 1, "adam": 2, "noop": 3, "nesterovs": 4, "adagrad": 5, "adamax": 6, "nadam": 7, "amsgrad": 8, "adadelta": 9}
NO_LR_UPDATERS = ("noop", "adadelta")
GRADIENT_NORMALIZATIONS = {"none": 0, "renormalize_l2_per_layer": 1, "renormalize_l2_per_param_type": 2, "clip_l2_per_layer": 4,
                           "clip_l2_per_param_type": 5}
SCHEDULE_KINDS = {"exponential": 1, "inverse": 2, "sigmoid": 3, "step": 4, "map": 5}
SCHEDULE_TYPES = {"iteration": 0, "epoch": 1}
FP32, BF16 = 0, 1


# ... 133 lines not shown

    def device_info(self):
        sm, mj, mn, mem = C.c_int32(), C.c_int32(), C.c_int32(), C.c_uint64()
        check(self.lib.b2g_device_info(self.h, C.byref(sm), C.byref(mj), C.byref(mn), C.byref(mem)))
        return dict(sm_count=sm.value, cc=(mj.value, mn.value), mem_bytes=mem.value)

    def comm_init(self, world: int, rank: int, unique_id: bytes):
        buf = C.create_string_buffer(unique_id, 128)
        check(self.lib.b2g_ctx_comm_init(self.h, world, rank, C.cast(buf, C.c_void_p)))
        self.world, self.rank = world, rank

    def allreduce_test(self, a: np.ndarray) -> np.ndarray:
        a = _f32(a).copy()
        check(self.lib.b2g_ctx_allreduce_test(self.h, _fp(a), a.size))
        return a

    def close(self):
        if self.h:
            self.lib.b2g_ctx_destroy(self.h)
            self.h = None


def comm_unique_id() -> bytes:
    buf = C.create_string_buffer(128)
    check(_lib.load().b2g_comm_unique_id(C.cast(buf, C.c_void_p)))
    return buf.raw


class Net:

    def __init__(self, ctx: Context, specs: Sequence[Dict], input_shape, max_batch: int, precision: int = FP32,
                 grad_clip: float = 0.0, xent_clip_eps: float = 1e-5, bn_groups: int = 1, seed: int = 666,
                 gradient_normalization: str = "none", gradient_normalization_threshold: float = 1.0):
        self.ctx, self.lib, self.specs = ctx, ctx.lib, copy.deepcopy(list(specs))
        self.lr_constants = [constant_lr((sp.get("updater") or {}).get("lr", 0.0)) for sp in self.specs]
        c, h, w = input_shape if len(input_shape) == 3 else (input_shape[0], 1, 1)
        self.input_shape = tuple(input_shape)
        cfg = NetConfig(h, w, c, max_batch, precision, grad_clip, xent_clip_eps, bn_groups, seed)
        arr = (LayerDesc * len(specs))(*[layer_desc(s) for s in specs])
        hnd = C.c_void_p()
        check(self.lib.b2g_net_create(ctx.h, C.byref(cfg), arr, len(specs), C.byref(hnd)))
        self.h = hnd
        self.max_batch, self.precision = max_batch, precision
        n = C.c_int64()
        check(self.lib.b2g_net_num_params(self.h, C.byref(n)))
        self.n_params = n.value
        check(self.lib.b2g_net_output_size(self.h, C.byref(n)))
        self.out_elems = n.value
        try:
            if gradient_normalization != "none":
                self.set_gradient_normalization(gradient_normalization, gradient_normalization_threshold)
            for sp in self.specs:
                lr = (sp.get("updater") or {}).get("lr", 0.0)
                if is_schedule(lr) and layer_has_lr(sp):
                    self.set_lr_schedule(lr, sp["name"])
        except Exception:
            self.close()
            raise

    def num_params(self) -> int:
        return self.n_params

    def set_param(self, layer: str, name: str, value):
        v = _f32(value).ravel()
        check(self.lib.b2g_net_set_param(self.h, layer.encode(), name.encode(), _fp(v), v.size))

    def get_param(self, layer: str, name: str, size: int) -> np.ndarray:
        out = np.empty(size, np.float32)
        check(self.lib.b2g_net_get_param(self.h, layer.encode(), name.encode(), _fp(out), size))
        return out

    def params(self) -> np.ndarray:
        out = np.empty(self.n_params, np.float32)
        check(self.lib.b2g_net_get_params(self.h, _fp(out), out.size))
        return out

    def set_params(self, flat):
        v = _f32(flat).ravel()
        check(self.lib.b2g_net_set_params(self.h, _fp(v), v.size))

    def gradients(self) -> np.ndarray:
        out = np.empty(self.n_params, np.float32)
        check(self.lib.b2g_net_get_gradients(self.h, _fp(out), out.size))
        return out

    def updater_state_size(self) -> int:
        n = C.c_int64()
        check(self.lib.b2g_net_updater_state_size(self.h, C.byref(n)))
        return n.value

    def updater_state(self) -> np.ndarray:
        out = np.empty(self.updater_state_size(), np.float32)
        check(self.lib.b2g_net_get_updater_state(self.h, _fp(out), out.size))
        return out

    def set_updater_state(self, st):
        v = _f32(st).ravel()
        check(self.lib.b2g_net_set_updater_state(self.h, _fp(v), v.size))

    def save(self, path, save_updater: bool = True):
        from . import serializer
        serializer.save_net(self, path, self.specs, self.input_shape, save_updater,
                            {"precision": "bf16" if self.precision == BF16 else "fp32", "max_batch": self.max_batch, "iteration": self.iteration(),
                             "dropout_pass": self.dropout_pass(), "epoch": self.epoch()})

    def restore(self, path, load_updater: bool = True):
        from . import serializer
        return serializer.restore_into(self, path, load_updater)

    def output(self, x, train: bool = False) -> np.ndarray:
        x = _f32(x)
        out = np.empty((x.shape[0], self.out_elems), np.float32)
        check(self.lib.b2g_net_output(self.h, _fp(x), x.shape[0], int(train), _fp(out)))
        return out

    def layer_output_size(self, layer: int) -> int:
        n = C.c_int64()
        check(self.lib.b2g_net_layer_output_size(self.h, layer, C.byref(n)))
        return n.value

    def activation(self, layer: int, batch: int) -> np.ndarray:
        out = np.empty((batch, self.layer_output_size(layer)), np.float32)
        check(self.lib.b2g_net_get_activation(self.h, layer, batch, _fp(out)))
        return out

    def compute_gradient_and_score(self, x, y) -> float:
        x, y = _f32(x), _f32(y)
        s = C.c_float()
        check(self.lib.b2g_net_compute_gradient_and_score(self.h, _fp(x), _fp(y), x.shape[0], C.byref(s)))
        return s.value

    def fit(self, x, y) -> float:
        x, y = _f32(x), _f32(y)
        s = C.c_float()
        check(self.lib.b2g_net_fit(self.h, _fp(x), _fp(y), x.shape[0], C.byref(s)))
        return s.value

    def set_gradient_normalization(self, mode: str, threshold: float = 1.0):
        if mode not in GRADIENT_NORMALIZATIONS:
            raise ValueError(f"unknown gradient normalization {mode!r}; one of {sorted(GRADIENT_NORMALIZATIONS)} (element-wise clipping is grad_clip)")
        check(self.lib.b2g_net_set_gradient_normalization(self.h, GRADIENT_NORMALIZATIONS[mode], float(threshold)))

    def set_lr_schedule(self, schedule: Optional[Dict], layer: Optional[str] = None):
        s, _arrays = schedule_struct(schedule)
        check(self.lib.b2g_net_set_lr_schedule(self.h, None if layer is None else layer.encode(), C.byref(s)))
        follow_lr_schedule(self.specs, self.lr_constants, schedule, layer)

    def learning_rate(self, layer: str) -> float:
        v = C.c_float()
        check(self.lib.b2g_net_get_learning_rate(self.h, layer.encode(), C.byref(v)))
        return v.value

    def epoch(self) -> int:
        v = C.c_int64()
        check(self.lib.b2g_net_get_epoch(self.h, C.byref(v)))
        return v.value

    def set_epoch(self, epoch: int):
        check(self.lib.b2g_net_set_epoch(self.h, int(epoch)))

    def set_grad_allreduce(self, enabled: bool):
        check(self.lib.b2g_net_set_grad_allreduce(self.h, int(enabled)))

    def set_sync_bn(self, enabled: bool):
        check(self.lib.b2g_net_set_sync_bn(self.h, int(enabled)))

    def set_grad_payload_bf16(self, enabled: bool):
        check(self.lib.b2g_net_set_grad_payload_bf16(self.h, int(enabled)))

    def enable_p2p_allreduce(self) -> bool:
        out = C.c_int32(0)
        check(self.lib.b2g_net_enable_p2p_allreduce(self.h, C.byref(out)))
        return bool(out.value)

    def average_parameters(self):
        check(self.lib.b2g_net_average_parameters(self.h))

    def iteration(self) -> int:
        v = C.c_int64()
        check(self.lib.b2g_net_get_iteration(self.h, C.byref(v)))
        return v.value

    def set_iteration(self, it: int):
        check(self.lib.b2g_net_set_iteration(self.h, int(it)))

    def dropout_pass(self) -> int:
        v = C.c_int64()
        check(self.lib.b2g_net_get_dropout_pass(self.h, C.byref(v)))
        return v.value

    def set_dropout_pass(self, p: int):
        check(self.lib.b2g_net_set_dropout_pass(self.h, int(p)))

    def simt_gemm_calls(self) -> int:
        v = C.c_uint64()
        check(self.lib.b2g_net_simt_gemm_calls(self.h, C.byref(v)))
        return v.value

    def time_hbm_kernels(self, rows: int, channels: int, iters: int = 10):
        ms = np.zeros(3, np.float32)
        check(self.lib.b2g_test_hbm_kernels(self.h, rows, channels, iters, _fp(ms)))
        return [float(v) for v in ms]

    def weight_operand(self, layer: int, which: int, size: int) -> np.ndarray:
        out = np.empty(size, np.float32)
        check(self.lib.b2g_test_net_shadow(self.h, layer, which, _fp(out), out.size))
        return out

    def input_gradient(self, batch: int) -> np.ndarray:
        out = np.empty((batch, int(np.prod(self.input_shape))), np.float32)
        check(self.lib.b2g_net_get_input_gradient(self.h, batch, _fp(out)))
        return out

    def close(self):
        if self.h:
            self.lib.b2g_net_destroy(self.h)
            self.h = None


class Gan:

    def __init__(self, gen: Net, dis: Net, fake_bn_train: bool = False, use_cuda_graph: bool = True):
        self.gen, self.dis, self.lib = gen, dis, gen.lib
        cfg = GanConfig(int(fake_bn_train), int(use_cuda_graph))
        h = C.c_void_p()
        check(self.lib.b2g_gan_create(gen.h, dis.h, C.byref(cfg), C.byref(h)))
        self.h = h

    def step(self, x_real, z_d, z_g, y_real, y_fake, y_gen):
        a = [_f32(v) for v in (x_real, z_d, z_g, y_real, y_fake, y_gen)]
        losses = np.zeros(3, np.float32)
        check(self.lib.b2g_gan_step(self.h, *[_fp(v) for v in a], a[0].shape[0], _fp(losses)))
        return losses

    def step_ptr(self, ptrs, batch: int, losses: np.ndarray):
        args = [C.cast(C.c_void_p(p), C.POINTER(C.c_float)) for p in ptrs]
        check(self.lib.b2g_gan_step(self.h, *args, batch, _fp(losses)))

    def upload(self, x_real, z_d, z_g, y_real, y_fake, y_gen):
        a = [_f32(v) for v in (x_real, z_d, z_g, y_real, y_fake, y_gen)]
        check(self.lib.b2g_gan_upload(self.h, *[_fp(v) for v in a], a[0].shape[0]))
        self.gen.ctx.sync()

    def step_resident(self, batch: int):
        check(self.lib.b2g_gan_step_resident(self.h, batch))

    def losses(self) -> np.ndarray:
        out = np.zeros(3, np.float32)
        check(self.lib.b2g_gan_read_losses(self.h, _fp(out)))
        return out

    def last_step_ms(self) -> float:
        v = C.c_float()
        check(self.lib.b2g_gan_last_step_ms(self.h, C.byref(v)))
        return v.value

    def close(self):
        if self.h:
            self.lib.b2g_gan_destroy(self.h)
            self.h = None


def test_conv(ctx: Context, kind: int, impl: int, precision: int, geom: Dict[str, int], a, b, out_size: int, iters: int = 1):
    g = _lib.ConvGeom(**geom)
    a, b = _f32(a).ravel(), _f32(b).ravel()
    out = np.empty(out_size, np.float32)
    ms = C.c_float()
    check(ctx.lib.b2g_test_conv(ctx.h, kind, impl, precision, C.byref(g), _fp(a), _fp(b), _fp(out), iters, C.byref(ms)))
    return out, ms.value


EPI_PLAIN, EPI_STATS, EPI_BNBWD, EPI_ACTBWD = 0, 1, 2, 3


def test_conv_ex(ctx: Context, kind: int, geom: Dict[str, int], a, b, out_size: int, *, epi: int = 0, act: str = "identity", alpha: float = 0.0,
                 bias=None, scale=None, groups: int = 1, aux=None, aux2=None, iters: int = 1, impl: int = 1, bn: int = 0, max_ctas: int = 0,
                 poison: bool = False, w_mn: bool = False, per_tap: bool = False, info: Optional[dict] = None, defer: bool = False, db=None,
                 precision: int = BF16, param_offset: int = 0):
    g = _lib.ConvGeom(**geom)
    a, b = _f32(a).ravel(), _f32(b).ravel()
    out = np.empty(out_size, np.float32)
    oc = geom["o"] if kind == 0 else geom["c"]
    o = _lib.TestConvOpts()
    o.epi, o.act, o.alpha, o.groups = epi, ACTS[act], alpha, groups
    o.bn, o.max_ctas, o.poison, o.w_mn, o.per_tap, o.defer = bn, max_ctas, int(poison), int(w_mn), int(per_tap), int(defer)
    o.param_offset = param_offset
    if db is not None:
        assert db.dtype == np.float32 and db.flags.c_contiguous
        o.db = _fp(db)
    keep = []
    for name, v in (("bias", bias), ("scale", scale), ("aux", aux), ("aux2", aux2)):
        if v is not None:
            arr = _f32(v).ravel(); keep.append(arr); setattr(o, name, _fp(arr))
    stats = None
    if epi in (EPI_STATS, EPI_BNBWD):
        stats = np.zeros((groups, 2, oc), np.float64); o.stats = stats.ctypes.data_as(C.POINTER(C.c_double))
    ms = C.c_float()
    check(ctx.lib.b2g_test_conv_ex(ctx.h, kind, impl, precision, C.byref(g), _fp(a), _fp(b), _fp(out), iters, C.byref(ms), C.byref(o)))
    if info is not None:
        info["slab"], info["splits"] = bool(o.slab), o.splits
    return out, stats, o.kernel.decode(), ms.value


def test_bn(ctx: Context, precision: int, path: int, x, eps_out, gamma, beta, run_mean, run_var, *, act: str = "identity", alpha: float = 0.0,
            eps: float = 1e-5, decay: float = 0.9, g_gamma=None, g_beta=None, want_param_grads: bool = True):
    x, e = _f32(x), _f32(eps_out)
    groups, rows, ch = x.shape
    par = [_f32(v).ravel() for v in (gamma, beta, run_mean, run_var)]
    r = {k: np.empty(x.shape, np.float32) for k in ("y", "eps_in")}
    r["g_gamma"] = _f32(np.zeros(ch) if g_gamma is None else g_gamma).copy()
    r["g_beta"] = _f32(np.zeros(ch) if g_beta is None else g_beta).copy()
    r.update({k: np.empty(ch, np.float32) for k in ("g_mean", "g_var")})
    r.update({k: np.empty((groups, ch), np.float32) for k in ("mean", "invstd")})
    check(ctx.lib.b2g_test_bn(ctx.h, precision, path, groups, rows, ch, _fp(x), _fp(e), *[_fp(v) for v in par], ACTS[act], alpha, eps, decay,
                              int(want_param_grads), *[_fp(r[k]) for k in ("y", "eps_in", "g_gamma", "g_beta", "g_mean", "g_var", "mean", "invstd")]))
    return r


def test_dropout(ctx: Context, precision: int, x, dy, p: float, *, seed: int = 666, layer: int = 0, rank: int = 0, pass_: int = 0):
    x, e = _f32(x), _f32(dy)
    rows = x.shape[0]
    h, w, c = (x.shape[1:] if x.ndim == 4 else (1, 1, int(np.prod(x.shape[1:]))))
    y, dx = np.empty_like(x), np.empty_like(x)
    check(ctx.lib.b2g_test_dropout(ctx.h, precision, seed, layer, rank, pass_, rows, h, w, c, p, _fp(x), _fp(e), _fp(y), _fp(dx)))
    return y, dx


EW_OPS = {"reduce_splits": 0, "reduce_multi": 1, "colsum": 2, "xent": 3, "softmax_xent": 4, "act_fwd": 5, "act_bwd": 6, "maxpool": 7,
          "upsample": 8, "sumsq": 9, "loss": 10}


def test_ew(ctx: Context, precision: int, op: str, in0, in1=None, out_sizes=(0, 0, 0), *, act: str = "identity", jobs=None, segments=None,
            loss: str = "xent", **opts):
    o = _lib.TestEwOpts()
    o.op, o.act, o.loss = EW_OPS[op], ACTS[act], LOSSES[loss]
    for k, v in opts.items():
        setattr(o, k, int(v) if isinstance(v, bool) else v)
    keep = []
    if jobs is not None:
        arr = (_lib.EwReduceJob * len(jobs))(*[_lib.EwReduceJob(j["n"], j["stride"], j["src_off"], j["dst_off"], j["splits"], 0) for j in jobs])
        o.n_jobs, o.jobs = len(jobs), arr
        keep.append(arr)
    if segments is not None:
        so, sl, sc = (np.ascontiguousarray(segments[0], np.int64), np.ascontiguousarray(segments[1], np.int64), _f32(segments[2]))
        keep += [so, sl, sc]
        o.n_seg = len(so)
        o.seg_off, o.seg_len, o.seg_coef = so.ctypes.data_as(C.POINTER(C.c_int64)), sl.ctypes.data_as(C.POINTER(C.c_int64)), _fp(sc)
    ins = [None if v is None else _f32(v).ravel() for v in (in0, in1)]
    outs = [np.empty(k, np.float32) if k else None for k in out_sizes]
    ptr = lambda a: None if a is None else _fp(a)
    check(ctx.lib.b2g_test_ew(ctx.h, precision, C.byref(o), *[ptr(a) for a in ins], *[ptr(a) for a in outs]))
    info = {"kernel": o.kernel.decode(), "sumsq": o.sumsq, "wide": [o.jobs[i].wide for i in range(o.n_jobs)] if jobs is not None else []}
    return outs, info
```

include/b200gan.h:

```cpp
#ifndef B200GAN_H
#define B200GAN_H

#include <stddef.h>
#include <stdint.h>

#ifdef __cplusplus
extern "C" {
#endif

#define B2G_VERSION 101
#define B2G_NAME_LEN 64

typedef struct b2g_ctx b2g_ctx;
typedef struct b2g_net b2g_net;
typedef struct b2g_gan b2g_gan;

typedef enum {
  B2G_OK = 0,
  B2G_ERR_ARG = -1,
  B2G_ERR_SHAPE = -2,
  B2G_ERR_CUDA = -3,
  B2G_ERR_NCCL = -4,
  B2G_ERR_OOM = -5,
  B2G_ERR_UNSUPPORTED = -6,
  B2G_ERR_NO_DEVICE = -7
} b2g_status;

typedef enum {
  B2G_LAYER_CONV2D = 0,
  B2G_LAYER_DECONV2D = 1,
  B2G_LAYER_BATCHNORM = 2,
  B2G_LAYER_DENSE = 3,
  B2G_LAYER_ACTIVATION = 4,
  B2G_LAYER_MAXPOOL = 5,
  B2G_LAYER_UPSAMPLE2D = 6,
  B2G_LAYER_OUTPUT = 7,
  B2G_LAYER_LOSS = 8,
  B2G_LAYER_FF_TO_CNN = 9,
  B2G_LAYER_CNN_TO_FF = 10,
  B2G_LAYER_DROPOUT = 11
} b2g_layer_type;


typedef enum {
  B2G_ACT_IDENTITY = 0, B2G_ACT_TANH = 1, B2G_ACT_SIGMOID = 2, B2G_ACT_RELU = 3, B2G_ACT_LRELU = 4
} b2g_activation;

typedef enum {
  B2G_UPD_SGD = 0, B2G_UPD_RMSPROP = 1, B2G_UPD_ADAM = 2, B2G_UPD_NOOP = 3, B2G_UPD_NESTEROVS = 4, B2G_UPD_ADAGRAD = 5, B2G_UPD_ADAMAX = 6,
  B2G_UPD_NADAM = 7, B2G_UPD_AMSGRAD = 8, B2G_UPD_ADADELTA = 9
} b2g_updater;

typedef enum { B2G_PREC_FP32 = 0, B2G_PREC_BF16 = 1 } b2g_precision;
typedef enum {
  B2G_LOSS_XENT = 0, B2G_LOSS_MCXENT = 1, B2G_LOSS_MSE = 2, B2G_LOSS_L1 = 3, B2G_LOSS_L2 = 4, B2G_LOSS_MAE = 5, B2G_LOSS_HINGE = 6,
  B2G_LOSS_SQUARED_HINGE = 7, B2G_LOSS_WASSERSTEIN = 8
} b2g_loss;

typedef struct {
  int32_t type;
  char name[B2G_NAME_LEN];
  int32_t n_in, n_out;
  int32_t k_h, k_w, s_h, s_w, p_h, p_w;
  int32_t has_bias;
  int32_t act;
  float act_alpha;
  int32_t updater;
  float lr, beta1, beta2, eps;
  float l2;
  float bn_decay, bn_eps;
  int32_t pre_h, pre_w, pre_c;
  int32_t loss;
  int32_t frozen;
} b2g_layer_desc;

typedef struct {
  int32_t in_h, in_w, in_c;
  int32_t max_batch;
  int32_t precision;
  float grad_clip;
  float xent_clip_eps;
  int32_t bn_groups;
  uint64_t seed;
} b2g_net_config;

int32_t b2g_version(void);
int32_t b2g_ctx_create(int32_t device, b2g_ctx** out);
int32_t b2g_ctx_destroy(b2g_ctx* ctx);
const char* b2g_last_error(void);
int32_t b2g_sync(b2g_ctx* ctx);
int32_t b2g_launch_count(b2g_ctx* ctx, uint64_t* out);
int32_t b2g_timer_start(b2g_ctx* ctx);
int32_t b2g_timer_stop_ms(b2g_ctx* ctx, float* ms);
int32_t b2g_flush_l2(b2g_ctx* ctx);
int32_t b2g_device_info(b2g_ctx* ctx, int32_t* sm_count, int32_t* cc_major, int32_t* cc_minor, uint64_t* mem_bytes);

int32_t b2g_net_create(b2g_ctx* ctx, const b2g_net_config* cfg, const b2g_layer_desc* layers, int32_t n_layers, b2g_net** out);
int32_t b2g_net_destroy(b2g_net* net);
int32_t b2g_net_num_params(b2g_net* net, int64_t* out);
int32_t b2g_net_output_size(b2g_net* net, int64_t* per_example);
int32_t b2g_net_layer_output_size(b2g_net* net, int32_t layer, int64_t* per_example);
int32_t b2g_net_set_param(b2g_net* net, const char* layer, const char* param, const float* host, int64_t n);
int32_t b2g_net_get_param(b2g_net* net, const char* layer, const char* param, float* host, int64_t n);
int32_t b2g_net_get_params(b2g_net* net, float* host, int64_t n);
int32_t b2g_net_set_params(b2g_net* net, const float* host, int64_t n);
int32_t b2g_net_get_gradients(b2g_net* net, float* host, int64_t n);
int32_t b2g_net_updater_state_size(b2g_net* net, int64_t* out);
int32_t b2g_net_get_updater_state(b2g_net* net, float* host, int64_t n);
int32_t b2g_net_set_updater_state(b2g_net* net, const float* host, int64_t n);
int32_t b2g_net_output(b2g_net* net, const float* x, int32_t batch, int32_t train, float* out);
int32_t b2g_net_get_activation(b2g_net* net, int32_t layer, int32_t batch, float* host);
int32_t b2g_net_compute_gradient_and_score(b2g_net* net, const float* x, const float* y, int32_t batch, float* score);
int32_t b2g_net_get_input_gradient(b2g_net* net, int32_t batch, float* host);
int32_t b2g_net_fit(b2g_net* net, const float* x, const float* y, int32_t batch, float* score);
int32_t b2g_net_get_iteration(b2g_net* net, int64_t* out);
int32_t b2g_net_set_iteration(b2g_net* net, int64_t iteration);
int32_t b2g_net_get_dropout_pass(b2g_net* net, int64_t* out);
int32_t b2g_net_set_dropout_pass(b2g_net* net, int64_t pass);
typedef enum {
  B2G_GN_NONE = 0, B2G_GN_RENORM_L2_LAYER = 1, B2G_GN_RENORM_L2_PARAM = 2, B2G_GN_CLIP_ELEMENTWISE = 3, B2G_GN_CLIP_L2_LAYER = 4, B2G_GN_CLIP_L2_PARAM = 5
} b2g_gradient_normalization;
int32_t b2g_net_set_gradient_normalization(b2g_net* net, int32_t mode, float threshold);
typedef enum {
  B2G_SCHED_NONE = 0, B2G_SCHED_EXPONENTIAL = 1, B2G_SCHED_INVERSE = 2, B2G_SCHED_SIGMOID = 3, B2G_SCHED_STEP = 4, B2G_SCHED_MAP = 5
} b2g_schedule_kind;
typedef enum { B2G_SCHED_ITERATION = 0, B2G_SCHED_EPOCH = 1 } b2g_schedule_type;
typedef struct {
  int32_t kind, type;
  double initial, gamma, power, step, decay_rate;
  int32_t n_map;
  const int32_t* map_keys;
  const double* map_values;
} b2g_lr_schedule;
int32_t b2g_net_set_lr_schedule(b2g_net* net, const char* layer, const b2g_lr_schedule* s);
int32_t b2g_net_get_learning_rate(b2g_net* net, const char* layer, float* out);
int32_t b2g_net_get_epoch(b2g_net* net, int64_t* out);
int32_t b2g_net_set_epoch(b2g_net* net, int64_t epoch);
int32_t b2g_net_simt_gemm_calls(b2g_net* net, uint64_t* out);

typedef struct {
  int32_t fake_bn_train;
  int32_t use_cuda_graph;
} b2g_gan_config;
int32_t b2g_gan_create(b2g_net* gen, b2g_net* dis, const b2g_gan_config* cfg, b2g_gan** out);
int32_t b2g_gan_destroy(b2g_gan* gan);
int32_t b2g_gan_step(b2g_gan* gan, const float* x_real, const float* z_d, const float* z_g,
                     const float* y_real, const float* y_fake, const float* y_gen, int32_t batch, float* losses);
int32_t b2g_gan_upload(b2g_gan* gan, const float* x_real, const float* z_d, const float* z_g,
                       const float* y_real, const float* y_fake, const float* y_gen, int32_t batch);
int32_t b2g_gan_step_resident(b2g_gan* gan, int32_t batch);
int32_t b2g_gan_read_losses(b2g_gan* gan, float* losses);
int32_t b2g_gan_last_step_ms(b2g_gan* gan, float* ms);

#define B2G_NCCL_ID_BYTES 128
int32_t b2g_comm_unique_id(void* id128);
int32_t b2g_ctx_comm_init(b2g_ctx* ctx, int32_t world, int32_t rank, const void* id128);
int32_t b2g_ctx_comm_destroy(b2g_ctx* ctx);
int32_t b2g_net_set_grad_allreduce(b2g_net* net, int32_t enabled);
int32_t b2g_net_average_parameters(b2g_net* net);
int32_t b2g_net_set_sync_bn(b2g_net* net, int32_t enabled);
int32_t b2g_net_set_grad_payload_bf16(b2g_net* net, int32_t enabled);
int32_t b2g_net_enable_p2p_allreduce(b2g_net* net, int32_t* enabled);
int32_t b2g_ctx_allreduce_test(b2g_ctx* ctx, float* host_inout, int64_t n);

typedef struct {
  int32_t n, h, w, c;
  int32_t oh, ow, o;
  int32_t kh, kw, sh, sw, ph, pw;
} b2g_conv_geom;
int32_t b2g_test_conv(b2g_ctx* ctx, int32_t kind, int32_t impl, int32_t precision, const b2g_conv_geom* g,
                      const float* x_or_dy, const float* w_or_x, float* out, int32_t iters, float* ms_per_iter);
typedef struct {
  int32_t epi;
  int32_t act; float alpha;
  const float* bias;
  const float* scale;
  int32_t groups;
  const float* aux;
  const float* aux2;
  double* stats;
  char kernel[64];
  int32_t bn;
  int32_t max_ctas;
  int32_t poison;
  int32_t w_mn;
  int32_t per_tap;
  int32_t slab;
  int32_t defer;
  float* db;
  int32_t param_offset;
  int32_t splits;
} b2g_test_conv_opts;
int32_t b2g_test_conv_ex(b2g_ctx* ctx, int32_t kind, int32_t impl, int32_t precision, const b2g_conv_geom* g,
                         const float* x_or_dy, const float* w_or_x, float* out, int32_t iters, float* ms_per_iter, b2g_test_conv_opts* opts);

int32_t b2g_test_hbm_kernels(b2g_net* net, int32_t rows, int32_t channels, int32_t iters, float* ms3);

int32_t b2g_test_bn(b2g_ctx* ctx, int32_t precision, int32_t path, int32_t groups, int32_t rows, int32_t C, const float* x, const float* eps_out,
                    const float* gamma, const float* beta, const float* run_mean, const float* run_var, int32_t act, float alpha, float eps, float decay,
                    int32_t want_param_grads, float* y, float* eps_in, float* g_gamma, float* g_beta, float* g_mean, float* g_var, float* mean, float* invstd);
int32_t b2g_test_net_shadow(b2g_net* net, int32_t layer, int32_t which, float* out, int64_t n);
int32_t b2g_test_dropout(b2g_ctx* ctx, int32_t precision, uint64_t seed, int32_t layer, int32_t rank, int64_t pass, int32_t rows, int32_t h, int32_t w,
                         int32_t c, float p, const float* x, const float* dy, float* y, float* dx);

typedef enum {
  B2G_EW_REDUCE_SPLITS = 0, B2G_EW_REDUCE_MULTI = 1, B2G_EW_COLSUM = 2, B2G_EW_XENT = 3, B2G_EW_SOFTMAX_XENT = 4,
  B2G_EW_ACT_FWD = 5, B2G_EW_ACT_BWD = 6, B2G_EW_MAXPOOL = 7, B2G_EW_UPSAMPLE = 8, B2G_EW_SUMSQ = 9, B2G_EW_LOSS = 10
} b2g_ew_op;
typedef struct {
  int64_t n, stride, src_off, dst_off;
  int32_t splits;
  int32_t wide;
} b2g_ew_reduce_job;
typedef struct {
  int32_t op;
  int64_t n;
  int32_t rows, cols;
  int32_t groups;
  int32_t splits; int64_t stride;
  int32_t N, H, W, C, KH, KW, SH, SW;
  int32_t act; float alpha;
  float clip_eps;
  int32_t offset;
  int32_t in_place;
  int32_t accumulate;
  int32_t poison;
  int32_t n_jobs; b2g_ew_reduce_job* jobs;
  int32_t n_seg; const int64_t* seg_off; const int64_t* seg_len; const float* seg_coef;
  double sumsq;
  char kernel[64];
  int32_t loss;
} b2g_test_ew_opts;
int32_t b2g_test_ew(b2g_ctx* ctx, int32_t precision, b2g_test_ew_opts* opts, const float* in0, const float* in1, float* out0, float* out1, float* out2);

#ifdef __cplusplus
}
#endif
#endif
```

Measured before the change: 89660.

## Use 2-CTA clusters with TMA multicast for slab-path weight tiles

Adds a cluster-of-two variant of the tensor-core conv kernel for the slab path in dgrad mode. Each CTA of the pair loads one of the two taps' weight tiles and multicasts it to both CTAs, and both release each stage through a cluster-wide empty barrier. The goal is to halve redundant weight traffic from L2. In exchange it adds cluster synchronisation, cross-CTA barrier arrivals, a drain loop at the end, and grid sizing based on cluster occupancy.

```diff
diff --git a/gan_deeplearning4j_b200/__init__.py b/gan_deeplearning4j_b200/__init__.py
--- a/gan_deeplearning4j_b200/__init__.py
+++ b/gan_deeplearning4j_b200/__init__.py
@@ -1,3 +1,3 @@
 from ._lib import B200GanError, LIB_PATH, PROTOTYPES, load
-from .engine import BF16, FP32, EPI_ACTBWD, EPI_BNBWD, EPI_PLAIN, EPI_STATS, Context, Gan, Net, comm_unique_id, test_bn, test_conv, test_conv_ex, test_dropout, test_ew
+from .engine import BF16, FP32, EPI_ACTBWD, EPI_BNBWD, EPI_PLAIN, EPI_STATS, Context, Gan, Net, comm_unique_id, set_tc_cluster, tc_last_cluster, test_bn, test_conv, test_conv_ex, test_dropout, test_ew
 from . import data, models, parallel, serializer
diff --git a/gan_deeplearning4j_b200/_lib.py b/gan_deeplearning4j_b200/_lib.py
--- a/gan_deeplearning4j_b200/_lib.py
+++ b/gan_deeplearning4j_b200/_lib.py
@@ -123,6 +123,8 @@
     "b2g_test_conv": (_i32, [_vp, _i32, _i32, _i32, C.POINTER(ConvGeom), _fp, _fp, _fp, _i32, _fp]),
     "b2g_test_hbm_kernels": (_i32, [_vp, _i32, _i32, _i32, _fp]),
     "b2g_test_conv_ex": (_i32, [_vp, _i32, _i32, _i32, C.POINTER(ConvGeom), _fp, _fp, _fp, _i32, _fp, C.POINTER(TestConvOpts)]),
+    "b2g_test_set_tc_cluster": (_i32, [_i32]),
+    "b2g_test_tc_last_cluster": (_i32, []),
     "b2g_test_bn": (_i32, [_vp, _i32, _i32, _i32, _i32, _i32, _fp, _fp, _fp, _fp, _fp, _fp, _i32, C.c_float, C.c_float, C.c_float,
                            _i32, _fp, _fp, _fp, _fp, _fp, _fp, _fp, _fp]),
     "b2g_test_net_shadow": (_i32, [_vp, _i32, _i32, _fp, _i64]),
diff --git a/gan_deeplearning4j_b200/csrc/common.cuh b/gan_deeplearning4j_b200/csrc/common.cuh
--- a/gan_deeplearning4j_b200/csrc/common.cuh
+++ b/gan_deeplearning4j_b200/csrc/common.cuh
@@ -14,11 +14,16 @@
 __device__ __forceinline__ void pdl_trigger() { asm volatile("griddepcontrol.launch_dependents;" ::: "memory"); }
 __device__ __forceinline__ void pdl_enter() { pdl_trigger(); pdl_wait(); }
 template <typename... KArgs, typename... Args>
+inline cudaError_t launch_pdl_cluster(unsigned cluster_x, void (*kernel)(KArgs...), dim3 grid, dim3 block, size_t smem, cudaStream_t stream, Args&&... args) {
+  cudaLaunchConfig_t cfg{}; cfg.gridDim = grid; cfg.blockDim = block; cfg.dynamicSmemBytes = smem; cfg.stream = stream;
+  cudaLaunchAttribute at[2]; at[0].id = cudaLaunchAttributeProgrammaticStreamSerialization; at[0].val.programmaticStreamSerializationAllowed = 1;
+  at[1].id = cudaLaunchAttributeClusterDimension; at[1].val.clusterDim.x = cluster_x; at[1].val.clusterDim.y = 1; at[1].val.clusterDim.z = 1;
+  cfg.attrs = at; cfg.numAttrs = cluster_x > 1 ? 2 : 1;
+  return cudaLaunchKernelEx(&cfg, kernel, static_cast<KArgs>(args)...);
+}
+template <typename... KArgs, typename... Args>
 inline cudaError_t launch_pdl(void (*kernel)(KArgs...), dim3 grid, dim3 block, size_t smem, cudaStream_t stream, Args&&... args) {
-  cudaLaunchConfig_t cfg{}; cfg.gridDim = grid; cfg.blockDim = block; cfg.dynamicSmemBytes = smem; cfg.stream = stream;
-  cudaLaunchAttribute at[1]; at[0].id = cudaLaunchAttributeProgrammaticStreamSerialization; at[0].val.programmaticStreamSerializationAllowed = 1;
-  cfg.attrs = at; cfg.numAttrs = 1;
-  return cudaLaunchKernelEx(&cfg, kernel, static_cast<KArgs>(args)...);
+  return launch_pdl_cluster(1u, kernel, grid, block, smem, stream, static_cast<Args&&>(args)...);
 }
 
 __device__ __forceinline__ void sacc_add(unsigned long long* hi_lo, size_t stride, size_t idx, double d) {
diff --git a/gan_deeplearning4j_b200/csrc/engine.cu b/gan_deeplearning4j_b200/csrc/engine.cu
--- a/gan_deeplearning4j_b200/csrc/engine.cu
+++ b/gan_deeplearning4j_b200/csrc/engine.cu
@@ -1391,7 +1391,7 @@
   }
   cudaEvent_t e0, e1; CU(cudaEventCreate(&e0)); CU(cudaEventCreate(&e1));
   int reps = iters < 1 ? 1 : iters; int rc = 0;
-  g_tc_last_kernel = ""; g_tc_last_slab = false; g_gemm_last_kernel = ""; g_gemm_last_splits = 0;
+  g_tc_last_kernel = ""; g_tc_last_slab = false; g_tc_last_cluster = 0; g_gemm_last_kernel = ""; g_gemm_last_splits = 0;
   TcTestSchedule schedule(force_bn, max_ctas, per_tap);
   for (int it = -1; it < reps; ++it) {
     if (it == 0) CU(cudaEventRecord(e0, s));
@@ -1450,6 +1450,11 @@
 extern "C" int32_t b2g_test_conv(b2g_ctx* c, int32_t kind, int32_t impl, int32_t precision, const b2g_conv_geom* gg, const float* a_host, const float* b_host, float* out, int32_t iters, float* ms_per_iter) {
   return b2g_test_conv_ex(c, kind, impl, precision, gg, a_host, b_host, out, iters, ms_per_iter, nullptr);
 }
+extern "C" int32_t b2g_test_set_tc_cluster(int32_t mode) {
+  if (mode != 0 && mode != 1) return fail(B2G_ERR_ARG, "tc cluster mode %d: 0 = production, 1 = one-CTA kernel", mode);
+  g_tc_test_no_cluster = mode; return 0;
+}
+extern "C" int32_t b2g_test_tc_last_cluster(void) { return g_tc_last_cluster; }
 
 extern "C" int32_t b2g_test_bn(b2g_ctx* c, int32_t precision, int32_t path, int32_t groups, int32_t rows, int32_t C, const float* x, const float* eps_out,
                                const float* gamma, const float* beta, const float* run_mean, const float* run_var, int32_t act, float alpha, float eps, float decay,
diff --git a/gan_deeplearning4j_b200/csrc/kernels.h b/gan_deeplearning4j_b200/csrc/kernels.h
--- a/gan_deeplearning4j_b200/csrc/kernels.h
+++ b/gan_deeplearning4j_b200/csrc/kernels.h
@@ -136,6 +136,7 @@
 extern int g_tc_test_bn, g_tc_test_max_ctas;
 extern int g_tc_test_per_tap;
 extern bool g_tc_last_slab;
+extern int g_tc_test_no_cluster, g_tc_last_cluster;
 enum { EPI_PLAIN = 0, EPI_STATS = 1, EPI_BNBWD = 2, EPI_ACTBWD = 3 };
 struct TcEpi {
   int mode;
diff --git a/gan_deeplearning4j_b200/csrc/kernels_tc.cu b/gan_deeplearning4j_b200/csrc/kernels_tc.cu
--- a/gan_deeplearning4j_b200/csrc/kernels_tc.cu
+++ b/gan_deeplearning4j_b200/csrc/kernels_tc.cu
@@ -53,6 +53,15 @@
   asm volatile("cp.async.bulk.tensor.2d.shared::cluster.global.tile.mbarrier::complete_tx::bytes [%0], [%1, {%3, %4}], [%2];"
                ::"r"(dst), "l"(map), "r"(bar), "r"(c0), "r"(c1) : "memory");
 }
+__device__ __forceinline__ void tma_load_3d_mc(uint32_t dst, const CUtensorMap* map, uint32_t bar, int c0, int c1, int c2, uint16_t mask) {
+  asm volatile("cp.async.bulk.tensor.3d.shared::cluster.global.tile.mbarrier::complete_tx::bytes.multicast::cluster [%0], [%1, {%3, %4, %5}], [%2], %6;"
+               ::"r"(dst), "l"(map), "r"(bar), "r"(c0), "r"(c1), "r"(c2), "h"(mask) : "memory");
+}
+__device__ __forceinline__ uint32_t cluster_ctarank() { uint32_t r; asm volatile("mov.u32 %0, %%cluster_ctarank;" : "=r"(r)); return r; }
+__device__ __forceinline__ void mbar_arrive_cluster(uint32_t bar, uint32_t cta) {
+  asm volatile("{\n\t.reg .b32 ra;\n\tmapa.shared::cluster.u32 ra, %0, %1;\n\tmbarrier.arrive.shared::cluster.b64 _, [ra];\n\t}" ::"r"(bar), "r"(cta) : "memory");
+}
+__device__ __forceinline__ void cluster_sync() { asm volatile("barrier.cluster.arrive.release;\n\tbarrier.cluster.wait.acquire;" ::: "memory"); }
 __device__ __forceinline__ bool elect_one_sync() {
   uint32_t pred = 0;
   asm volatile("{\n\t.reg .pred P1;\n\t.reg .b32 rx;\n\telect.sync rx|P1, %1;\n\t@P1 mov.s32 %0, 1;\n\t}" : "+r"(pred) : "r"(0xffffffffu));
@@ -281,12 +290,13 @@
   }
 }
 
-template <int BN>
+template <int BN, bool MC = false>
 __device__ __forceinline__ void load_b_tile(const TcConvParams& p, const CUtensorMap* tmB, uint32_t dst, uint32_t bar, int ch, int wtap, int nb0) {
-  if (!p.b_mn) tma_load_3d(dst, tmB, bar, ch * 64, wtap, nb0);
+  auto box = [&](uint32_t d, int c0, int c1, int c2) { if constexpr (MC) tma_load_3d_mc(d, tmB, bar, c0, c1, c2, 0x3); else tma_load_3d(d, tmB, bar, c0, c1, c2); };
+  if (!p.b_mn) box(dst, ch * 64, wtap, nb0);
   else {
 #pragma unroll
-    for (int j = 0; j < (BN >= 64 ? BN / 64 : 1); ++j) tma_load_3d(dst + j * 8192, tmB, bar, nb0 + j * 64, wtap, ch * 64);
+    for (int j = 0; j < (BN >= 64 ? BN / 64 : 1); ++j) box(dst + j * 8192, nb0 + j * 64, wtap, ch * 64);
   }
 }
 template <int BN, int NB, int NACC>
@@ -326,15 +336,16 @@
   tap_coords(p, p.mode == 0 ? ta + 2 : 0, tb, py, px, ax2, dy2, whi);
 }
 
-template <int BN>
+template <int BN, int CL>
 struct TcConvRegs {
-  static constexpr int LAUNCH = 96, PRODUCER = 24, MMA = BN >= 128 ? 96 : 64, EPI = BN >= 128 ? 128 : 160;
+  static constexpr int LAUNCH = 96, PRODUCER = CL > 1 ? 32 : 24, MMA = BN >= 128 ? 96 : 64, EPI = BN >= 128 ? 128 : 160;
   static_assert(PRODUCER + 2 * MMA + 2 * EPI <= 5 * LAUNCH, "setmaxnreg budget exceeds the launch allocation");
 };
-template <int BN, int STAGES, int EPI, bool AFFINE, bool PS = false, bool SLAB = false>
+template <int BN, int STAGES, int EPI, bool AFFINE, bool PS = false, bool SLAB = false, int CL = 1>
 __global__ void __launch_bounds__(TC_CONV_THREADS, 1) tc_conv_kernel(const __grid_constant__ CUtensorMap tmA, const __grid_constant__ CUtensorMap tmB, const TcConvParams p) {
+  static_assert(CL == 1 || (CL == 2 && SLAB), "CTA pairs share the two taps' weight tiles of the slab path");
   using S = TcSmem<BN, STAGES, EPI, SLAB>;
-  using R = TcConvRegs<BN>;
+  using R = TcConvRegs<BN, CL>;
   constexpr int NB = BN >= 64 ? BN / 64 : 1, NACC = BN >= 64 ? 32 : BN / 2;
   extern __shared__ uint8_t smem_raw[];
   const uint32_t smem_base = (smem_u32(smem_raw) + 1023u) & ~1023u;
@@ -355,17 +366,19 @@
 
   if (threadIdx.x == 0) {
     prefetch_map(&tmA); prefetch_map(&tmB);
-    for (int s = 0; s < STAGES; ++s) { mbar_init(bar_full + 8 * s, 1); mbar_init(bar_empty + 8 * s, 8); }
+    for (int s = 0; s < STAGES; ++s) { mbar_init(bar_full + 8 * s, 1); mbar_init(bar_empty + 8 * s, 8 * CL); }
     for (int k = 0; k < S::PARKS; ++k) { mbar_init(park_full + 8 * k, 256); mbar_init(park_empty + 8 * k, 256); }
     fence_mbar_init();
   }
   __syncthreads();
+  if constexpr (CL > 1) cluster_sync();
   pdl_wait();
 
   if (warp >= 16) {
     setmaxnreg_dec<R::PRODUCER>();
     if (warp == 16) {
       int s = 0; uint32_t ph = 0;
+      const int rank = CL > 1 ? (int)cluster_ctarank() : 0;
       for (int t = blockIdx.x; t < tiles; t += gridDim.x) {
         int nb0, phase, n0, y0; tile_coords(t, nb0, phase, n0, y0);
         const int py = phase >> 1, px = phase & 1;
@@ -380,20 +393,31 @@
             const uint32_t st = smem_base + s * S::STAGE_BYTES;
             mbar_expect_tx(bar_full + 8 * s, SLAB ? p.slab_bytes + S::B_BYTES : S::STAGE_BYTES);
             tma_load_4d(st, &tmA, bar_full + 8 * s, ch * 64, ax, ybase + dy_, n0);
-            load_b_tile<BN>(p, &tmB, st + S::A_BYTES, bar_full + 8 * s, ch, wtap, nb0);
-            if constexpr (SLAB) load_b_tile<BN>(p, &tmB, st + S::A_BYTES + BN * 128, bar_full + 8 * s, ch, wtap2, nb0);
+            if constexpr (CL > 1) {
+              load_b_tile<BN, true>(p, &tmB, st + S::A_BYTES + rank * BN * 128, bar_full + 8 * s, ch, rank ? wtap2 : wtap, nb0);
+            } else {
+              load_b_tile<BN>(p, &tmB, st + S::A_BYTES, bar_full + 8 * s, ch, wtap, nb0);
+              if constexpr (SLAB) load_b_tile<BN>(p, &tmB, st + S::A_BYTES + BN * 128, bar_full + 8 * s, ch, wtap2, nb0);
+            }
           }
           __syncwarp();
           if (++s == STAGES) { s = 0; ph ^= 1; }
           if (++ch == p.chunks) { ch = 0; if (++tb == p.taps_w) { tb = 0; ++ta; } coords(); }
         }
       }
+      if constexpr (CL > 1) {
+        for (int i = 0; i < STAGES; ++i) { mbar_wait(bar_empty + 8 * s, ph ^ 1); if (++s == STAGES) { s = 0; ph ^= 1; } }
+      }
     }
   } else if (warp < 8) {
     if constexpr (R::MMA < R::LAUNCH) setmaxnreg_dec<R::MMA>();
     const int wg = warp >> 2;
     const int r0 = wg * 64 + (warp & 3) * 16 + (lane >> 2);
     int s = 0, k = 0; uint32_t ph = 0, kph = 0;
+    auto release = [&](int slot) {
+      mbar_arrive(bar_empty + 8 * slot);
+      if constexpr (CL > 1) mbar_arrive_cluster(bar_empty + 8 * slot, cluster_ctarank() ^ 1);
+    };
     for (int t = blockIdx.x; t < tiles; t += gridDim.x) {
       float acc[NB][NACC];
 #pragma unroll
@@ -414,12 +438,12 @@
         }
         wg_commit();
         wg_wait<1>();
-        if (prev >= 0 && lane == 0) mbar_arrive(bar_empty + 8 * prev);
+        if (prev >= 0 && lane == 0) release(prev);
         prev = s;
         if (++s == STAGES) { s = 0; ph ^= 1; }
       }
       wg_wait<0>();
-      if (lane == 0) mbar_arrive(bar_empty + 8 * prev);
+      if (lane == 0) release(prev);
       mbar_wait(park_empty + 8 * k, kph ^ 1);
       float* park = reinterpret_cast<float*>(smem_gen + S::PARK_OFF + k * S::PARK_BYTES);
 #pragma unroll
@@ -491,7 +515,9 @@
 
 const char* g_tc_last_kernel = "";
 bool g_tc_last_slab = false;
+int g_tc_last_cluster = 0;
 int g_tc_test_bn = 0, g_tc_test_max_ctas = 0, g_tc_test_per_tap = 0;
+int g_tc_test_no_cluster = 0;
 static int tc_device() { int dev = 0; cudaGetDevice(&dev); return dev < 0 || dev >= 64 ? 0 : dev; }
 #define TC_SET_SMEM_ONCE(kernel, bytes)                                                                                            \
   do { static bool set_[64] = {}; const int d_ = tc_device();                                                                       \
@@ -525,33 +551,56 @@
 }
 static bool tc_epi_ok(const TcEpi* e, int Nt) { return !e || e->mode == EPI_PLAIN || e->mode == EPI_ACTBWD || (e->imgs_per_group > 0 && e->imgs_per_group % Nt == 0 && e->acc); }
 
-template <int BN, int STAGES, int EPI, bool AFFINE, bool PS = false, bool SLAB = false>
+template <int BN, int STAGES, int EPI, bool AFFINE, bool PS = false, bool SLAB = false, int CL = 1>
 static int launch_conv_e(const CUtensorMap& tmA, const CUtensorMap& tmB, const TcConvParams& p, cudaStream_t s) {
   using S = TcSmem<BN, STAGES, EPI, SLAB>;
-  TC_SET_SMEM_ONCE((tc_conv_kernel<BN, STAGES, EPI, AFFINE, PS, SLAB>), S::TOTAL);
+  auto kernel = tc_conv_kernel<BN, STAGES, EPI, AFFINE, PS, SLAB, CL>;
+  TC_SET_SMEM_ONCE(kernel, S::TOTAL);
   const long tiles = (long)p.tiles_m * p.tiles_n * p.phases;
-  const unsigned grid = (unsigned)std::min<long>(tiles, g_tc_test_max_ctas > 0 ? g_tc_test_max_ctas : device_sm_count());
-  launch_pdl(tc_conv_kernel<BN, STAGES, EPI, AFFINE, PS, SLAB>, dim3(grid), dim3(TC_CONV_THREADS), (size_t)(S::TOTAL), s, tmA, tmB, p);
-  LAUNCHED();
+  long cap = g_tc_test_max_ctas > 0 ? g_tc_test_max_ctas / CL : device_sm_count();
+  if constexpr (CL > 1) {
+    if (g_tc_test_max_ctas <= 0) {
+      static int clusters_[64] = {};
+      const int d = tc_device();
+      if (!clusters_[d]) {
+        cudaLaunchConfig_t cfg{}; cfg.gridDim = dim3(CL * device_sm_count()); cfg.blockDim = dim3(TC_CONV_THREADS); cfg.dynamicSmemBytes = S::TOTAL;
+        cudaLaunchAttribute at[1]; at[0].id = cudaLaunchAttributeClusterDimension; at[0].val.clusterDim.x = CL; at[0].val.clusterDim.y = 1; at[0].val.clusterDim.z = 1;
+        cfg.attrs = at; cfg.numAttrs = 1;
+        int n = 0;
+        if (cudaOccupancyMaxActiveClusters(&n, kernel, &cfg) != cudaSuccess || n < 1) return -2;
+        clusters_[d] = n;
+      }
+      cap = clusters_[d];
+    }
+  }
+  const unsigned grid = CL * (unsigned)std::min<long>(tiles / CL, cap);
+  launch_pdl_cluster(CL, kernel, dim3(grid), dim3(TC_CONV_THREADS), (size_t)(S::TOTAL), s, tmA, tmB, p);
+  LAUNCHED(); g_tc_last_cluster = CL;
   return cudaPeekAtLastError() == cudaSuccess ? 0 : -3;
 }
-template <int BN, int STAGES, bool SLAB>
+template <int BN, int STAGES, bool SLAB, int CL>
 static int launch_conv(const CUtensorMap& tmA, const CUtensorMap& tmB, const TcConvParams& p, cudaStream_t s, const char* name) {
   g_tc_last_kernel = name; g_tc_last_slab = SLAB;
   switch (p.epi) {
-    case EPI_STATS: return launch_conv_e<BN, STAGES, EPI_STATS, false, false, SLAB>(tmA, tmB, p, s);
-    case EPI_BNBWD: return launch_conv_e<BN, STAGES, EPI_BNBWD, false, false, SLAB>(tmA, tmB, p, s);
-    case EPI_ACTBWD: return launch_conv_e<BN, STAGES, EPI_ACTBWD, false, false, SLAB>(tmA, tmB, p, s);
-  }
-  return (p.scale && p.bias) ? launch_conv_e<BN, STAGES, EPI_PLAIN, true, false, SLAB>(tmA, tmB, p, s) : launch_conv_e<BN, STAGES, EPI_PLAIN, false, false, SLAB>(tmA, tmB, p, s);
-}
-static int dispatch_conv(int BN, bool slab, const CUtensorMap& tmA, const CUtensorMap& tmB, const TcConvParams& p, cudaStream_t s) {
-  switch (BN * 2 + slab) {
-    case 128: return launch_conv<64, 4, false>(tmA, tmB, p, s, "tc_conv_kernel<64,4>");
-    case 256: return launch_conv<128, 4, false>(tmA, tmB, p, s, "tc_conv_kernel<128,4>");
-    case 129: return launch_conv<64, 4, true>(tmA, tmB, p, s, "tc_conv_kernel<64,4>");
+    case EPI_STATS: return launch_conv_e<BN, STAGES, EPI_STATS, false, false, SLAB, CL>(tmA, tmB, p, s);
+    case EPI_BNBWD: return launch_conv_e<BN, STAGES, EPI_BNBWD, false, false, SLAB, CL>(tmA, tmB, p, s);
+    case EPI_ACTBWD: return launch_conv_e<BN, STAGES, EPI_ACTBWD, false, false, SLAB, CL>(tmA, tmB, p, s);
+  }
+  return (p.scale && p.bias) ? launch_conv_e<BN, STAGES, EPI_PLAIN, true, false, SLAB, CL>(tmA, tmB, p, s)
+                             : launch_conv_e<BN, STAGES, EPI_PLAIN, false, false, SLAB, CL>(tmA, tmB, p, s);
+}
+static int dispatch_conv(int BN, bool slab, int cl, const CUtensorMap& tmA, const CUtensorMap& tmB, const TcConvParams& p, cudaStream_t s) {
+  switch (BN * 4 + slab * 2 + (cl - 1)) {
+    case 256: return launch_conv<64, 4, false, 1>(tmA, tmB, p, s, "tc_conv_kernel<64,4>");
+    case 512: return launch_conv<128, 4, false, 1>(tmA, tmB, p, s, "tc_conv_kernel<128,4>");
+    case 258: return launch_conv<64, 4, true, 1>(tmA, tmB, p, s, "tc_conv_kernel<64,4>");
+    case 259: return launch_conv<64, 4, true, 2>(tmA, tmB, p, s, "tc_conv_kernel<64,4>");
   }
   return -4;
+}
+static int conv_cluster(const TcConvParams& p, bool slab) {
+  if (!slab || p.mode != 1 || g_tc_test_no_cluster || p.tiles_m % 2 || (g_tc_test_max_ctas > 0 && g_tc_test_max_ctas % 2)) return 1;
+  return 2;
 }
 static bool slab_tile(const TcConvParams& p, int BN) {
   if (g_tc_test_per_tap || BN != 64 || p.Wt % 8) return false;
@@ -598,7 +647,7 @@
   if (make_map_bf16(&tmA, x, 4, dims, strides, box, es)) return -1;
   p.tiles_m = g.N * g.OH * g.OW / 128; p.tiles_n = g.O / BN; p.phases = 1;
   if (w_mn ? weight_map(&tmB, w, g.C, 1, g.O, 64) : weight_map(&tmB, w, g.O, g.KH * g.KW, g.C, BN)) return -1;
-  return dispatch_conv(BN, slab, tmA, tmB, p, s);
+  return dispatch_conv(BN, slab, conv_cluster(p, slab), tmA, tmB, p, s);
 }
 
 int k_tc_dgrad(const ConvGeom& g, const __nv_bfloat16* dy, const __nv_bfloat16* w, const float* bias, __nv_bfloat16* dx, int act, float alpha, cudaStream_t s, const TcEpi* epi) {
@@ -618,7 +667,7 @@
   if (weight_map(&tmB, w, g.O, 16, g.C, 64)) return -1;
   if (make_map_bf16(&tmA, dy, 4, dims, strides, box, es)) return -1;
   p.tiles_m = g.N * g.OH * g.OW / 128; p.tiles_n = g.C / BN; p.phases = 4;
-  return dispatch_conv(BN, slab, tmA, tmB, p, s);
+  return dispatch_conv(BN, slab, conv_cluster(p, slab), tmA, tmB, p, s);
 }
 
 bool tc_deconv_ps_shape(const ConvGeom& g) { return is_k4s2p1_geom(g) && g.C >= 1 && g.C <= 4 && g.O % 64 == 0; }
diff --git a/gan_deeplearning4j_b200/engine.py b/gan_deeplearning4j_b200/engine.py
--- a/gan_deeplearning4j_b200/engine.py
+++ b/gan_deeplearning4j_b200/engine.py
@@ -459,6 +459,14 @@
     return out, stats, o.kernel.decode(), ms.value
 
 
+def set_tc_cluster(ctx: Context, one_cta: bool):
+    check(ctx.lib.b2g_test_set_tc_cluster(int(one_cta)))
+
+
+def tc_last_cluster(ctx: Context) -> int:
+    return int(ctx.lib.b2g_test_tc_last_cluster())
+
+
 def test_bn(ctx: Context, precision: int, path: int, x, eps_out, gamma, beta, run_mean, run_var, *, act: str = "identity", alpha: float = 0.0,
             eps: float = 1e-5, decay: float = 0.9, g_gamma=None, g_beta=None, want_param_grads: bool = True):
     x, e = _f32(x), _f32(eps_out)
diff --git a/include/b200gan.h b/include/b200gan.h
--- a/include/b200gan.h
+++ b/include/b200gan.h
@@ -193,6 +193,8 @@
 } b2g_test_conv_opts;
 int32_t b2g_test_conv_ex(b2g_ctx* ctx, int32_t kind, int32_t impl, int32_t precision, const b2g_conv_geom* g,
                          const float* x_or_dy, const float* w_or_x, float* out, int32_t iters, float* ms_per_iter, b2g_test_conv_opts* opts);
+int32_t b2g_test_set_tc_cluster(int32_t mode);
+int32_t b2g_test_tc_last_cluster(void);
 
 int32_t b2g_test_hbm_kernels(b2g_net* net, int32_t rows, int32_t channels, int32_t iters, float* ms3);
 
```

Result: no change. 89850 (median of 6 runs) (+0.2%).
